# The-African-Research-Collective/karanta-ocr

Measured on AMD Instinct MI355X. Metric: pages_per_sec, higher is better.
Workload: dtype bf16; 1 GPU; Qwen2-VL-2B bf16 greedy, batch=8 synthetic 1024x1024 pages per GPU, max_pixels=1003520 (grid 70x70, 1225 image tokens), prompt P=1394 tokens, T_out=1024 (ignore_eos), random-init weights; global_batch=8, parallelism=dp1, decode=hipGraph replay

## Files before the change

include/karanta_hip.h:

```cpp
#ifndef KARANTA_HIP_H
#define KARANTA_HIP_H

#include <stddef.h>
#include <stdint.h>

#ifdef __cplusplus
extern "C" {
#endif

typedef void* kr_stream;
typedef uint16_t kr_bf16;

#define KR_ABI_VERSION 403

#define KR_OK 0
#define KR_ERR_ARG (-1)
#define KR_ERR_HIP (-2)
#define KR_ERR_RCCL (-3)
#define KR_ERR_STATE (-4)

#define KR_EPI_NONE 0
#define KR_EPI_QUICK_GELU 1
#define KR_EPI_GELU_ERF 2
#define KR_EPI_SILU_MUL 3
#define KR_EPI_SILU_MUL8 4

int kr_version(void);
const char* kr_last_error(void);
int kr_device_info(int device, char* name64, int* compute_units, size_t* total_mem);
int kr_set_device(int device);
int kr_stream_synchronize(kr_stream s);
int kr_stream_create_cu_mask(kr_stream* out, int cus_enabled);
int kr_stream_create_cu_range(kr_stream* out, int first_cu, int n_cus);
int kr_stream_destroy(kr_stream s);

int kr_event_create(void** ev);
int kr_event_destroy(void* ev);
int kr_event_record(void* ev, kr_stream s);
int kr_stream_wait_event(kr_stream s, void* ev);
int kr_event_synchronize(void* ev);
int kr_event_elapsed_ms(void* start, void* stop, float* ms);

int kr_graph_begin_capture(kr_stream s);
int kr_graph_end_capture(kr_stream s, void** graph_exec);
int kr_graph_launch(void* graph_exec, kr_stream s);
int kr_graph_destroy(void* graph_exec);


int kr_cast_pad_f32_bf16(const float* src, kr_bf16* dst, int64_t rows, int k, int k_pad, kr_stream s);

int kr_layernorm(const kr_bf16* x, const kr_bf16* w, const kr_bf16* b, kr_bf16* y,
                 int64_t rows, int d, float eps, kr_stream s);

int kr_rmsnorm(const kr_bf16* x, int64_t ldx, const kr_bf16* w, kr_bf16* y,
               int64_t rows, int d, float eps, kr_stream s);


int kr_gemm_bf16(const kr_bf16* A, int64_t lda, const kr_bf16* W, const kr_bf16* bias,
                 const kr_bf16* residual, int64_t ldr, kr_bf16* C, int64_t ldc,
                 int64_t M, int N, int K, int epilogue, int w_packed, kr_stream s);

#define KR_GEMM_SCRATCH_BYTES ((size_t)512 * 65536)
int kr_gemm_bf16_ws(const kr_bf16* A, int64_t lda, const kr_bf16* W, const kr_bf16* bias,
                    const kr_bf16* residual, int64_t ldr, kr_bf16* C, int64_t ldc,
                    int64_t M, int N, int K, int epilogue, int w_packed, float* scratch, size_t scratch_bytes, kr_stream s);

int kr_gemm_fp8(const kr_bf16* A, int64_t lda, const uint8_t* w_packed_fp8, const float* w_scale, const kr_bf16* bias,
                const kr_bf16* residual, int64_t ldr, kr_bf16* C, int64_t ldc, int64_t M, int N, int K, int epilogue,
                kr_stream s);

int kr_quantize_rows_fp8(const kr_bf16* x, int64_t ldx, uint8_t* q, int64_t ldq, float* scale, int64_t rows, int K, kr_stream s);
int kr_gemm_fp8a(const uint8_t* A8, int64_t lda, const float* a_scale, const uint8_t* w_packed_fp8, const float* w_scale,
                 const kr_bf16* bias, const kr_bf16* residual, int64_t ldr, kr_bf16* C, int64_t ldc, int64_t M, int N, int K,
                 int epilogue, kr_stream s);

int kr_gemv_bf16(const kr_bf16* x, int64_t ldx, const kr_bf16* W, const kr_bf16* bias,
                 const kr_bf16* residual, int64_t ldr, kr_bf16* out, float* out_f32, int64_t ldc,
                 int M, int N, int K, int epilogue,
                 const kr_bf16* norm_w, float norm_eps, kr_stream s);


int kr_qkv_prep(const kr_bf16* qkv, int64_t ld_qkv, int q_off, int k_off, int v_off,
                const float* cos, const float* sin,
                const int32_t* blk_tok0, const int32_t* blk_ntok,
                const int64_t* blk_k_row0, const int64_t* blk_vt_blk, int n_blk,
                kr_bf16* q_out, int64_t q_head_stride, kr_bf16* k_out, int64_t k_head_stride,
                kr_bf16* vt_out, int64_t vt_head_stride, int q_heads, int kv_heads, int hd,
                kr_stream s);

int kr_rope2d_vision(kr_bf16* x, const float* cos, const float* sin, int64_t n, int heads, int hd,
                     int64_t row_stride, kr_stream s);

int kr_attn_varlen(const kr_bf16* q, const kr_bf16* k, const kr_bf16* vt, kr_bf16* out,
                   const int32_t* qblk, const int32_t* qblk_len, int n_qblk,
                   int64_t nq_total, int q_heads, int kv_heads, int hd,
                   int64_t k_head_stride, int64_t vt_head_stride, float scale, int causal,
                   kr_stream s);
int kr_attn_varlen_q(const kr_bf16* q, const kr_bf16* k, const kr_bf16* vt, kr_bf16* out,
                     const int32_t* qblk, const int32_t* qblk_len, int n_qblk,
                     int64_t nq_total, int q_heads, int kv_heads, int hd,
                     int64_t k_head_stride, int64_t vt_head_stride, float scale, int causal,
                     int q_block, kr_stream s);


int kr_embed_scatter(const int32_t* src, const kr_bf16* table, const kr_bf16* image_embeds,
                     kr_bf16* out, int64_t rows, int d, kr_stream s);


int kr_mrope(kr_bf16* x, const float* cos, const float* sin, int64_t n, int heads, int hd,
             int64_t row_stride, kr_stream s);
int kr_kv_append(const kr_bf16* k, const kr_bf16* v, int64_t row_stride,
                 const int32_t* tok_seq, const int32_t* tok_pos,
                 kr_bf16* kcache, kr_bf16* vtcache,
                 int64_t n, int kv_heads, int hd, int layer, int batch, int s_max, kr_stream s);

int kr_decode_qkv_prep(const kr_bf16* qkv, const float* inv_freq, const int32_t* ctx_len,
                       const int32_t* rope_delta, kr_bf16* q_out, kr_bf16* kcache, kr_bf16* vtcache,
                       int batch, int heads, int kv_heads, int hd, int layer, int s_max, kr_stream s);

int kr_attn_decode_gqa(const kr_bf16* q, const kr_bf16* kcache, const kr_bf16* vtcache,
                       const int32_t* ctx_len, kr_bf16* out, float* workspace,
                       int batch, int heads, int kv_heads, int hd, int layer, int s_max,
                       int n_split, float scale, kr_stream s);

int kr_argmax_embed(const float* logits, int64_t ld_logits, int vocab,
                    const kr_bf16* embed_table, int d,
                    int32_t* tokens_out, int32_t* history, int32_t* step_ptr, int32_t* ctx_len,
                    int32_t* finished, const int32_t* eos, int n_eos, int pad_id, int ignore_eos,
                    kr_bf16* x_next, int batch, int hist_stride, kr_stream s);

int kr_argmax(const float* logits, int64_t ld_logits, int vocab, int32_t* out, int batch, kr_stream s);

#define KR_DEC_PLAIN 0
#define KR_DEC_SILU 1
#define KR_DEC_ROPE_KV 2
#define KR_DEC_ARGMAX 3
#define KR_DEC_SILU8 4
#define KR_DEC_OUT_XP 0x100
int kr_linear_decode(int mode, const kr_bf16* x, int64_t ldx, const kr_bf16* w_packed, const kr_bf16* bias,
                     const kr_bf16* norm_w, float norm_eps, const kr_bf16* residual, int64_t ldr,
                     kr_bf16* out, float* out_f32, int64_t ldc, int M, int N, int K, int waves, int max_blocks, int ksplit,
                     float* ws, int32_t* counters, const float* attn_partials, int attn_split,
                     const float* cs_table, int cs_stride, const int32_t* prompt_len, const int32_t* ctx_len,
                     kr_bf16* q_out, kr_bf16* kcache, kr_bf16* vtcache, int heads, int kv_heads, int s_max,
                     float* amax_val, int32_t* amax_idx, kr_stream s);

int kr_linear_decode_wide(int mode, const kr_bf16* x, int64_t ldx, const kr_bf16* w_packed, const kr_bf16* bias,
                          const kr_bf16* norm_w, float norm_eps, const kr_bf16* residual, int64_t ldr,
                          kr_bf16* out, float* out_f32, int64_t ldc, int M, int N, int K, int blocks, int waves,
                          float* amax_val, int32_t* amax_idx, kr_stream s);

typedef struct kr_narrow_opts {
    float* zero_ptr;
    uint64_t zero_bytes;
    int32_t atomic_out;
    int32_t part_rows;
} kr_narrow_opts;

int kr_linear_decode_narrow(int mode, const kr_bf16* x, int64_t ldx, const float* part_in, int n_part_in,
                            kr_bf16* x_out, int64_t ldxo, const kr_bf16* w_packed, const kr_bf16* bias,
                            const kr_bf16* norm_w, float norm_eps, const kr_bf16* residual, int64_t ldr,
                            kr_bf16* out, float* out_f32, int64_t ldc, int M, int N, int K, int waves, int ksplit,
                            const float* cs_table, int cs_stride, const int32_t* prompt_len, const int32_t* ctx_len,
                            kr_bf16* q_out, kr_bf16* kcache, kr_bf16* vtcache, int heads, int kv_heads, int s_max,
                            const kr_narrow_opts* opts, kr_stream s);

int kr_decode_resnorm(const kr_bf16* x, int64_t ldx, const float* part_in, int n_part_in, int part_rows, kr_bf16* x_out,
                      int64_t ldxo, const kr_bf16* norm_w, float norm_eps, kr_bf16* h, int64_t ldh, int M, int K, kr_stream s);

int kr_linear_decode_wide_fp8(int mode, const kr_bf16* x, int64_t ldx, const uint8_t* w_packed_fp8, const float* w_scale,
                              const kr_bf16* bias, const kr_bf16* norm_w, float norm_eps, const kr_bf16* residual,
                              int64_t ldr, kr_bf16* out, float* out_f32, int64_t ldc, int M, int N, int K, int blocks,
                              int waves, float* amax_val, int32_t* amax_idx, kr_stream s);
int kr_linear_decode_narrow_fp8(int mode, const kr_bf16* x, int64_t ldx, const float* part_in, int n_part_in,
                                kr_bf16* x_out, int64_t ldxo, const uint8_t* w_packed_fp8, const float* w_scale,
                                const kr_bf16* bias, const kr_bf16* norm_w, float norm_eps, const kr_bf16* residual,
                                int64_t ldr, kr_bf16* out, float* out_f32, int64_t ldc, int M, int N, int K, int waves,
                                int ksplit, const float* cs_table, int cs_stride, const int32_t* prompt_len,
                                const int32_t* ctx_len, kr_bf16* q_out, kr_bf16* kcache, kr_bf16* vtcache, int heads,
                                int kv_heads, int s_max, const kr_narrow_opts* opts, kr_stream s);
int kr_pack_rows32(const kr_bf16* x, int64_t ldx, int M, int K, kr_bf16* xp, kr_stream s);

typedef struct kr_dec32 {
    const kr_bf16* xp;
    const void* w_packed;
    const float* w_scale;
    const kr_bf16* bias;
    const kr_bf16* residual;
    int64_t ldr;
    kr_bf16* out;
    float* out_f32;
    int64_t ldc;
    int32_t M, N, K;
    int32_t waves_ref, ksplit;
    int32_t atomic_out;
    int32_t tiles_per_wg;
    int32_t group_split;
    int32_t reserved0;
    float* zero_ptr;
    uint64_t zero_bytes;
    const float* cs_table; int32_t cs_stride; const int32_t* prompt_len; const int32_t* ctx_len;
    kr_bf16* q_out; kr_bf16* kcache; kr_bf16* vtcache; int32_t heads, kv_heads, s_max;
} kr_dec32;
int kr_linear_decode32(int mode, const kr_dec32* args, kr_stream s);

int kr_decode_resnorm32(const kr_bf16* x, int64_t ldx, const float* part_in, int n_part_in, int part_rows, kr_bf16* x_out,
                        int64_t ldxo, const kr_bf16* norm_w, float norm_eps, kr_bf16* h_xp, int M, int K, int sum_slabs_first,
                        kr_stream s);

int kr_fp8_to_bf16(const uint8_t* src, kr_bf16* dst, int64_t n, kr_stream s);

int kr_attn_decode_fused(const kr_bf16* q, const kr_bf16* kcache, const kr_bf16* vtcache,
                         const int32_t* ctx_len, kr_bf16* out, float* workspace, int32_t* counters,
                         int batch, int heads, int kv_heads, int hd, int s_max, int n_split,
                         float scale, kr_stream s);
int kr_attn_decode_slots(const kr_bf16* q, const kr_bf16* kcache, const kr_bf16* vtcache, const int32_t* ctx_len,
                         const int32_t* finished, float* workspace, int batch, int heads, int kv_heads, int hd, int s_max,
                         int n_split, float scale, kr_stream s);
// ... 85 lines not shown
```

karanta_ocr_amd/_lib.py:

```python
from __future__ import annotations

import ctypes as C
import os
from typing import Optional

_HERE = os.path.dirname(os.path.abspath(__file__))
LIB_PATH = os.path.join(_HERE, "libkaranta_hip.so")

c_p = C.c_void_p
i32, i64, f32 = C.c_int, C.c_int64, C.c_float


class KarantaHipError(RuntimeError):
    pass


SIGNATURES = {
    "kr_version": [],
    "kr_last_error": [],
    "kr_device_info": [i32, C.c_char_p, C.POINTER(i32), C.POINTER(C.c_size_t)],
    "kr_set_device": [i32],
    "kr_stream_synchronize": [c_p],
    "kr_stream_create_cu_mask": [C.POINTER(c_p), i32],
    "kr_stream_create_cu_range": [C.POINTER(c_p), i32, i32],
    "kr_stream_destroy": [c_p],
    "kr_event_create": [C.POINTER(c_p)],
    "kr_event_destroy": [c_p],
    "kr_event_record": [c_p, c_p],
    "kr_event_synchronize": [c_p],
    "kr_stream_wait_event": [c_p, c_p],
    "kr_event_elapsed_ms": [c_p, c_p, C.POINTER(f32)],
    "kr_graph_begin_capture": [c_p],
    "kr_graph_end_capture": [c_p, C.POINTER(c_p)],
    "kr_graph_launch": [c_p, c_p],
    "kr_graph_destroy": [c_p],
    "kr_cast_pad_f32_bf16": [c_p, c_p, i64, i32, i32, c_p],
    "kr_layernorm": [c_p, c_p, c_p, c_p, i64, i32, f32, c_p],
    "kr_rmsnorm": [c_p, i64, c_p, c_p, i64, i32, f32, c_p],
    "kr_gemm_bf16": [c_p, i64, c_p, c_p, c_p, i64, c_p, i64, i64, i32, i32, i32, i32, c_p],
    "kr_decode_resnorm": [c_p, i64, c_p, i32, i32, c_p, i64, c_p, f32, c_p, i64, i32, i32, c_p],
    "kr_decode_resnorm32": [c_p, i64, c_p, i32, i32, c_p, i64, c_p, f32, c_p, i32, i32, i32, c_p],
    "kr_pack_rows32": [c_p, i64, i32, i32, c_p, c_p],
    "kr_linear_decode32": [i32, c_p, c_p],
    "kr_attn_decode_merge32": [c_p, c_p, i32, i32, i32, i32, c_p],
    "kr_quantize_rows_fp8": [c_p, i64, c_p, i64, c_p, i64, i32, c_p],
    "kr_gemm_fp8a": [c_p, i64, c_p, c_p, c_p, c_p, c_p, i64, c_p, i64, i64, i32, i32, i32, c_p],
    "kr_gemm_bf16_ws": [c_p, i64, c_p, c_p, c_p, i64, c_p, i64, i64, i32, i32, i32, i32, c_p, C.c_size_t, c_p],
    "kr_gemv_bf16": [c_p, i64, c_p, c_p, c_p, i64, c_p, c_p, i64, i32, i32, i32, i32, c_p, f32, c_p],
    "kr_qkv_prep": [c_p, i64, i32, i32, i32, c_p, c_p, c_p, c_p, c_p, c_p, i32, c_p, i64, c_p, i64, c_p, i64,
                    i32, i32, i32, c_p],
    "kr_rope2d_vision": [c_p, c_p, c_p, i64, i32, i32, i64, c_p],
    "kr_attn_varlen": [c_p, c_p, c_p, c_p, c_p, c_p, i32, i64, i32, i32, i32, i64, i64, f32, i32, c_p],
    "kr_attn_varlen_q": [c_p, c_p, c_p, c_p, c_p, c_p, i32, i64, i32, i32, i32, i64, i64, f32, i32, i32, c_p],
    "kr_embed_scatter": [c_p, c_p, c_p, c_p, i64, i32, c_p],
    "kr_mrope": [c_p, c_p, c_p, i64, i32, i32, i64, c_p],
    "kr_kv_append": [c_p, c_p, i64, c_p, c_p, c_p, c_p, i64, i32, i32, i32, i32, i32, c_p],
    "kr_decode_qkv_prep": [c_p, c_p, c_p, c_p, c_p, c_p, c_p, i32, i32, i32, i32, i32, i32, c_p],
    "kr_attn_decode_gqa": [c_p, c_p, c_p, c_p, c_p, c_p, i32, i32, i32, i32, i32, i32, i32, f32, c_p],
    "kr_argmax_embed": [c_p, i64, i32, c_p, i32, c_p, c_p, c_p, c_p, c_p, c_p, i32, i32, i32, c_p, i32, i32, c_p],
    "kr_argmax": [c_p, i64, i32, c_p, i32, c_p],
    "kr_linear_decode": [i32, c_p, i64, c_p, c_p, c_p, f32, c_p, i64, c_p, c_p, i64, i32, i32, i32, i32, i32, i32, c_p, c_p,
                         c_p, i32, c_p, i32, c_p, c_p, c_p, c_p, c_p, i32, i32, i32, c_p, c_p, c_p],
    "kr_linear_decode_wide": [i32, c_p, i64, c_p, c_p, c_p, f32, c_p, i64, c_p, c_p, i64, i32, i32, i32, i32, i32, c_p, c_p, c_p],
    "kr_image_resize_bicubic_u8": [c_p, i32, i32, c_p, i32, i32, c_p, c_p, c_p, i32, c_p, c_p, i32, c_p],
    "kr_image_normalize_patchify": [c_p, i32, i32, c_p, c_p, i32, i32, i32, c_p, c_p],
    "kr_linear_decode_wide_fp8": [i32, c_p, i64, c_p, c_p, c_p, c_p, f32, c_p, i64, c_p, c_p, i64, i32, i32, i32, i32, i32, c_p, c_p, c_p],
    "kr_linear_decode_narrow_fp8": [i32, c_p, i64, c_p, i32, c_p, i64, c_p, c_p, c_p, c_p, f32, c_p, i64, c_p, c_p, i64,
                                    i32, i32, i32, i32, i32, c_p, i32, c_p, c_p, c_p, c_p, c_p, i32, i32, i32, c_p, c_p],
    "kr_fp8_to_bf16": [c_p, c_p, i64, c_p],
    "kr_gemm_fp8": [c_p, i64, c_p, c_p, c_p, c_p, i64, c_p, i64, i64, i32, i32, i32, c_p],
    "kr_gumbel_argmax": [c_p, i64, i32, c_p, c_p, c_p, c_p, c_p, c_p, i32, i32, c_p],
    "kr_gumbel_argmax_guided": [c_p, i64, i32, c_p, c_p, c_p, c_p, c_p, c_p, i32, i32, c_p, c_p, i32, i32, c_p],
    "kr_guide_build_masks": [c_p, c_p, i32, c_p, c_p, i32, c_p, i32, c_p, i32, c_p],
    "kr_sample_threshold": [c_p, i64, i32, c_p, c_p, c_p, i64, c_p, i32, c_p, c_p, i32, c_p, i32, c_p, i64, c_p, c_p, i32, c_p],
    "kr_gumbel_argmax_processed": [c_p, i64, i32, c_p, c_p, c_p, c_p, c_p, c_p, i32, i32, c_p, c_p, i32, i32, c_p, c_p, i64, c_p,
                                   i32, c_p, c_p],
    "kr_sample_count": [c_p, c_p, c_p, i64, i32, i32, c_p],
    "kr_logits_adjust": [c_p, i64, i32, c_p, c_p, c_p, c_p, c_p, c_p, c_p, i32, c_p],
    "kr_logits_restore": [c_p, i64, i32, c_p, c_p, c_p, i32, c_p],
    "kr_stop_tokens": [c_p, c_p, c_p, c_p, c_p, i32, i32, c_p],
    "kr_guide_advance": [c_p, c_p, c_p, c_p, c_p, c_p, i32, i32, c_p],
    "kr_logprobs_topk": [c_p, i64, i32, i32, i32, c_p, c_p, c_p, c_p, c_p, c_p, c_p, c_p, c_p, i32, i32, i32, i32, c_p],
    "kr_linear_decode_narrow": [i32, c_p, i64, c_p, i32, c_p, i64, c_p, c_p, c_p, f32, c_p, i64, c_p, c_p, i64,
                                i32, i32, i32, i32, i32, c_p, i32, c_p, c_p, c_p, c_p, c_p, i32, i32, i32, c_p, c_p],
    "kr_attn_decode_fused": [c_p, c_p, c_p, c_p, c_p, c_p, c_p, i32, i32, i32, i32, i32, i32, f32, c_p],
    "kr_attn_decode_slots": [c_p, c_p, c_p, c_p, c_p, c_p, i32, i32, i32, i32, i32, i32, f32, c_p],
    "kr_attn_decode_merge": [c_p, c_p, i32, i32, i32, i32, c_p],
    "kr_sample_greedy": [c_p, c_p, i32, c_p, i32, c_p, c_p, i32, c_p, c_p, c_p, c_p, i32, i32, i32, c_p, i32, c_p],
    "kr_comm_unique_id": [c_p],
    "kr_comm_init": [C.POINTER(c_p), i32, i32, c_p],
    "kr_comm_count": [c_p, C.POINTER(i32)],
    "kr_comm_destroy": [c_p],
    "kr_rccl_version": [C.POINTER(i32)],
    "kr_bcast_weights": [c_p, c_p, C.c_size_t, i32, c_p],
    "kr_selftest_mfma": [c_p],
    "kr_probe_launch_floor": [c_p, i32, i32, i32, C.POINTER(f32)],
    "kr_probe_stream_read": [c_p, C.c_size_t, i32, i32, c_p, C.POINTER(f32)],
    "kr_launch_null": [c_p],
}
_RESTYPES = {"kr_last_error": C.c_char_p}

EXPERIMENT_SIGNATURES = {
    "kr_linear_decode_narrow_x32": [i32, c_p, i64, c_p, i32, c_p, i64, c_p, i64, c_p, c_p, c_p, c_p, f32, c_p, i64, c_p, c_p, i64,
                                    i32, i32, i32, i32, i32, c_p, i32, c_p, c_p, c_p, c_p, c_p, i32, i32, i32, c_p,
                                    c_p, C.c_size_t, i32, c_p],
    "kr_oproj_heads": [c_p, i32, c_p, c_p, c_p, i64, i32, i32, i32, c_p],
    "kr_linear_decode_wide_x32": [i32, c_p, i64, c_p, i64, c_p, c_p, c_p, f32, c_p, c_p, i64, i32, i32, i32, i32, i32, c_p, c_p, c_p],
    "kr_prefetch": [c_p, C.c_size_t, i32, c_p],
}


class NarrowOpts(C.Structure):
    _fields_ = [("zero_ptr", c_p), ("zero_bytes", C.c_uint64), ("atomic_out", C.c_int32), ("part_rows", C.c_int32)]


def narrow_opts(zero_ptr: int = 0, zero_bytes: int = 0, atomic_out: bool = False, part_rows: int = 0):
    if not (zero_bytes or atomic_out or part_rows):
        return None
    return C.byref(NarrowOpts(zero_ptr or None, int(zero_bytes), 1 if atomic_out else 0, int(part_rows)))

class Dec32(C.Structure):
    _fields_ = [("xp", c_p), ("w_packed", c_p), ("w_scale", c_p), ("bias", c_p), ("residual", c_p), ("ldr", C.c_int64),
                ("out", c_p), ("out_f32", c_p), ("ldc", C.c_int64), ("M", C.c_int32), ("N", C.c_int32), ("K", C.c_int32),
                ("waves_ref", C.c_int32), ("ksplit", C.c_int32), ("atomic_out", C.c_int32), ("tiles_per_wg", C.c_int32),
                ("group_split", C.c_int32), ("reserved0", C.c_int32), ("zero_ptr", c_p), ("zero_bytes", C.c_uint64),
                ("cs_table", c_p), ("cs_stride", C.c_int32), ("prompt_len", c_p), ("ctx_len", c_p),
                ("q_out", c_p), ("kcache", c_p), ("vtcache", c_p), ("heads", C.c_int32), ("kv_heads", C.c_int32), ("s_max", C.c_int32)]


ABI_MAJOR = 4
DEC_OUT_XP = 0x100
ADJ_CAP = 320
EPI_NONE, EPI_QUICK_GELU, EPI_GELU_ERF, EPI_SILU_MUL, EPI_SILU_MUL8 = 0, 1, 2, 3, 4
DEC_PLAIN, DEC_SILU, DEC_ROPE_KV, DEC_ARGMAX, DEC_SILU8 = 0, 1, 2, 3, 4


class _Lib:
    def __init__(self, path: str):
        if not os.path.exists(path):
            raise KarantaHipError(
                f"{path} not found: build it with `python -m karanta_ocr_amd.build` "
                "(the MI355X engine has no CPU fallback)")
        import torch

        try:
            self._dll = C.CDLL(path, mode=C.RTLD_GLOBAL)
        except OSError as e:
            raise KarantaHipError(f"cannot load {path}: {e}") from e
        self.path = path
        for name, argtypes in SIGNATURES.items():
            try:
                fn = getattr(self._dll, name)
            except AttributeError as e:
                raise KarantaHipError(f"{path} does not export {name}") from e
            fn.argtypes = argtypes
            fn.restype = _RESTYPES.get(name, C.c_int)
            if name in ("kr_version", "kr_last_error"):
                setattr(self, name, fn)
            else:
                setattr(self, name, self._checked(name, fn))
        if self.kr_version() // 100 != ABI_MAJOR:
            raise KarantaHipError(f"{path} reports kr_version() = {self.kr_version()}, this binding is written against ABI major "
                                  f"{ABI_MAJOR} (include/karanta_hip.h): rebuild with `python -m karanta_ocr_amd.build`")
        self.experiments = hasattr(self._dll, "kr_oproj_heads")
        for name, argtypes in EXPERIMENT_SIGNATURES.items():
            if self.experiments:
                fn = getattr(self._dll, name)
                fn.argtypes, fn.restype = argtypes, C.c_int
                setattr(self, name, self._checked(name, fn))
            else:
                setattr(self, name, self._absent(name))

    @staticmethod
    def _absent(name):
        def call(*_):
            raise KarantaHipError(f"{name} is an experiment entry point (include/karanta_hip_experiments.h): this library was built "
                                  "without -DKR_EXPERIMENTS (csrc/tools/build_variant.py; load it through KARANTA_HIP_LIB)")
        call.__name__ = name
        return call

    def _checked(self, name, fn):
        def call(*args):
            rc = fn(*args)
            if rc != 0:
                msg = self._dll.kr_last_error()
                raise KarantaHipError(f"{name} -> {rc}: {msg.decode() if msg else ''}")
            return rc

        call.__name__ = name
        call.raw = fn
        return call


_LIB: Optional[_Lib] = None


def lib() -> _Lib:
    global _LIB
    if _LIB is None:
        _LIB = _Lib(os.environ.get("KARANTA_HIP_LIB", LIB_PATH))
# ... 6 lines not shown
```

karanta_ocr_amd/csrc/kr_gemm.hip:

```cpp
#include <algorithm>
#include <cstdlib>
#include <mutex>
#include <optional>

#include "kr_common.h"

namespace {

constexpr int BK = 64;
struct G128 { static constexpr int BM = 128, BN = 128, WM = 2, WN = 2; };
struct G256 { static constexpr int BM = 256, BN = 256, WM = 2, WN = 4; };

__device__ __forceinline__ int lds_off(int r, int c) { return r * 128 + ((c ^ ((r >> 1) & 7)) << 4); }

template <bool PACKED, int ROWS, int NTHR>
__device__ __forceinline__ void stage_tile(const kr_bf16* __restrict__ g, int64_t ld, int64_t row0, int64_t rows_total,
                                           int k0, char* lds_tile, int tid, int wave) {
#pragma unroll
    for (int p = 0; p < ROWS * 8 / NTHR; ++p) {
        const int idx = p * NTHR + tid;
        const int r = idx >> 3, cp = idx & 7;
        const int c = cp ^ ((r >> 1) & 7);
        int64_t gr = row0 + r;
        gr = gr < rows_total ? gr : rows_total - 1;
// ... 5 lines not shown
    }
}

template <int EPI, int NT, int MT, bool LDSEPI, bool HAS_R, int CH = 0>
__device__ __forceinline__ void gemm_epilogue_impl(f32x4 (&acc)[NT][MT], const kr_bf16* __restrict__ bias,
                                                   const kr_bf16* __restrict__ R, int64_t ldr, kr_bf16* __restrict__ C, int64_t ldc,
                                                   int64_t M, int N, int64_t m_base, int n_base, int fr, int fg, char* wlds_) {
    constexpr bool HALF = EPI == KR_EPI_SILU_MUL8;
    constexpr int ROWB = HALF ? 64 : 128;
    char* const wlds = wlds_;
    auto swz = [](int r) { return HALF ? ((r >> 1) & 3) : (r & 7); };
    auto flush = [&](int mt0, int nmt) {
        constexpr int LPR = ROWB / 16, RPI = 64 / LPR;
        const int lane = fg * 16 + fr;
        const int n_out = HALF ? (n_base >> 1) : n_base, n_lim = HALF ? (N >> 1) : N;
#pragma unroll
        for (int it = 0; it < MT * 16 / RPI; ++it) {
            if (it < nmt * 16 / RPI) {
                const int r = it * RPI + lane / LPR, c = lane % LPR;
                const u32x4 v = *reinterpret_cast<const u32x4*>(wlds + r * ROWB + ((c ^ swz(r)) << 4));
                const int64_t m = m_base + mt0 * 16 + r;
                const int n = n_out + c * 8;
                if (m < M && n < n_lim) *reinterpret_cast<u32x4*>(C + m * ldc + n) = v;
            }
        }
    };
    constexpr int RM = CH > 0 ? CH : MT;
    if (EPI == KR_EPI_SILU_MUL8) {
        bf16x4 bv[NT];
#pragma unroll
        for (int nt = 0; nt < NT; ++nt) {
            const int n = min(n_base + nt * 16, N - 16);
            bv[nt] = bias ? *reinterpret_cast<const bf16x4*>(bias + n + fg * 4) : bf16x4{};
        }
#pragma unroll
        for (int mt = 0; mt < MT; ++mt) {
            const int64_t m = m_base + mt * 16 + fr;
#pragma unroll
            for (int nt = 0; nt < NT; ++nt) {
                const int n = n_base + nt * 16;
                float g[4], u[4];
#pragma unroll
                for (int j = 0; j < 4; ++j) g[j] = acc[nt][mt][j] + bf2f(bv[nt][j]);
#pragma unroll
                for (int j = 0; j < 4; ++j) u[j] = __shfl_xor(g[j], 32, 64);
                bf16x4 o;
#pragma unroll
                for (int j = 0; j < 4; ++j) o[j] = f2bf(act_silu(g[j]) * u[j]);
                if (LDSEPI) {
                    const int r = (mt % RM) * 16 + fr;
                    if (fg < 2) *reinterpret_cast<bf16x4*>(wlds + r * ROWB + ((nt ^ swz(r)) << 4) + (fg & 1) * 8) = o;
                } else if (fg < 2 && n < N && m < M) {
                    *reinterpret_cast<bf16x4*>(C + m * ldc + (n >> 1) + fg * 4) = o;
                }
            }
            if (LDSEPI && CH > 0 && (mt % RM) == RM - 1) flush(mt - (RM - 1), RM);
        }
    } else if (EPI == KR_EPI_SILU_MUL) {
#pragma unroll
        for (int mt = 0; mt < MT; ++mt) {
            const int64_t m = m_base + mt * 16 + fr;
            if (m >= M) continue;
#pragma unroll
            for (int pr = 0; pr < NT / 2; ++pr) {
                const int n = n_base + pr * 32 + fg * 4;
                if (n >= N) continue;
                const int oc = ((n_base) >> 1) + pr * 16 + fg * 4;
                bf16x4 o;
#pragma unroll
                for (int j = 0; j < 4; ++j) o[j] = f2bf(act_silu(acc[2 * pr][mt][j]) * acc[2 * pr + 1][mt][j]);
                *reinterpret_cast<bf16x4*>(C + m * ldc + oc) = o;
            }
        }
    } else {
        bf16x4 bv[NT];
        int ncl[NT];
#pragma unroll
        for (int nt = 0; nt < NT; ++nt) {
            ncl[nt] = min(n_base + nt * 16 + fg * 4, N - 4);
            bv[nt] = bias ? *reinterpret_cast<const bf16x4*>(bias + ncl[nt]) : bf16x4{};
        }
#pragma unroll
        for (int mt = 0; mt < MT; ++mt) {
            const int64_t m = m_base + mt * 16 + fr;
            const int64_t mc = m < M ? m : M - 1;
            bf16x4 rv[NT];
#pragma unroll
            for (int nt = 0; nt < NT; ++nt) rv[nt] = HAS_R ? *reinterpret_cast<const bf16x4*>(R + mc * ldr + ncl[nt]) : bf16x4{};
#pragma unroll
            for (int nt = 0; nt < NT; ++nt) {
                const int n = n_base + nt * 16 + fg * 4;
                float v[4];
#pragma unroll
                for (int j = 0; j < 4; ++j) v[j] = acc[nt][mt][j];
                if (bias) {
#pragma unroll
                    for (int j = 0; j < 4; ++j) v[j] += bf2f(bv[nt][j]);
                }
                if (EPI == KR_EPI_QUICK_GELU) {
#pragma unroll
                    for (int j = 0; j < 4; ++j) v[j] = act_quick_gelu(v[j]);
                } else if (EPI == KR_EPI_GELU_ERF) {
#pragma unroll
                    for (int j = 0; j < 4; ++j) v[j] = act_gelu_erf(v[j]);
                }
                if (HAS_R) {
#pragma unroll
                    for (int j = 0; j < 4; ++j) v[j] += bf2f(rv[nt][j]);
                }
                bf16x4 o;
#pragma unroll
                for (int j = 0; j < 4; ++j) o[j] = f2bf(v[j]);
                if (LDSEPI) {
                    const int r = (mt % RM) * 16 + fr;
                    *reinterpret_cast<bf16x4*>(wlds + r * ROWB + (((nt * 2 + (fg >> 1)) ^ swz(r)) << 4) + (fg & 1) * 8) = o;
                } else if (m < M && n < N) {
                    *reinterpret_cast<bf16x4*>(C + m * ldc + n) = o;
                }
            }
            if (LDSEPI && CH > 0 && (mt % RM) == RM - 1) flush(mt - (RM - 1), RM);
        }
    }
    if (LDSEPI && CH == 0) flush(0, MT);
}

template <int EPI, int NT, int MT, bool LDSEPI, int CH = 0>
__device__ __forceinline__ void gemm_epilogue(f32x4 (&acc)[NT][MT], const kr_bf16* __restrict__ bias,
                                              const kr_bf16* __restrict__ R, int64_t ldr, kr_bf16* __restrict__ C, int64_t ldc,
                                              int64_t M, int N, int64_t m_base, int n_base, int fr, int fg, char* wlds) {
    constexpr bool L = LDSEPI && EPI != KR_EPI_SILU_MUL;
    if constexpr (EPI == KR_EPI_SILU_MUL || EPI == KR_EPI_SILU_MUL8) {
        gemm_epilogue_impl<EPI, NT, MT, L, false, CH>(acc, bias, R, ldr, C, ldc, M, N, m_base, n_base, fr, fg, wlds);
    } else {
        if (R) gemm_epilogue_impl<EPI, NT, MT, L, true, CH>(acc, bias, R, ldr, C, ldc, M, N, m_base, n_base, fr, fg, wlds);
        else gemm_epilogue_impl<EPI, NT, MT, L, false, CH>(acc, bias, R, ldr, C, ldc, M, N, m_base, n_base, fr, fg, wlds);
    }
}

__device__ __forceinline__ void tile_coords(unsigned id, unsigned tiles_m, unsigned tiles_n, unsigned group_m, unsigned& tm,
                                            unsigned& tn) {
    if (group_m <= 1) {
        tm = id / tiles_n;
        tn = id - tm * tiles_n;
        return;
    }
    const unsigned per_group = group_m * tiles_n;
    const unsigned g = id / per_group, first = g * group_m;
    const unsigned gsz = min(tiles_m - first, group_m);
    const unsigned r = id - g * per_group;
    tn = r / gsz;
    tm = first + (r - tn * gsz);
}

template <int EPI, bool WPACK, typename G, int STAGES = 2>
__global__ void __launch_bounds__(G::WM * G::WN * 64) gemm_kernel(const kr_bf16* __restrict__ A, int64_t lda,
                                                   const kr_bf16* __restrict__ W, const kr_bf16* __restrict__ bias,
                                                   const kr_bf16* __restrict__ R, int64_t ldr, kr_bf16* __restrict__ C,
                                                   int64_t ldc, int64_t M, int N, int K, int tiles_n, unsigned nwg,
                                                   int ptiles_n, unsigned qbase, int group_m, int ksplit, int ks_mode,
                                                   float* __restrict__ ws) {
    constexpr int BM = G::BM, BN = G::BN, NTHR = G::WM * G::WN * 64;
    constexpr int WTM = BM / G::WM, WTN = BN / G::WN;
    constexpr int MT = WTM / 16, NT = WTN / 16;
    constexpr int A_BYTES = BM * BK * 2, W_BYTES = BN * BK * 2, STAGE = A_BYTES + W_BYTES;
    extern __shared__ __attribute__((aligned(16))) char smem[];
    const int tid = threadIdx.x;
    const int lane = tid & 63;
    const int wave = __builtin_amdgcn_readfirstlane(tid >> 6);
    const int wr = wave / G::WN, wc = wave % G::WN;

    unsigned wg = xcd_remap(blockIdx.x, nwg);
    int64_t m0 = (int64_t)(wg / tiles_n) * BM;
    int n0 = (int)(wg % tiles_n) * BN;
    unsigned qid = 0, sidx = 0;
    if (ptiles_n > 0) {
        if (ks_mode == 1) {
            wg = blockIdx.x;
            qid = wg / (unsigned)ksplit;
            sidx = wg - qid * (unsigned)ksplit;
            wg = qid;
        } else {
            qid = wg;
        }
        const unsigned parent = qbase + (wg >> 2), sub = wg & 3u;
        unsigned tm, tn;
        tile_coords(parent, (unsigned)((M + 255) >> 8), (unsigned)ptiles_n, (unsigned)group_m, tm, tn);
        m0 = (int64_t)tm * 256 + (sub >> 1) * 128;
        n0 = (int)tn * 256 + (int)(sub & 1u) * 128;
        if (m0 >= M) return;
    }

    f32x4 acc[NT][MT];
#pragma unroll
    for (int i = 0; i < NT; ++i)
#pragma unroll
        for (int j = 0; j < MT; ++j) acc[i][j] = (f32x4){0.f, 0.f, 0.f, 0.f};

    int kt0 = 0, nk = K / BK;
    if (ks_mode == 1) {
        const int q = nk / ksplit, r = nk - q * ksplit;
        kt0 = (int)sidx * q + min((int)sidx, r);
        nk = kt0 + q + ((int)sidx < r ? 1 : 0);
    }
    const int fr = lane & 15, fg = lane >> 4;
    constexpr int FRAGS = NT * MT;
    if (ks_mode == 2) {
        for (int sp = 0; sp < ksplit; ++sp) {
            const f32x4* part = reinterpret_cast<const f32x4*>(ws) + (((size_t)qid * ksplit + sp) * NTHR + tid) * FRAGS;
#pragma unroll
            for (int i = 0; i < NT; ++i)
#pragma unroll
                for (int j = 0; j < MT; ++j) {
                    const f32x4 pv = part[i * MT + j];
#pragma unroll
                    for (int c = 0; c < 4; ++c) acc[i][j][c] += pv[c];
                }
        }
        nk = 0;
    }
    constexpr int LPT = (BM + BN) * 8 / NTHR;
    auto stage = [&](int kt, int buf) {
        stage_tile<false, BM, NTHR>(A, lda, m0, M, kt * BK, smem + buf * STAGE, tid, wave);
        stage_tile<WPACK, BN, NTHR>(W, K, n0, N, kt * BK, smem + buf * STAGE + A_BYTES, tid, wave);
    };
    if constexpr (STAGES == 2) {
        if (kt0 < nk) {
            stage(kt0, 0);
            asm volatile("s_waitcnt vmcnt(0)" ::: "memory");
        }
        __syncthreads();
    } else {
        static_assert(STAGES == 4, "ring depth");
#pragma unroll
        for (int p = 0; p < STAGES - 1; ++p)
            if (kt0 + p < nk) stage(kt0 + p, p);
    }

    for (int kt = kt0; kt < nk; ++kt) {
        const int ki = kt - kt0;
        char* cur = smem + (ki % STAGES) * STAGE;
        if constexpr (STAGES == 2) {
            if (kt + 1 < nk) stage(kt + 1, (ki + 1) & 1);
        } else {
            if (kt + STAGES - 1 < nk) stage(kt + STAGES - 1, (ki + STAGES - 1) % STAGES);
            const int later = min(STAGES - 1, nk - 1 - kt);
            if (later == 3) asm volatile("s_waitcnt vmcnt(%0)" ::"n"(3 * LPT) : "memory");
            else if (later == 2) asm volatile("s_waitcnt vmcnt(%0)" ::"n"(2 * LPT) : "memory");
            else if (later == 1) asm volatile("s_waitcnt vmcnt(%0)" ::"n"(1 * LPT) : "memory");
            else asm volatile("s_waitcnt vmcnt(0)" ::: "memory");
            asm volatile("" ::: "memory");
            __builtin_amdgcn_s_barrier();
            asm volatile("" ::: "memory");
        }
        const char* At = cur;
        const char* Wt = cur + A_BYTES;
#pragma unroll
        for (int ks = 0; ks < 2; ++ks) {
            bf16x8 xa[MT], wb[NT];
#pragma unroll
            for (int t = 0; t < NT; ++t)
                wb[t] = *reinterpret_cast<const bf16x8*>(Wt + lds_off(wc * WTN + t * 16 + fr, ks * 4 + fg));
#pragma unroll
            for (int t = 0; t < MT; ++t)
                xa[t] = *reinterpret_cast<const bf16x8*>(At + lds_off(wr * WTM + t * 16 + fr, ks * 4 + fg));
#pragma unroll
            for (int nt = 0; nt < NT; ++nt)
#pragma unroll
                for (int mt = 0; mt < MT; ++mt)
                    acc[nt][mt] = __builtin_amdgcn_mfma_f32_16x16x32_bf16(wb[nt], xa[mt], acc[nt][mt], 0, 0, 0);
        }
        if constexpr (STAGES == 2) {
            asm volatile("s_waitcnt vmcnt(0)" ::: "memory");
            __syncthreads();
        } else {
            asm volatile("" ::: "memory");
            __builtin_amdgcn_s_barrier();
            asm volatile("" ::: "memory");
        }
    }

    if (ks_mode == 1) {
        f32x4* part = reinterpret_cast<f32x4*>(ws) + (((size_t)qid * ksplit + sidx) * NTHR + tid) * FRAGS;
#pragma unroll
        for (int i = 0; i < NT; ++i)
#pragma unroll
            for (int j = 0; j < MT; ++j) part[i * MT + j] = acc[i][j];
        return;
    }
    gemm_epilogue<EPI, NT, MT, G::BM == 256>(acc, bias, R, ldr, C, ldc, M, N, m0 + wr * WTM, n0 + wc * WTN, fr, fg,
                                             smem + wave * (WTM * 128));
}

constexpr int PK = 32, PBUF = 2 * 256 * PK * 2, PSTAGES = 4;

template <bool PACKED>
__device__ __forceinline__ void stage_rows32(const kr_bf16* __restrict__ g, int64_t ld, int64_t row0, int64_t rows_total, int k0,
                                             char* lds_op, int lane, int wave) {
#pragma unroll
    for (int h = 0; h < 2; ++h) {
        const int r = h * 128 + wave * 16 + (lane >> 2);
        const int c = (lane & 3) ^ (((lane >> 5) & 1) << 1);
        int64_t gr = row0 + r;
        gr = gr < rows_total ? gr : rows_total - 1;
        const kr_bf16* src = PACKED ? g + ((((gr >> 4) * (ld >> 5) + (k0 >> 5)) * 4 + c) * 16 + (gr & 15)) * 8
                                    : g + gr * ld + k0 + c * 8;
        char* dst = lds_op + (h * 128 + wave * 16) * 64;
        __builtin_amdgcn_global_load_lds((const __attribute__((address_space(1))) void*)src,
                                         (__attribute__((address_space(3))) void*)dst, 16, 0, 0);
    }
}

__device__ __forceinline__ void stage_w8_rows32(const uint8_t* __restrict__ g, int K, int n0, int N, int k0, char* lds_op, int lane,
                                                int wave) {
    int rb = (n0 >> 4) + 2 * wave + (lane >> 5);
    rb = min(rb, (N >> 4) - 1);
    const uint8_t* src = g + ((int64_t)rb * (K >> 6) + (k0 >> 6)) * 1024 + ((k0 & 32) ? 512 : 0) + (lane & 31) * 16;
    char* dst = lds_op + wave * 1024;
    __builtin_amdgcn_global_load_lds((const __attribute__((address_space(1))) void*)src,
                                     (__attribute__((address_space(3))) void*)dst, 16, 0, 0);
}

__device__ __forceinline__ void stage_a8_rows32(const uint8_t* __restrict__ g, int64_t ld, int64_t row0, int64_t rows_total, int k0,
                                                char* lds_op, int lane, int wave) {
    const int r = wave * 32 + (lane >> 1);
    const int p = (lane & 1) ^ ((r >> 3) & 1);
    int64_t gr = row0 + r;
    gr = gr < rows_total ? gr : rows_total - 1;
    const uint8_t* src = g + gr * ld + k0 + p * 16;
    char* dst = lds_op + wave * 1024;
    __builtin_amdgcn_global_load_lds((const __attribute__((address_space(1))) void*)src,
                                     (__attribute__((address_space(3))) void*)dst, 16, 0, 0);
}

__device__ __forceinline__ bf16x8 fp8x8_to_bf16(u32x2 q) {
    u32x4 o;
#pragma unroll
    for (int i = 0; i < 2; ++i) {
        o[2 * i + 0] = __builtin_bit_cast(unsigned, __builtin_amdgcn_cvt_scalef32_pk_bf16_fp8((int)q[i], 1.0f, false));
        o[2 * i + 1] = __builtin_bit_cast(unsigned, __builtin_amdgcn_cvt_scalef32_pk_bf16_fp8((int)q[i], 1.0f, true));
    }
    return __builtin_bit_cast(bf16x8, o);
}

template <int EPI, bool WPACK, bool W8, bool A8 = false, bool PERSIST = false>
__global__ void __launch_bounds__(512) gemm_pipe_kernel(const kr_bf16* __restrict__ A, int64_t lda, const kr_bf16* __restrict__ W,
                                                        const kr_bf16* __restrict__ bias, const kr_bf16* __restrict__ R,
                                                        int64_t ldr, kr_bf16* __restrict__ C, int64_t ldc, int64_t M, int N, int K,
                                                        int tiles_n, unsigned nwg, const float* __restrict__ w_scale, int group_m,
                                                        const float* __restrict__ a_scale = nullptr, int stagger = 0) {
    static_assert(!A8 || W8, "fp8 activations go with fp8 weights");
    if (stagger > 0 && blockIdx.x < 256u && ((blockIdx.x >> 3) & 1u)) {
        for (int i = 0; i < stagger; ++i) __builtin_amdgcn_s_sleep(127);
    }
    constexpr int NT = 4, MT = 8, A_BYTES = 256 * PK * 2;
    const uint8_t* W8p = reinterpret_cast<const uint8_t*>(W);
    const uint8_t* A8p = reinterpret_cast<const uint8_t*>(A);
    extern __shared__ __attribute__((aligned(16))) char smem[];
    const int tid = threadIdx.x, lane = tid & 63;
    const int wave = __builtin_amdgcn_readfirstlane(tid >> 6);
    const int wr = wave >> 2, wc = wave & 3;
    const int fr = lane & 15, fg = lane >> 4;
    int64_t m0;
    int n0;
    auto set_tile = [&](unsigned t) {
        unsigned id;
        if constexpr (PERSIST) {
            const unsigned r0 = (t / gridDim.x) * gridDim.x;
            id = r0 + xcd_remap(t - r0, min(gridDim.x, nwg - r0));
        } else {
            id = xcd_remap(t, nwg);
        }
        unsigned tm, tn;
        tile_coords(id, (unsigned)((M + 255) >> 8), (unsigned)tiles_n, (unsigned)group_m, tm, tn);
        m0 = (int64_t)tm * 256;
        n0 = (int)tn * 256;
    };
    unsigned tile = blockIdx.x;
    set_tile(tile);

    f32x4 acc[NT][MT];

    const int nk = K / PK;
    const int sw = ((fg ^ (((fr >> 3) & 1) << 1)) << 4);
    const int a_off = A8 ? (wr * 128 + fr) * 32 + ((((fg >> 1) ^ ((fr >> 3) & 1))) << 4) + ((fg & 1) << 3)
                         : (wr * 128 + fr) * 64 + sw;
    const int w_off = W8 ? A_BYTES + wc * 4 * 512 + (fg >> 1) * 256 + fr * 16 + (fg & 1) * 8
                         : A_BYTES + (wc * 64 + fr) * 64 + sw;
    auto stage_w = [&](int k0, char* buf) {
        if constexpr (W8) stage_w8_rows32(W8p, K, n0, N, k0, buf + A_BYTES, lane, wave);
        else stage_rows32<WPACK>(W, K, n0, N, k0, buf + A_BYTES, lane, wave);
    };
    auto stage_a = [&](int k0, char* buf) {
        if constexpr (A8) stage_a8_rows32(A8p, lda, m0, M, k0, buf, lane, wave);
        else stage_rows32<false>(A, lda, m0, M, k0, buf, lane, wave);
    };

#pragma unroll
    for (int t = 0; t < 3; ++t) {
        if (t < nk) {
            char* buf = smem + t * PBUF;
            stage_w(t * PK, buf);
            stage_a(t * PK, buf);
        }
    }
    auto wait_two = [] {
        if constexpr (A8) asm volatile("s_waitcnt vmcnt(4)" ::: "memory");
        else if constexpr (W8) asm volatile("s_waitcnt vmcnt(6)" ::: "memory");
        else asm volatile("s_waitcnt vmcnt(8)" ::: "memory");
    };
    auto wait_one = [] {
        if constexpr (A8) asm volatile("s_waitcnt vmcnt(2)" ::: "memory");
        else if constexpr (W8) asm volatile("s_waitcnt vmcnt(3)" ::: "memory");
        else asm volatile("s_waitcnt vmcnt(4)" ::: "memory");
    };
    if (nk >= 3) wait_two();
    else if (nk == 2) wait_one();
    else asm volatile("s_waitcnt vmcnt(0)" ::: "memory");
    __builtin_amdgcn_s_barrier();

    bf16x8 wb[NT], xa[4];
    u32x2 xq[4];
    for (;;) {
#pragma unroll
    for (int i = 0; i < NT; ++i)
#pragma unroll
        for (int j = 0; j < MT; ++j) acc[i][j] = (f32x4){0.f, 0.f, 0.f, 0.f};
    if (wr == 1) __builtin_amdgcn_s_barrier();
    for (int k = 0; k < nk; ++k) {
        const char* cur = smem + (k & 3) * PBUF;
        char* nxt = smem + ((k + 3) & 3) * PBUF;
        const bool more = k + 3 < nk;
        u32x2 wq[NT];
        if constexpr (W8) {
#pragma unroll
            for (int t = 0; t < NT; ++t) wq[t] = *reinterpret_cast<const u32x2*>(cur + w_off + t * 512);
        } else {
#pragma unroll
            for (int t = 0; t < NT; ++t) wb[t] = *reinterpret_cast<const bf16x8*>(cur + w_off + t * 16 * 64);
        }
        __builtin_amdgcn_sched_barrier(0);
        if constexpr (A8) {
#pragma unroll
            for (int t = 0; t < 4; ++t) xq[t] = *reinterpret_cast<const u32x2*>(cur + a_off + t * 16 * 32);
        } else {
#pragma unroll
            for (int t = 0; t < 4; ++t) xa[t] = *reinterpret_cast<const bf16x8*>(cur + a_off + t * 16 * 64);
        }
        if (more) stage_w((k + 3) * PK, nxt);
        __builtin_amdgcn_s_barrier();
        asm volatile("s_waitcnt lgkmcnt(0)" ::: "memory");
        if constexpr (W8 && !A8) {
#pragma unroll
            for (int t = 0; t < NT; ++t) wb[t] = fp8x8_to_bf16(wq[t]);
        }
        __builtin_amdgcn_s_setprio(1);
#pragma unroll
        for (int mt = 0; mt < 4; ++mt)
#pragma unroll
            for (int nt = 0; nt < NT; ++nt) {
                if constexpr (A8)
                    acc[nt][mt] = __builtin_amdgcn_mfma_f32_16x16x32_fp8_fp8(__builtin_bit_cast(long, wq[nt]), __builtin_bit_cast(long, xq[mt]),
                                                                             acc[nt][mt], 0, 0, 0);
                else
                    acc[nt][mt] = __builtin_amdgcn_mfma_f32_16x16x32_bf16(wb[nt], xa[mt], acc[nt][mt], 0, 0, 0);
            }
        __builtin_amdgcn_s_setprio(0);
        __builtin_amdgcn_s_barrier();
        if constexpr (A8) {
#pragma unroll
            for (int t = 0; t < 4; ++t) xq[t] = *reinterpret_cast<const u32x2*>(cur + a_off + (4 + t) * 16 * 32);
        } else {
#pragma unroll
            for (int t = 0; t < 4; ++t) xa[t] = *reinterpret_cast<const bf16x8*>(cur + a_off + (4 + t) * 16 * 64);
        }
        if (more) stage_a((k + 3) * PK, nxt);
        if (more) wait_two();
        else if (k + 3 == nk) wait_one();
        else asm volatile("s_waitcnt vmcnt(0)" ::: "memory");
        __builtin_amdgcn_s_barrier();
        asm volatile("s_waitcnt lgkmcnt(0)" ::: "memory");
        __builtin_amdgcn_s_setprio(1);
#pragma unroll
        for (int mt = 0; mt < 4; ++mt)
#pragma unroll
            for (int nt = 0; nt < NT; ++nt) {
                if constexpr (A8)
                    acc[nt][4 + mt] = __builtin_amdgcn_mfma_f32_16x16x32_fp8_fp8(__builtin_bit_cast(long, wq[nt]), __builtin_bit_cast(long, xq[mt]),
                                                                                 acc[nt][4 + mt], 0, 0, 0);
                else
                    acc[nt][4 + mt] = __builtin_amdgcn_mfma_f32_16x16x32_bf16(wb[nt], xa[mt], acc[nt][4 + mt], 0, 0, 0);
            }
        __builtin_amdgcn_s_setprio(0);
        __builtin_amdgcn_s_barrier();
    }
    if (wr == 0) __builtin_amdgcn_s_barrier();
    const int64_t m0_cur = m0;
    const int n0_cur = n0;
    bool more_tiles = false;
    if constexpr (PERSIST) {
        tile += gridDim.x;
        more_tiles = tile < nwg;
        if (more_tiles) {
            set_tile(tile);
#pragma unroll
            for (int t = 0; t < 3; ++t) {
                if (t < nk) {
                    char* buf = smem + t * PBUF;
                    stage_w(t * PK, buf);
                    stage_a(t * PK, buf);
                }
            }
        }
    }
    if constexpr (W8) {
#pragma unroll
        for (int nt = 0; nt < NT; ++nt) {
            const f32x4 sc = *reinterpret_cast<const f32x4*>(w_scale + min(n0_cur + wc * 64 + nt * 16 + fg * 4, N - 4));
#pragma unroll
            for (int mt = 0; mt < MT; ++mt)
#pragma unroll
                for (int j = 0; j < 4; ++j) acc[nt][mt][j] *= sc[j];
        }
    }
    if constexpr (A8) {
#pragma unroll
        for (int mt = 0; mt < MT; ++mt) {
            const int64_t m = m0_cur + wr * 128 + mt * 16 + fr;
            const float as = a_scale[m < M ? m : M - 1];
#pragma unroll
            for (int nt = 0; nt < NT; ++nt)
#pragma unroll
                for (int j = 0; j < 4; ++j) acc[nt][mt][j] *= as;
        }
    }
    if constexpr (PERSIST) {
        gemm_epilogue<EPI, NT, MT, true, 2>(acc, bias, R, ldr, C, ldc, M, N, m0_cur + wr * 128, n0_cur + wc * 64, fr, fg,
                                            smem + PSTAGES * PBUF + wave * 4096);
        if (!more_tiles) break;
        asm volatile("s_waitcnt vmcnt(0)" ::: "memory");
        __builtin_amdgcn_s_barrier();
    } else {
        gemm_epilogue<EPI, NT, MT, true>(acc, bias, R, ldr, C, ldc, M, N, m0_cur + wr * 128, n0_cur + wc * 64, fr, fg,
                                         smem + wave * (128 * 128));
        break;
    }
    }
}

typedef __attribute__((ext_vector_type(8))) int i32x8;
typedef __attribute__((ext_vector_type(16))) float f32x16;

__device__ __forceinline__ void stage_a8_rows64(const uint8_t* __restrict__ g, int64_t ld, int64_t row0, int64_t rows_total, int k0,
                                                char* lds_op, int lane, int wave) {
#pragma unroll
    for (int h = 0; h < 2; ++h) {
        const int r = h * 128 + wave * 16 + (lane >> 2);
        const int c = (lane & 3) ^ ((lane >> 4) & 3);
        int64_t gr = row0 + r;
        gr = gr < rows_total ? gr : rows_total - 1;
        const uint8_t* src = g + gr * ld + k0 + c * 16;
        char* dst = lds_op + (h * 128 + wave * 16) * 64;
        __builtin_amdgcn_global_load_lds((const __attribute__((address_space(1))) void*)src,
                                         (__attribute__((address_space(3))) void*)dst, 16, 0, 0);
    }
}

__device__ __forceinline__ void stage_w8_rows64(const uint8_t* __restrict__ g, int K, int n0, int N, int k0, char* lds_op, int lane,
                                                int wave) {
#pragma unroll
    for (int h = 0; h < 2; ++h) {
        int rb = (n0 >> 4) + 2 * wave + h;
        rb = min(rb, (N >> 4) - 1);
        const uint8_t* src = g + ((int64_t)rb * (K >> 6) + (k0 >> 6)) * 1024 + lane * 16;
        char* dst = lds_op + (2 * wave + h) * 1024;
        __builtin_amdgcn_global_load_lds((const __attribute__((address_space(1))) void*)src,
                                         (__attribute__((address_space(3))) void*)dst, 16, 0, 0);
    }
}

template <int EPI, bool TWO>
__global__ void __launch_bounds__(512) gemm_pipe_mx_kernel(const uint8_t* __restrict__ A8p, int64_t lda, const uint8_t* __restrict__ W8p,
                                                           const kr_bf16* __restrict__ bias, const kr_bf16* __restrict__ R, int64_t ldr,
                                                           kr_bf16* __restrict__ C, int64_t ldc, int64_t M, int N, int K, int tiles_n,
                                                           unsigned nwg, const float* __restrict__ w_scale, int group_m,
                                                           const float* __restrict__ a_scale) {
    constexpr int NT = 2, MT = 4, XK = 64, A_BYTES = 256 * XK, XBUF = 2 * A_BYTES;
    constexpr int ONE = 0x7f7f7f7f;
    extern __shared__ __attribute__((aligned(16))) char smem[];
    const int tid = threadIdx.x, lane = tid & 63;
    const int wave = __builtin_amdgcn_readfirstlane(tid >> 6);
    const int wr = wave >> 2, wc = wave & 3;
    const int cl = lane & 31, h = lane >> 5;
    const unsigned wg = xcd_remap(blockIdx.x, nwg);
    unsigned tm, tn;
    tile_coords(wg, (unsigned)((M + 255) >> 8), (unsigned)tiles_n, (unsigned)group_m, tm, tn);
    const int64_t m0 = (int64_t)tm * 256;
    const int n0 = (int)tn * 256;

    f32x16 acc[NT][MT];
#pragma unroll
    for (int i = 0; i < NT; ++i)
#pragma unroll
        for (int j = 0; j < MT; ++j)
#pragma unroll
            for (int e = 0; e < 16; ++e) acc[i][j][e] = 0.f;

    const int nk = K / XK;
    const int a_off = (wr * 128 + cl) * 64 + ((((2 * h) ^ ((cl >> 2) & 3))) << 4);
    const int a_off2 = (wr * 128 + cl) * 64 + ((((2 * h + 1) ^ ((cl >> 2) & 3))) << 4);
    const int w_off = A_BYTES + (wc * 4 + (cl >> 4)) * 1024 + (2 * h) * 256 + (cl & 15) * 16;

    if constexpr (TWO) {
        const int ni = nk >> 1;
        {
            stage_w8_rows64(W8p, K, n0, N, 0, smem + A_BYTES, lane, wave);
            stage_a8_rows64(A8p, lda, m0, M, 0, smem, lane, wave);
            stage_w8_rows64(W8p, K, n0, N, XK, smem + XBUF + A_BYTES, lane, wave);
            stage_a8_rows64(A8p, lda, m0, M, XK, smem + XBUF, lane, wave);
        }
        asm volatile("s_waitcnt vmcnt(0)" ::: "memory");
        __builtin_amdgcn_s_barrier();
        if (wr == 1) __builtin_amdgcn_s_barrier();
        for (int i = 0; i < ni; ++i) {
            const char* cur = smem + (i & 1) * 2 * XBUF;
            char* oth = smem + ((i + 1) & 1) * 2 * XBUF;
            const bool more = i + 1 < ni;
            u32x4 wq[2][NT][2], xq[2][2][2];
#pragma unroll
            for (int kt = 0; kt < 2; ++kt)
#pragma unroll
                for (int t = 0; t < NT; ++t) {
                    wq[kt][t][0] = *reinterpret_cast<const u32x4*>(cur + kt * XBUF + w_off + t * 2048);
                    wq[kt][t][1] = *reinterpret_cast<const u32x4*>(cur + kt * XBUF + w_off + t * 2048 + 256);
                }
            __builtin_amdgcn_sched_barrier(0);
#pragma unroll
            for (int kt = 0; kt < 2; ++kt)
#pragma unroll
                for (int t = 0; t < 2; ++t) {
                    xq[kt][t][0] = *reinterpret_cast<const u32x4*>(cur + kt * XBUF + a_off + t * 32 * 64);
                    xq[kt][t][1] = *reinterpret_cast<const u32x4*>(cur + kt * XBUF + a_off2 + t * 32 * 64);
                }
            if (more) {
#pragma unroll
                for (int kt = 0; kt < 2; ++kt) {
                    stage_w8_rows64(W8p, K, n0, N, (2 * i + 2 + kt) * XK, oth + kt * XBUF + A_BYTES, lane, wave);
                    stage_a8_rows64(A8p, lda, m0, M, (2 * i + 2 + kt) * XK, oth + kt * XBUF, lane, wave);
                }
            }
            __builtin_amdgcn_s_barrier();
            asm volatile("s_waitcnt lgkmcnt(0)" ::: "memory");
            i32x8 wf[2][NT];
#pragma unroll
            for (int kt = 0; kt < 2; ++kt)
#pragma unroll
                for (int t = 0; t < NT; ++t)
#pragma unroll
                    for (int e = 0; e < 4; ++e) {
                        wf[kt][t][e] = (int)wq[kt][t][0][e];
                        wf[kt][t][4 + e] = (int)wq[kt][t][1][e];
                    }
            __builtin_amdgcn_s_setprio(1);
#pragma unroll
            for (int kt = 0; kt < 2; ++kt)
#pragma unroll
                for (int mt = 0; mt < 2; ++mt) {
                    i32x8 xf;
#pragma unroll
                    for (int e = 0; e < 4; ++e) {
                        xf[e] = (int)xq[kt][mt][0][e];
                        xf[4 + e] = (int)xq[kt][mt][1][e];
                    }
#pragma unroll
                    for (int nt = 0; nt < NT; ++nt)
                        acc[nt][mt] = __builtin_amdgcn_mfma_scale_f32_32x32x64_f8f6f4(wf[kt][nt], xf, acc[nt][mt], 0, 0, 0, ONE, 0, ONE);
                }
            __builtin_amdgcn_s_setprio(0);
            __builtin_amdgcn_s_barrier();
#pragma unroll
            for (int kt = 0; kt < 2; ++kt)
#pragma unroll
                for (int t = 0; t < 2; ++t) {
                    xq[kt][t][0] = *reinterpret_cast<const u32x4*>(cur + kt * XBUF + a_off + (2 + t) * 32 * 64);
                    xq[kt][t][1] = *reinterpret_cast<const u32x4*>(cur + kt * XBUF + a_off2 + (2 + t) * 32 * 64);
                }
            asm volatile("s_waitcnt vmcnt(0) lgkmcnt(0)" ::: "memory");
            __builtin_amdgcn_s_barrier();
            __builtin_amdgcn_s_setprio(1);
#pragma unroll
            for (int kt = 0; kt < 2; ++kt)
#pragma unroll
                for (int mt = 0; mt < 2; ++mt) {
                    i32x8 xf;
// ... 70 lines not shown
        for (int t = 0; t < 2; ++t) {
            xq[t][0] = *reinterpret_cast<const u32x4*>(cur + a_off + (2 + t) * 32 * 64);
            xq[t][1] = *reinterpret_cast<const u32x4*>(cur + a_off2 + (2 + t) * 32 * 64);
        }
        if (more) stage_a8_rows64(A8p, lda, m0, M, (k + 3) * XK, nxt, lane, wave);
        if (more) asm volatile("s_waitcnt vmcnt(8)" ::: "memory");
        else if (k + 3 == nk) asm volatile("s_waitcnt vmcnt(4)" ::: "memory");
        else asm volatile("s_waitcnt vmcnt(0)" ::: "memory");
        __builtin_amdgcn_s_barrier();
        asm volatile("s_waitcnt lgkmcnt(0)" ::: "memory");
        __builtin_amdgcn_s_setprio(1);
#pragma unroll
        for (int mt = 0; mt < 2; ++mt) {
            i32x8 xf;
#pragma unroll
            for (int e = 0; e < 4; ++e) {
                xf[e] = (int)xq[mt][0][e];
                xf[4 + e] = (int)xq[mt][1][e];
            }
#pragma unroll
            for (int nt = 0; nt < NT; ++nt)
                acc[nt][2 + mt] = __builtin_amdgcn_mfma_scale_f32_32x32x64_f8f6f4(wf[nt], xf, acc[nt][2 + mt], 0, 0, 0, ONE, 0, ONE);
        }
        __builtin_amdgcn_s_setprio(0);
        __builtin_amdgcn_s_barrier();
    }
    }
    if (wr == 0) __builtin_amdgcn_s_barrier();

    constexpr bool HALF = EPI == KR_EPI_SILU_MUL8;
    constexpr int ROWB = HALF ? 64 : 128;
    char* const wlds = smem + wave * (128 * 128);
    const int64_t m_base = m0 + wr * 128;
    const int n_base = n0 + wc * 64;
    auto swz = [](int r) { return HALF ? ((r >> 1) & 3) : (r & 7); };
    float as[MT];
#pragma unroll
    for (int mt = 0; mt < MT; ++mt) {
        const int64_t m = m_base + mt * 32 + cl;
        as[mt] = a_scale[m < M ? m : M - 1];
    }
#pragma unroll
    for (int nt = 0; nt < NT; ++nt) {
#pragma unroll
        for (int q = 0; q < 4; ++q) {
            const int nq = n_base + nt * 32 + 8 * q + 4 * h;
            const int ncl = min(nq, N - 4);
            const f32x4 ws4 = *reinterpret_cast<const f32x4*>(w_scale + ncl);
            const bf16x4 bv = bias ? *reinterpret_cast<const bf16x4*>(bias + ncl) : bf16x4{};
#pragma unroll
            for (int mt = 0; mt < MT; ++mt)
#pragma unroll
                for (int j = 0; j < 4; ++j) acc[nt][mt][4 * q + j] = acc[nt][mt][4 * q + j] * ws4[j] * as[mt] + bf2f(bv[j]);
        }
    }
#pragma unroll
    for (int mt = 0; mt < MT; ++mt) {
        const int r = mt * 32 + cl;
        const int64_t m = m_base + r;
        const int64_t mc = m < M ? m : M - 1;
#pragma unroll
        for (int nt = 0; nt < NT; ++nt) {
            if constexpr (HALF) {
#pragma unroll
                for (int k16 = 0; k16 < 2; ++k16) {
                    bf16x4 o;
#pragma unroll
                    for (int j = 0; j < 4; ++j) o[j] = f2bf(act_silu(acc[nt][mt][8 * k16 + j]) * acc[nt][mt][8 * k16 + 4 + j]);
                    const int cc = nt * 2 + k16;
                    *reinterpret_cast<bf16x4*>(wlds + r * ROWB + ((cc ^ swz(r)) << 4) + h * 8) = o;
                }
            } else {
#pragma unroll
                for (int q = 0; q < 4; ++q) {
                    const int nq = n_base + nt * 32 + 8 * q + 4 * h;
                    float v[4];
#pragma unroll
                    for (int j = 0; j < 4; ++j) v[j] = acc[nt][mt][4 * q + j];
                    if (R) {
                        const bf16x4 rv = *reinterpret_cast<const bf16x4*>(R + mc * ldr + min(nq, N - 4));
#pragma unroll
                        for (int j = 0; j < 4; ++j) v[j] += bf2f(rv[j]);
                    }
                    bf16x4 o;
#pragma unroll
                    for (int j = 0; j < 4; ++j) o[j] = f2bf(v[j]);
                    const int cc = nt * 4 + q;
                    *reinterpret_cast<bf16x4*>(wlds + r * ROWB + ((cc ^ swz(r)) << 4) + h * 8) = o;
                }
            }
        }
    }
    {
        constexpr int LPR = ROWB / 16, RPI = 64 / LPR;
        const int n_out = HALF ? (n_base >> 1) : n_base, n_lim = HALF ? (N >> 1) : N;
#pragma unroll
        for (int it = 0; it < 128 / RPI; ++it) {
            const int r = it * RPI + lane / LPR, c = lane % LPR;
            const u32x4 v = *reinterpret_cast<const u32x4*>(wlds + r * ROWB + ((c ^ swz(r)) << 4));
            const int64_t m = m_base + r;
            const int n = n_out + c * 8;
            if (m < M && n < n_lim) *reinterpret_cast<u32x4*>(C + m * ldc + n) = v;
        }
    }
}

inline int kr_cu_count() {
    static int cus[64] = {0};
    int dev = 0;
    if (hipGetDevice(&dev) != hipSuccess || dev < 0 || dev >= 64) return 256;
    if (cus[dev] == 0) {
        int n = 0;
        cus[dev] = (hipDeviceGetAttribute(&n, hipDeviceAttributeMultiprocessorCount, dev) == hipSuccess && n > 0) ? n : 256;
    }
    return cus[dev];
}

inline std::optional<int> env_int(const char* name) {
    const char* v = getenv(name);
    return v ? std::optional<int>(atoi(v)) : std::nullopt;
}
constexpr bool MX_TWO_DEFAULT = false;

struct GemmTuning {
    int tile = env_int("KARANTA_GEMM_TILE").value_or(0);
    bool tail = env_int("KARANTA_GEMM_TAIL").value_or(1) != 0;
    int tail_min_k = env_int("KARANTA_GEMM_TAIL_MINK").value_or(0);
    int tail_ksplit = env_int("KARANTA_GEMM_TAIL_KSPLIT").value_or(16);
    std::optional<int> group_m = env_int("KARANTA_GEMM_GROUP_M");
    int stagger = env_int("KARANTA_GEMM_STAGGER").value_or(0);
    std::optional<int> stages = env_int("KARANTA_GEMM_STAGES");
    bool mx = env_int("KARANTA_FP8_MX").value_or(1) != 0;
    bool mx2 = env_int("KARANTA_FP8_MX2").value_or(MX_TWO_DEFAULT) != 0;
#ifdef KR_GEMM_PERSIST_EXPERIMENT
    bool persist = env_int("KARANTA_GEMM_PERSIST").value_or(1) != 0;
#endif

    int group_m_for(int tiles_n) const { return group_m.value_or(tiles_n >= 8 ? 8 : 1); }
    bool deep_ring(int64_t nwg) const { return stages ? *stages == 4 : nwg <= kr_cu_count(); }
};

struct GemmCall {
    const kr_bf16* A;
    int64_t lda;
    const kr_bf16 *W, *bias, *R;
    int64_t ldr;
    kr_bf16* C;
    int64_t ldc, M;
    int N, K;
    const float *w_scale, *a_scale;
    float* scratch;
    kr_stream s;
    GemmTuning tune;
};
constexpr int TAIL_MAX_WGS = 512, TAIL_WG_BYTES = 256 * 16 * 16;
static_assert((size_t)TAIL_MAX_WGS * TAIL_WG_BYTES == KR_GEMM_SCRATCH_BYTES, "karanta_hip.h: KR_GEMM_SCRATCH_BYTES");

template <int EPI, bool WPACK, typename G, int STAGES>
int launch_gemm_kernel(const GemmCall& c, unsigned nwg, int tiles_n, int ptiles_n, unsigned qbase, int group_m, int ksplit = 1,
                       int ks_mode = 0, float* ws = nullptr) {
    constexpr int LDS = STAGES * (G::BM + G::BN) * BK * 2;
    static KrPerDeviceOnce attr_set;
    if (attr_set.need()) {
        KR_CHECK_HIP(hipFuncSetAttribute(reinterpret_cast<const void*>(&gemm_kernel<EPI, WPACK, G, STAGES>),
                                         hipFuncAttributeMaxDynamicSharedMemorySize, LDS));
    }
    gemm_kernel<EPI, WPACK, G, STAGES><<<nwg, G::WM * G::WN * 64, LDS, kr_hs(c.s)>>>(
        c.A, c.lda, c.W, c.bias, c.R, c.ldr, c.C, c.ldc, c.M, c.N, c.K, tiles_n, nwg, ptiles_n, qbase, group_m, ksplit, ks_mode, ws);
    KR_CHECK_LAUNCH();
    return KR_OK;
}

template <int EPI, bool WPACK, typename G>
int launch_gemm3(const GemmCall& c) {
    const int64_t tiles_m = (c.M + G::BM - 1) / G::BM;
    const int tiles_n = (c.N + G::BN - 1) / G::BN;
    const int64_t nwg = tiles_m * tiles_n;
    KR_CHECK_ARG(nwg < (1ll << 31), "kr_gemm_bf16: grid too large");
    if constexpr (G::BM == 128) {
        if (c.tune.deep_ring(nwg)) return launch_gemm_kernel<EPI, WPACK, G, 4>(c, (unsigned)nwg, tiles_n, 0, 0u, 0);
    }
    return launch_gemm_kernel<EPI, WPACK, G, 2>(c, (unsigned)nwg, tiles_n, 0, 0u, 0);
}

template <int EPI, bool WPACK>
int launch_gemm_tail(const GemmCall& c, int ptiles_n, unsigned tile0, unsigned n_tiles, int group_m) {
    const unsigned nq = 4 * n_tiles;
    const int cap = c.tune.tail_ksplit;
    int ksplit = 1;
    if (cap > 1 && c.K >= 4096) ksplit = std::max(1, std::min(std::min(cap, (c.K / BK) / 8), (int)(kr_cu_count() / nq)));
    float* ws = (ksplit > 1 && nq * (unsigned)ksplit <= (unsigned)TAIL_MAX_WGS) ? c.scratch : nullptr;
    if (ws) {
        int rc = launch_gemm_kernel<EPI, WPACK, G128, 4>(c, nq * ksplit, 1, ptiles_n, tile0, group_m, ksplit, 1, ws);
        if (rc != KR_OK) return rc;
        return launch_gemm_kernel<EPI, WPACK, G128, 2>(c, nq, 1, ptiles_n, tile0, group_m, ksplit, 2, ws);
    }
    if (c.tune.deep_ring(nq)) return launch_gemm_kernel<EPI, WPACK, G128, 4>(c, nq, 1, ptiles_n, tile0, group_m);
    return launch_gemm_kernel<EPI, WPACK, G128, 2>(c, nq, 1, ptiles_n, tile0, group_m);
}

template <int EPI, bool WPACK, bool W8 = false, bool A8 = false>
int launch_gemm_pipe(const GemmCall& c) {
    constexpr int LDS = PSTAGES * PBUF;
    const int64_t tiles_m = (c.M + 255) / 256;
    const int tiles_n = (c.N + 255) / 256;
    int64_t nwg = tiles_m * tiles_n;
    KR_CHECK_ARG(nwg < (1ll << 31), "kr_gemm_bf16: grid too large");
    unsigned tail = 0;
    if constexpr (!W8) {
        const int cus = kr_cu_count();
        const int64_t t = nwg % cus;
        if (nwg > cus && t > 0 && 2 * t <= cus && (c.K >= c.tune.tail_min_k || t <= 4) && c.tune.tail) {
            tail = (unsigned)t;
            nwg -= t;
        }
    }
    static KrPerDeviceOnce attr_set;
    if (attr_set.need()) {
        KR_CHECK_HIP(hipFuncSetAttribute(reinterpret_cast<const void*>(&gemm_pipe_kernel<EPI, WPACK, W8, A8>),
                                         hipFuncAttributeMaxDynamicSharedMemorySize, LDS));
#ifdef KR_GEMM_PERSIST_EXPERIMENT
        KR_CHECK_HIP(hipFuncSetAttribute(reinterpret_cast<const void*>(&gemm_pipe_kernel<EPI, WPACK, W8, A8, true>),
                                         hipFuncAttributeMaxDynamicSharedMemorySize, LDS + 8 * 4096));
#endif
    }
    const int group_m = c.tune.group_m_for(tiles_n);
#ifdef KR_GEMM_PERSIST_EXPERIMENT
    if (c.tune.persist && nwg > kr_cu_count())
        gemm_pipe_kernel<EPI, WPACK, W8, A8, true><<<(unsigned)kr_cu_count(), 512, LDS + 8 * 4096, kr_hs(c.s)>>>(
            c.A, c.lda, c.W, c.bias, c.R, c.ldr, c.C, c.ldc, c.M, c.N, c.K, tiles_n, (unsigned)nwg, c.w_scale, group_m, c.a_scale, 0);
    else
#endif
        gemm_pipe_kernel<EPI, WPACK, W8, A8><<<(unsigned)nwg, 512, LDS, kr_hs(c.s)>>>(
            c.A, c.lda, c.W, c.bias, c.R, c.ldr, c.C, c.ldc, c.M, c.N, c.K, tiles_n, (unsigned)nwg, c.w_scale, group_m, c.a_scale,
            c.tune.stagger);
    KR_CHECK_LAUNCH();
    if constexpr (!W8) {
        if (tail) return launch_gemm_tail<EPI, WPACK>(c, tiles_n, (unsigned)nwg, tail, group_m);
    }
    return KR_OK;
}

template <int EPI>
int launch_gemm_pipe_mx(const GemmCall& c) {
    constexpr int LDS = 4 * 32768;
    const int64_t tiles_m = (c.M + 255) / 256;
    const int tiles_n = (c.N + 255) / 256;
    const int64_t nwg = tiles_m * tiles_n;
    KR_CHECK_ARG(nwg < (1ll << 31), "kr_gemm_fp8a: grid too large");
    static KrPerDeviceOnce attr_set;
    if (attr_set.need()) {
        KR_CHECK_HIP(hipFuncSetAttribute(reinterpret_cast<const void*>(&gemm_pipe_mx_kernel<EPI, false>), hipFuncAttributeMaxDynamicSharedMemorySize, LDS));
        KR_CHECK_HIP(hipFuncSetAttribute(reinterpret_cast<const void*>(&gemm_pipe_mx_kernel<EPI, true>), hipFuncAttributeMaxDynamicSharedMemorySize, LDS));
    }
    const auto fn = (c.tune.mx2 && (c.K % 128) == 0) ? &gemm_pipe_mx_kernel<EPI, true> : &gemm_pipe_mx_kernel<EPI, false>;
    fn<<<(unsigned)nwg, 512, LDS, kr_hs(c.s)>>>(reinterpret_cast<const uint8_t*>(c.A), c.lda, reinterpret_cast<const uint8_t*>(c.W), c.bias,
                                                c.R, c.ldr, c.C, c.ldc, c.M, c.N, c.K, tiles_n, (unsigned)nwg, c.w_scale,
                                                c.tune.group_m_for(tiles_n), c.a_scale);
    KR_CHECK_LAUNCH();
    return KR_OK;
}

template <int EPI, bool WPACK>
int launch_gemm2(const GemmCall& c) {
    int tile = c.tune.tile;
    if (tile != 128 && tile != 256 && tile != 512) {
        const int64_t wgs = ((c.M + 255) / 256) * ((c.N + 255) / 256);
        tile = (wgs >= 192 && c.N % 256 == 0) ? 512 : 128;
    }
    if ((c.ldc & 7) != 0 || (reinterpret_cast<uintptr_t>(c.C) & 15) != 0) tile = 128;
    if (tile == 512) return launch_gemm_pipe<EPI, WPACK>(c);
    if (tile == 256) return launch_gemm3<EPI, WPACK, G256>(c);
    return launch_gemm3<EPI, WPACK, G128>(c);
}

template <int EPI>
int launch_gemm(const GemmCall& c, int w_packed) {
    return w_packed ? launch_gemm2<EPI, true>(c) : launch_gemm2<EPI, false>(c);
}

}

extern "C" int kr_gemm_bf16(const kr_bf16* A, int64_t lda, const kr_bf16* W, const kr_bf16* bias,
                            const kr_bf16* residual, int64_t ldr, kr_bf16* C, int64_t ldc, int64_t M, int N, int K,
                            int epilogue, int w_packed, kr_stream s) {
    return kr_gemm_bf16_ws(A, lda, W, bias, residual, ldr, C, ldc, M, N, K, epilogue, w_packed, nullptr, 0, s);
}

extern "C" int kr_gemm_bf16_ws(const kr_bf16* A, int64_t lda, const kr_bf16* W, const kr_bf16* bias,
                               const kr_bf16* residual, int64_t ldr, kr_bf16* C, int64_t ldc, int64_t M, int N, int K,
                               int epilogue, int w_packed, float* scratch, size_t scratch_bytes, kr_stream s) {
    KR_CHECK_ARG(scratch == nullptr || (scratch_bytes >= KR_GEMM_SCRATCH_BYTES && ((uintptr_t)scratch & 15) == 0),
                 "kr_gemm_bf16_ws: scratch of %zu bytes (KR_GEMM_SCRATCH_BYTES = %zu, 16-byte aligned)", scratch_bytes,
                 (size_t)KR_GEMM_SCRATCH_BYTES);
    KR_CHECK_ARG(A && W && C, "kr_gemm_bf16: null pointer");
    KR_CHECK_ARG(M >= 0 && N > 0 && K > 0, "kr_gemm_bf16: bad sizes M=%lld N=%d K=%d", (long long)M, N, K);
    KR_CHECK_ARG(K % BK == 0, "kr_gemm_bf16: K=%d must be a multiple of %d", K, BK);
    KR_CHECK_ARG(N % 16 == 0, "kr_gemm_bf16: N=%d must be a multiple of 16", N);
    KR_CHECK_ARG(lda >= K && (lda & 7) == 0, "kr_gemm_bf16: lda=%lld", (long long)lda);
    KR_CHECK_ARG((ldc & 3) == 0 && (residual == nullptr || (ldr & 3) == 0), "kr_gemm_bf16: ldc/ldr alignment");
    KR_CHECK_ARG(((uintptr_t)A & 15) == 0 && ((uintptr_t)W & 15) == 0 && ((uintptr_t)C & 7) == 0,
                 "kr_gemm_bf16: pointer alignment");
    if (M == 0) return KR_OK;
    const GemmCall c{A, lda, W, bias, residual, ldr, C, ldc, M, N, K, nullptr, nullptr, scratch, s, GemmTuning()};
    switch (epilogue) {
        case KR_EPI_NONE:
            KR_CHECK_ARG(ldc >= N, "kr_gemm_bf16: ldc < N");
            return launch_gemm<KR_EPI_NONE>(c, w_packed);
        case KR_EPI_QUICK_GELU:
            KR_CHECK_ARG(ldc >= N, "kr_gemm_bf16: ldc < N");
            return launch_gemm<KR_EPI_QUICK_GELU>(c, w_packed);
        case KR_EPI_GELU_ERF:
            KR_CHECK_ARG(ldc >= N, "kr_gemm_bf16: ldc < N");
            return launch_gemm<KR_EPI_GELU_ERF>(c, w_packed);
        case KR_EPI_SILU_MUL:
            KR_CHECK_ARG(N % 32 == 0 && ldc >= N / 2 && !bias && !residual,
                         "kr_gemm_bf16: SILU_MUL needs N%%32==0, no bias/residual");
            return launch_gemm<KR_EPI_SILU_MUL>(c, w_packed);
        case KR_EPI_SILU_MUL8:
            KR_CHECK_ARG(ldc >= N / 2 && !residual, "kr_gemm_bf16: SILU_MUL8 takes no residual");
            return launch_gemm<KR_EPI_SILU_MUL8>(c, w_packed);
        default:
            kr_set_error("kr_gemm_bf16: unknown epilogue %d", epilogue);
            return KR_ERR_ARG;
    }
}

namespace {
template <int QMAX>
__global__ void __launch_bounds__(256) quantize_rows_fp8_kernel(const kr_bf16* __restrict__ x, int64_t ldx, uint8_t* __restrict__ q,
                                                                int64_t ldq, float* __restrict__ scale, int K) {
    __shared__ float red[4];
    const int tid = threadIdx.x, lane = tid & 63, wave = tid >> 6, kc = K >> 3;
    const kr_bf16* xr = x + (int64_t)blockIdx.x * ldx;
    bf16x8 v[QMAX];
    float amax = 0.f;
#pragma unroll
    for (int i = 0; i < QMAX; ++i) {
        const int c = tid + i * 256;
        if (c < kc) {
            v[i] = ld8(xr + c * 8);
#pragma unroll
            for (int j = 0; j < 8; ++j) amax = fmaxf(amax, fabsf(bf2f(v[i][j])));
        }
    }
#pragma unroll
    for (int o = 32; o >= 1; o >>= 1) amax = fmaxf(amax, __shfl_xor(amax, o, 64));
    if (lane == 0) red[wave] = amax;
    __syncthreads();
    amax = fmaxf(fmaxf(red[0], red[1]), fmaxf(red[2], red[3]));
    const float sc = amax > 0.f ? amax / 448.0f : 1.0f;
    if (tid == 0) scale[blockIdx.x] = sc;
    uint8_t* qr = q + (int64_t)blockIdx.x * ldq;
#pragma unroll
    for (int i = 0; i < QMAX; ++i) {
        const int c = tid + i * 256;
        if (c < kc) {
            u32x2 o;
#pragma unroll
            for (int h = 0; h < 2; ++h) {
                int w = 0;
                w = __builtin_amdgcn_cvt_pk_fp8_f32(bf2f(v[i][4 * h + 0]) / sc, bf2f(v[i][4 * h + 1]) / sc, w, false);
                w = __builtin_amdgcn_cvt_pk_fp8_f32(bf2f(v[i][4 * h + 2]) / sc, bf2f(v[i][4 * h + 3]) / sc, w, true);
                o[h] = (unsigned)w;
            }
            *reinterpret_cast<u32x2*>(qr + c * 8) = o;
        }
    }
}
}

extern "C" int kr_quantize_rows_fp8(const kr_bf16* x, int64_t ldx, uint8_t* q, int64_t ldq, float* scale, int64_t rows, int K,
                                    kr_stream s) {
    KR_CHECK_ARG(x && q && scale, "kr_quantize_rows_fp8: null pointer");
    KR_CHECK_ARG(rows >= 0 && rows < (1ll << 31) && K > 0 && K % 8 == 0 && K <= 8 * 256 * 12, "kr_quantize_rows_fp8: rows=%lld K=%d (K %% 8, K <= 24576)",
                 (long long)rows, K);
    KR_CHECK_ARG(ldx >= K && (ldx & 7) == 0 && ldq >= K && (ldq & 15) == 0 && ((uintptr_t)x & 15) == 0 && ((uintptr_t)q & 15) == 0,
                 "kr_quantize_rows_fp8: strides / alignment");
    if (rows == 0) return KR_OK;
    const int per = ((K >> 3) + 255) / 256;
    if (per <= 2) quantize_rows_fp8_kernel<2><<<(unsigned)rows, 256, 0, kr_hs(s)>>>(x, ldx, q, ldq, scale, K);
    else if (per <= 4) quantize_rows_fp8_kernel<4><<<(unsigned)rows, 256, 0, kr_hs(s)>>>(x, ldx, q, ldq, scale, K);
    else if (per <= 8) quantize_rows_fp8_kernel<8><<<(unsigned)rows, 256, 0, kr_hs(s)>>>(x, ldx, q, ldq, scale, K);
    else quantize_rows_fp8_kernel<12><<<(unsigned)rows, 256, 0, kr_hs(s)>>>(x, ldx, q, ldq, scale, K);
    KR_CHECK_LAUNCH();
    return KR_OK;
}

extern "C" int kr_gemm_fp8a(const uint8_t* A8, int64_t lda, const float* a_scale, const uint8_t* w_packed_fp8, const float* w_scale,
                            const kr_bf16* bias, const kr_bf16* residual, int64_t ldr, kr_bf16* C, int64_t ldc, int64_t M, int N, int K,
                            int epilogue, kr_stream s) {
    KR_CHECK_ARG(A8 && a_scale && w_packed_fp8 && w_scale && C, "kr_gemm_fp8a: null pointer");
    KR_CHECK_ARG(M >= 0 && N > 0 && K > 0, "kr_gemm_fp8a: bad sizes M=%lld N=%d K=%d", (long long)M, N, K);
    KR_CHECK_ARG(K % 64 == 0 && N % 16 == 0, "kr_gemm_fp8a: K=%d must be a multiple of 64, N=%d of 16", K, N);
    KR_CHECK_ARG(lda >= K && (lda & 15) == 0, "kr_gemm_fp8a: lda=%lld (bytes, a multiple of 16)", (long long)lda);
    KR_CHECK_ARG((ldc & 7) == 0 && ((uintptr_t)C & 15) == 0 && (residual == nullptr || (ldr & 3) == 0),
                 "kr_gemm_fp8a: C must be 16-byte aligned with ldc %% 8 == 0 (ldr %% 4 == 0)");
    KR_CHECK_ARG(((uintptr_t)A8 & 15) == 0 && ((uintptr_t)w_packed_fp8 & 15) == 0 && ((uintptr_t)w_scale & 15) == 0,
                 "kr_gemm_fp8a: pointer alignment");
    if (M == 0) return KR_OK;
    const GemmCall c{reinterpret_cast<const kr_bf16*>(A8), lda, reinterpret_cast<const kr_bf16*>(w_packed_fp8), bias, residual, ldr, C, ldc,
                     M, N, K, w_scale, a_scale, nullptr, s, GemmTuning()};
    const bool mx = c.tune.mx && N % 32 == 0;
    switch (epilogue) {
        case KR_EPI_NONE:
            KR_CHECK_ARG(ldc >= N, "kr_gemm_fp8a: ldc < N");
            return mx ? launch_gemm_pipe_mx<KR_EPI_NONE>(c) : launch_gemm_pipe<KR_EPI_NONE, true, true, true>(c);
        case KR_EPI_SILU_MUL8:
            KR_CHECK_ARG(ldc >= N / 2 && !residual, "kr_gemm_fp8a: SILU_MUL8 takes no residual");
            return mx ? launch_gemm_pipe_mx<KR_EPI_SILU_MUL8>(c) : launch_gemm_pipe<KR_EPI_SILU_MUL8, true, true, true>(c);
        default:
            kr_set_error("kr_gemm_fp8a: epilogue %d (NONE and SILU_MUL8 only: the decoder's prefill linears)", epilogue);
            return KR_ERR_ARG;
    }
}

extern "C" int kr_gemm_fp8(const kr_bf16* A, int64_t lda, const uint8_t* w_packed_fp8, const float* w_scale, const kr_bf16* bias,
                           const kr_bf16* residual, int64_t ldr, kr_bf16* C, int64_t ldc, int64_t M, int N, int K, int epilogue,
                           kr_stream s) {
    KR_CHECK_ARG(A && w_packed_fp8 && w_scale && C, "kr_gemm_fp8: null pointer");
    KR_CHECK_ARG(M >= 0 && N > 0 && K > 0, "kr_gemm_fp8: bad sizes M=%lld N=%d K=%d", (long long)M, N, K);
    KR_CHECK_ARG(K % 64 == 0 && N % 16 == 0, "kr_gemm_fp8: K=%d must be a multiple of 64, N=%d of 16", K, N);
    KR_CHECK_ARG(lda >= K && (lda & 7) == 0, "kr_gemm_fp8: lda=%lld", (long long)lda);
    KR_CHECK_ARG((ldc & 7) == 0 && ((uintptr_t)C & 15) == 0 && (residual == nullptr || (ldr & 3) == 0),
                 "kr_gemm_fp8: C must be 16-byte aligned with ldc %% 8 == 0 (ldr %% 4 == 0)");
    KR_CHECK_ARG(((uintptr_t)A & 15) == 0 && ((uintptr_t)w_packed_fp8 & 15) == 0 && ((uintptr_t)w_scale & 15) == 0,
                 "kr_gemm_fp8: pointer alignment");
    if (M == 0) return KR_OK;
    const GemmCall c{A, lda, reinterpret_cast<const kr_bf16*>(w_packed_fp8), bias, residual, ldr, C, ldc, M, N, K, w_scale, nullptr, nullptr,
                     s, GemmTuning()};
    switch (epilogue) {
        case KR_EPI_NONE:
            KR_CHECK_ARG(ldc >= N, "kr_gemm_fp8: ldc < N");
            return launch_gemm_pipe<KR_EPI_NONE, true, true>(c);
        case KR_EPI_SILU_MUL8:
            KR_CHECK_ARG(ldc >= N / 2 && !residual, "kr_gemm_fp8: SILU_MUL8 takes no residual");
            return launch_gemm_pipe<KR_EPI_SILU_MUL8, true, true>(c);
        default:
            kr_set_error("kr_gemm_fp8: epilogue %d (NONE and SILU_MUL8 only: the decoder's prefill linears)", epilogue);
            return KR_ERR_ARG;
    }
}

namespace {

constexpr int GV_U = 4;

template <int NT, int EPI, bool XLDS, bool OUTF32>
__global__ void __launch_bounds__(256) gemv_kernel(const kr_bf16* __restrict__ x, int64_t ldx,
                                                   const kr_bf16* __restrict__ W, const kr_bf16* __restrict__ bias,
                                                   const kr_bf16* __restrict__ R, int64_t ldr, kr_bf16* __restrict__ out,
                                                   float* __restrict__ outf, int64_t ldc, int M, int N, int K,
                                                   const kr_bf16* __restrict__ norm_w, float norm_eps) {
    extern __shared__ __attribute__((aligned(16))) char smem[];
    const int tid = threadIdx.x;
    const int lane = tid & 63;
    const int wave = __builtin_amdgcn_readfirstlane(tid >> 6);
    const int fr = lane & 15, fg = lane >> 4;
    const int n_base = blockIdx.x * (NT * 16);
    const int nchunks = K >> 6;
    const int xrow_bytes = K * 2 + 16;
    float* red = reinterpret_cast<float*>(smem + (XLDS ? ((M * xrow_bytes + 127) & ~127) : 0));
    float* rstd_s = red + 4 * NT * 256;

    const kr_bf16* wp[NT];
#pragma unroll
    for (int t = 0; t < NT; ++t) {
        int n = n_base + t * 16 + fr;
        n = n < N ? n : N - 1;
        wp[t] = W + (int64_t)n * K + fg * 16;
    }
    bf16x8 wbuf[GV_U][NT][2];
#pragma unroll
    for (int u = 0; u < GV_U; ++u) {
        const int c = wave + 4 * u;
        if (c < nchunks) {
#pragma unroll
            for (int t = 0; t < NT; ++t) {
                wbuf[u][t][0] = ld8_nt(wp[t] + c * 64);
                wbuf[u][t][1] = ld8_nt(wp[t] + c * 64 + 8);
// ... 192 lines not shown
```

karanta_ocr_amd/engine.py:

```python
from __future__ import annotations

import ctypes as C
import math
import os
import time
from dataclasses import dataclass, field
from typing import Any, Dict, List, Optional, Sequence, Tuple

import numpy as np
import torch

from . import image_processing as IP
from . import positions as POS
from ._lib import (ADJ_CAP, DEC_ARGMAX, DEC_OUT_XP, DEC_PLAIN, DEC_ROPE_KV, DEC_SILU8, Dec32, EPI_GELU_ERF, EPI_NONE, EPI_QUICK_GELU, EPI_SILU_MUL8,
                   KarantaHipError, lib, narrow_opts, ptr)
from .config import ModelConfig
from .sampling import StepFeatures, adjust_table, has_penalties, needs_processing, sampling_params, temperature
from .weights import pack_w16x64, to_bf16_bits

BF16 = torch.bfloat16
GEMM_SCRATCH_BYTES = 512 * 65536
FP8_ACT_DEFAULT = False
SEQUENCE_SWITCHES = ("KARANTA_NARROW", "KARANTA_NARROW_O", "KARANTA_DEFER_DOWN", "KARANTA_WIDE", "KARANTA_ATOMIC_SLAB", "KARANTA_DEC32")


def _bits(w: np.ndarray) -> np.ndarray:
    return w if w.dtype == np.uint16 else to_bf16_bits(np.asarray(w, dtype=np.float32))


def _align(n: int, a: int = 256) -> int:
    return (n + a - 1) // a * a


class DeviceWeights:

    def __init__(self, cfg: ModelConfig, device: torch.device, weight_dtype: str = "bf16"):
        if weight_dtype not in ("bf16", "fp8"):
            raise ValueError(f"weight_dtype {weight_dtype!r} (bf16 or fp8)")
        self.cfg = cfg
        self.device = device
        self.weight_dtype = weight_dtype
        self.layout: Dict[str, Tuple[int, Tuple[int, ...]]] = {}
        self.nbytes = 0
        self.arena: Optional[torch.Tensor] = None
        self._plan()

    def _add(self, name: str, shape: Tuple[int, ...], itemsize: int = 2):
        self.layout[name] = (self.nbytes, tuple(shape))
        self.nbytes = _align(self.nbytes + itemsize * int(np.prod(shape)))

    def _plan(self):
        v, t = self.cfg.vision, self.cfg.text
        self._add("vit.patch", (v.embed_dim, v.patch_dim_padded))
        v25 = v.variant == "qwen2_5"
        for i in range(v.depth):
            p = f"vit.{i}."
            self._add(p + "ln1.w", (v.embed_dim,))
            self._add(p + "qkv.w", (3 * v.embed_dim, v.embed_dim)); self._add(p + "qkv.b", (3 * v.embed_dim,))
            self._add(p + "proj.w", (v.embed_dim, v.embed_dim)); self._add(p + "proj.b", (v.embed_dim,))
            self._add(p + "ln2.w", (v.embed_dim,))
            if v25:
                fp = v.mlp_dim_padded
                self._add(p + "gate_up.w", (2 * fp, v.embed_dim)); self._add(p + "gate_up.b", (2 * fp,))
                self._add(p + "down.w", (v.embed_dim, fp)); self._add(p + "down.b", (v.embed_dim,))
            else:
                self._add(p + "ln1.b", (v.embed_dim,)); self._add(p + "ln2.b", (v.embed_dim,))
                self._add(p + "fc1.w", (v.mlp_dim, v.embed_dim)); self._add(p + "fc1.b", (v.mlp_dim,))
                self._add(p + "fc2.w", (v.embed_dim, v.mlp_dim)); self._add(p + "fc2.b", (v.embed_dim,))
        self._add("vit.merger.ln.w", (v.embed_dim,))
        if not v25:
            self._add("vit.merger.ln.b", (v.embed_dim,))
        self._add("vit.merger.fc1.w", (v.merge_dim, v.merge_dim)); self._add("vit.merger.fc1.b", (v.merge_dim,))
        self._add("vit.merger.fc2.w", (v.hidden_size, v.merge_dim)); self._add("vit.merger.fc2.b", (v.hidden_size,))
        self._add("llm.embed", (t.vocab_size, t.hidden_size))
        for i in range(t.num_layers):
            p = f"llm.{i}."
            self._add(p + "ln1.w", (t.hidden_size,))
            self._add(p + "qkv.w", (t.qkv_dim, t.hidden_size)); self._add(p + "qkv.b", (t.qkv_dim,))
            self._add(p + "o.w", (t.hidden_size, t.q_dim))
            self._add(p + "ln2.w", (t.hidden_size,))
            self._add(p + "gate_up.w", (2 * t.intermediate_size, t.hidden_size))
            self._add(p + "down.w", (t.hidden_size, t.intermediate_size))
            if self.weight_dtype == "fp8":
                for n, shape in (("qkv", (t.qkv_dim, t.hidden_size)), ("o", (t.hidden_size, t.q_dim)),
                                 ("gate_up", (2 * t.intermediate_size, t.hidden_size)), ("down", (t.hidden_size, t.intermediate_size))):
                    self._add(p + n + ".w8", shape, itemsize=1)
                    self._add(p + n + ".s", (shape[0],), itemsize=4)
        self._add("llm.norm.w", (t.hidden_size,))
        self._add("llm.lm_head", (t.vocab_size, t.hidden_size))

    def allocate(self):
        self.arena = torch.zeros(self.nbytes, dtype=torch.uint8, device=self.device)

    def view(self, name: str) -> torch.Tensor:
        off, shape = self.layout[name]
        n = int(np.prod(shape))
        return self.arena[off:off + 2 * n].view(BF16).view(*shape)

    def view_u8(self, name: str) -> torch.Tensor:
        off, shape = self.layout[name]
        return self.arena[off:off + int(np.prod(shape))].view(*shape)

    def view_f32(self, name: str) -> torch.Tensor:
        off, shape = self.layout[name]
        return self.arena[off:off + 4 * int(np.prod(shape))].view(torch.float32).view(*shape)

    def has(self, name: str) -> bool:
        return name in self.layout

    def _put(self, name: str, bits: np.ndarray):
        off, shape = self.layout[name]
        assert tuple(bits.shape) == shape, (name, bits.shape, shape)
        src = torch.from_numpy(np.ascontiguousarray(bits).view(np.uint8).reshape(-1))
        self.arena[off:off + src.numel()].copy_(src, non_blocking=False)

    def load(self, w: Dict[str, np.ndarray]):
        if self.arena is None:
            self.allocate()
        v, t = self.cfg.vision, self.cfg.text
        V, Lm = "model.visual.", "model.language_model."
        pe = _bits(w[V + "patch_embed.proj.weight"]).reshape(v.embed_dim, -1)
        pad = np.zeros((v.embed_dim, v.patch_dim_padded), np.uint16)
        pad[:, :pe.shape[1]] = pe
        self._put("vit.patch", pad)
        v25 = v.variant == "qwen2_5"
        for i in range(v.depth):
            s, d = f"{V}blocks.{i}.", f"vit.{i}."
            names = [("norm1.weight", "ln1.w"), ("attn.qkv.weight", "qkv.w"), ("attn.qkv.bias", "qkv.b"),
                     ("attn.proj.weight", "proj.w"), ("attn.proj.bias", "proj.b"), ("norm2.weight", "ln2.w")]
            if not v25:
                names += [("norm1.bias", "ln1.b"), ("norm2.bias", "ln2.b"), ("mlp.fc1.weight", "fc1.w"),
                          ("mlp.fc1.bias", "fc1.b"), ("mlp.fc2.weight", "fc2.w"), ("mlp.fc2.bias", "fc2.b")]
            for a, b in names:
                self._put(d + b, _bits(w[s + a]))
            if v25:
                ffv, fp, D = v.mlp_dim, v.mlp_dim_padded, v.embed_dim
                def padded(a, rows):
                    out = np.zeros((rows,) + a.shape[1:], np.uint16)
                    out[:a.shape[0]] = a
                    return out
                g = padded(_bits(w[s + "mlp.gate_proj.weight"]), fp).reshape(fp // 8, 8, D)
                u = padded(_bits(w[s + "mlp.up_proj.weight"]), fp).reshape(fp // 8, 8, D)
                self._put(d + "gate_up.w", np.stack([g, u], 1).reshape(2 * fp, D))
                gb = padded(_bits(w[s + "mlp.gate_proj.bias"]), fp).reshape(fp // 8, 8)
                ub = padded(_bits(w[s + "mlp.up_proj.bias"]), fp).reshape(fp // 8, 8)
                self._put(d + "gate_up.b", np.stack([gb, ub], 1).reshape(2 * fp))
                dw = np.zeros((D, fp), np.uint16)
                dw[:, :ffv] = _bits(w[s + "mlp.down_proj.weight"])
                self._put(d + "down.w", dw)
                self._put(d + "down.b", _bits(w[s + "mlp.down_proj.bias"]))
        merger = [("merger.ln_q.weight", "ln.w"), ("merger.mlp.0.weight", "fc1.w"), ("merger.mlp.0.bias", "fc1.b"),
                  ("merger.mlp.2.weight", "fc2.w"), ("merger.mlp.2.bias", "fc2.b")]
        if not v25:
            merger.append(("merger.ln_q.bias", "ln.b"))
        for a, b in merger:
            self._put("vit.merger." + b, _bits(w[V + a]))
        self._put("llm.embed", _bits(w[Lm + "embed_tokens.weight"]))
        ff = t.intermediate_size
        if ff % 8:
            raise KarantaHipError(f"intermediate_size {ff} must be a multiple of 8")
        fp8 = self.weight_dtype == "fp8"
        for i in range(t.num_layers):
            s, d = f"{Lm}layers.{i}.", f"llm.{i}."
            self._put(d + "ln1.w", _bits(w[s + "input_layernorm.weight"]))
            self._put(d + "ln2.w", _bits(w[s + "post_attention_layernorm.weight"]))
            self._put(d + "qkv.b", np.concatenate([_bits(w[s + f"self_attn.{n}_proj.bias"]) for n in "qkv"], 0))
            if fp8:
                from .weights import as_f32, fp8_e4m3_to_f32, pack_w16x64_fp8, quantize_fp8_rows
                qs = {n: quantize_fp8_rows(as_f32(w[s + n + ".weight"])) for n in
                      ("self_attn.q_proj", "self_attn.k_proj", "self_attn.v_proj", "self_attn.o_proj", "mlp.gate_proj",
                       "mlp.up_proj", "mlp.down_proj")}
                il = lambda a, b: np.stack([a.reshape((ff // 8, 8) + a.shape[1:]), b.reshape((ff // 8, 8) + b.shape[1:])], 1) \
                    .reshape((2 * ff,) + a.shape[1:])
                fused = {"qkv": tuple(np.concatenate([qs[f"self_attn.{n}_proj"][k] for n in "qkv"], 0) for k in (0, 1)),
                         "o": qs["self_attn.o_proj"],
                         "gate_up": (il(qs["mlp.gate_proj"][0], qs["mlp.up_proj"][0]), il(qs["mlp.gate_proj"][1], qs["mlp.up_proj"][1])),
                         "down": qs["mlp.down_proj"]}
                for n, (q, sc) in fused.items():
                    off8, _ = self.layout[d + n + ".w8"]
                    src = torch.from_numpy(np.ascontiguousarray(pack_w16x64_fp8(q)).reshape(-1))
                    self.arena[off8:off8 + src.numel()].copy_(src, non_blocking=False)
                    offs, _ = self.layout[d + n + ".s"]
                    srcs = torch.from_numpy(np.ascontiguousarray(sc, np.float32).view(np.uint8).reshape(-1))
                    self.arena[offs:offs + srcs.numel()].copy_(srcs, non_blocking=False)
                    self._put(d + n + ".w", pack_w16x64(to_bf16_bits(fp8_e4m3_to_f32(q) * sc[:, None])))
                continue
            self._put(d + "qkv.w", pack_w16x64(np.concatenate([_bits(w[s + f"self_attn.{n}_proj.weight"]) for n in "qkv"], 0)))
            self._put(d + "o.w", pack_w16x64(_bits(w[s + "self_attn.o_proj.weight"])))
            g = _bits(w[s + "mlp.gate_proj.weight"]).reshape(ff // 8, 8, -1)
            u = _bits(w[s + "mlp.up_proj.weight"]).reshape(ff // 8, 8, -1)
            self._put(d + "gate_up.w", pack_w16x64(np.stack([g, u], 1).reshape(2 * ff, -1)))
            self._put(d + "down.w", pack_w16x64(_bits(w[s + "mlp.down_proj.weight"])))
        self._put("llm.norm.w", _bits(w[Lm + "norm.weight"]))
        head = w[Lm + "embed_tokens.weight"] if (t.tie_word_embeddings or "lm_head.weight" not in w) else w["lm_head.weight"]
        self._put("llm.lm_head", pack_w16x64(_bits(head)))
        torch.cuda.synchronize(self.device)


@dataclass
class PageRequest:
    input_ids: np.ndarray
    pixel_values: Optional[np.ndarray] = None
    grids: List[Tuple[int, int, int]] = field(default_factory=list)
    temperature: float = 0.0
    seed: int = 0
    images: Optional[List[Any]] = None
    guide: Any = None
    logprobs: Optional[int] = None
    top_k: int = 0
    top_p: float = 1.0
    min_p: float = 0.0
    repetition_penalty: float = 1.0
    frequency_penalty: float = 0.0
    presence_penalty: float = 0.0
    logit_bias: Optional[Dict[int, float]] = None
    min_tokens: int = 0
    stop_token_ids: Tuple[int, ...] = ()


@dataclass
class GenerateResult:
    tokens: List[np.ndarray]
    finish_reasons: List[str]
    prompt_tokens: List[int]
    timings: Dict[str, float]
    logits: Optional[np.ndarray] = None
    logprobs: Optional[List[Optional[Dict[str, np.ndarray]]]] = None


class DeviceGuide:

    def __init__(self, guide, trans: torch.Tensor, masks: torch.Tensor):
        self.guide, self.trans, self.masks = guide, trans, masks
        self.start = int(guide.start)


@dataclass
class DevicePlan:
    host: POS.AttnPlan
    blk_tok0: torch.Tensor
    blk_ntok: torch.Tensor
    blk_kr: torch.Tensor
    blk_vb: torch.Tensor
    qblk: torch.Tensor
    qlen: torch.Tensor
    n_blk: int


def device_plan(plan: POS.AttnPlan, dev: torch.device) -> DevicePlan:
    t_ = lambda a: torch.from_numpy(np.ascontiguousarray(a)).to(dev)
    return DevicePlan(plan, t_(plan.blk_tok0), t_(plan.blk_ntok), t_(plan.blk_k_row0), t_(plan.blk_vt_blk), t_(plan.qblk),
                      t_(plan.qblk_len), len(plan.blk_tok0))


@dataclass
class VitTables:
    cos: torch.Tensor
    sin: torch.Tensor
    full: DevicePlan
    perm: Optional[torch.Tensor] = None
    inv: Optional[torch.Tensor] = None
    win: Optional[DevicePlan] = None


@dataclass
class Admission:
    B: int
    slots: List[int]
    whole_batch: bool
    lens: List[int]
    M: int
    src: np.ndarray
    cos: np.ndarray
    sin: np.ndarray
    deltas: np.ndarray
    plan: POS.AttnPlan
    last_rows: np.ndarray
    cs: np.ndarray
    n_img: int
    temps: Optional[np.ndarray] = None
    seeds: Optional[np.ndarray] = None
    guides: Optional[list] = None
    procs: Optional[list] = None
    adjs: Optional[list] = None
    need: StepFeatures = StepFeatures()


class Engine:
    def __init__(self, cfg: ModelConfig, device: str = "cuda:0", max_batch: int = 8, s_max: int = 4096,
                 max_patches: int = 8 * 5476, max_prompt_tokens: int = 8 * 2048, decode_splits: int = 16,
                 weight_dtype: str = "bf16", fp8_activations: Optional[bool] = None, admission_cus: Optional[int] = None):
        if not torch.cuda.is_available():
            raise KarantaHipError("no HIP device: the karanta MI355X engine has no CPU fallback")
        self.L = lib()
        self.cfg = cfg
        self.device = torch.device(device)
        torch.cuda.set_device(self.device)
        self.stream = torch.cuda.Stream(device=self.device)
        self.s = self.stream.cuda_stream
        self.B = max_batch
        if max_batch > 32:
            raise KarantaHipError("max_batch > 32: the decode kernels take at most two 16-row column tiles")
        self.s_max = _align(s_max, 64)
        self.max_patches = max_patches
        self.max_tokens = max_prompt_tokens
        self.n_split = decode_splits
        self._ignore_eos = self._freeze_finished = self._want_logits = False
        self._caps = self._step = StepFeatures()
        self._logprobs = None
        self._adm_stream = None
        env_cus = os.environ.get("KARANTA_ADMIT_CUS")
        self.admission_cus = int(env_cus) if env_cus is not None else (int(admission_cus) if admission_cus else 0)
        self._adm_stream_handle = None
        self.disjoint_decode = os.environ.get("KARANTA_DISJOINT_DECODE", "1") != "0"
        self._dec_stream, self._dec_stream_handle, self._adm_inflight = None, None, 0
        self.n_cus = int(torch.cuda.get_device_properties(self.device).multi_processor_count)
        self._resample_cache: Dict[tuple, tuple] = {}
        self.persist_blocks = int(os.environ.get("KARANTA_PERSIST_BLOCKS", "512"))
        if type(self) is Engine and any(os.environ.get(k, "0") not in ("", "0") for k in
                                        ("KARANTA_PREFETCH", "KARANTA_FAST_RESIDUAL", "KARANTA_ATTN_FUSED", "KARANTA_MERGE_IN_OPROJ")):
            raise KarantaHipError("KARANTA_PREFETCH / KARANTA_FAST_RESIDUAL / KARANTA_ATTN_FUSED / KARANTA_MERGE_IN_OPROJ are decode "
                                  "experiments: they run on csrc/tools/experiment_engine.ExperimentEngine with a -DKR_EXPERIMENTS "
                                  "library (csrc/tools/build_variant.py, KARANTA_HIP_LIB), not on the product engine")
        if os.environ.get("KARANTA_RESNORM32_QKV", "1") != "1":
            raise KarantaHipError("KARANTA_RESNORM32_QKV is retired: the packed family with the fused row-major qkv launch was "
                                  "measured and dropped (profiles/r04_decode32_chains.txt)")
        moved = [k for k in SEQUENCE_SWITCHES if os.environ.get(k, "1") != "1"] + [k for k in ("KARANTA_RESNORM_QKV",) if k in os.environ]
        if type(self) is Engine and moved:
            raise KarantaHipError(" / ".join(moved) + ": superseded decode launch sequences run on csrc/tools/experiment_engine."
                                  "ExperimentEngine (csrc/tools/decode_ab.py builds it for such a variant), not on the product engine")
        v, t = cfg.vision, cfg.text
        if v.head_dim not in (80, 128) or t.head_dim != 128:
            raise KarantaHipError(f"unsupported head dims vit={v.head_dim} llm={t.head_dim}")
        self.w = DeviceWeights(cfg, self.device, weight_dtype)
        self.fp8 = weight_dtype == "fp8"
        self.fp8_prefill_gemm = os.environ.get("KARANTA_FP8_PREFILL", "1") == "1"
        env = os.environ.get("KARANTA_FP8_ACT")
        self.fp8_act = self.fp8 and self.fp8_prefill_gemm and (bool(fp8_activations) if fp8_activations is not None
                                                              else (env == "1" if env is not None else FP8_ACT_DEFAULT))
        self._graphs: Dict[Tuple[int, bool], int] = {}
        self._prof_on = False
        self._prof_events: List[Tuple[C.c_void_p, C.c_void_p]] = []
        self._prof_next = 0
        self._last_batch = max_batch
        self._alloc()

    def _alloc(self):
        v, t, dev = self.cfg.vision, self.cfg.text, self.device
        N, M, B = self.max_patches, self.max_tokens, self.B
        z = lambda *shape, dtype=BF16: torch.zeros(*shape, dtype=dtype, device=dev)
        nvb = N // 64 + 64
        if v.variant == "qwen2_5":
            per_win = (v.window_merge_units * v.spatial_merge_size) ** 2
            nvb = max(nvb, 2 * (N // max(1, min(64, per_win))) + 64)
        self.v_pix = z(N, v.patch_dim, dtype=torch.float32)
        self.v_in = z(N, v.patch_dim_padded)
        self.v_x = z(N, v.embed_dim)
        self.v_h = z(N, v.embed_dim)
        self.v_qkv = z(N, 3 * v.embed_dim)
        self.v_q = z(v.num_heads, N, v.head_dim)
        self.v_k = z(v.num_heads, N, v.head_dim)
        self.v_vt = z(v.num_heads, nvb, v.head_dim, 64)
        self.v_o = z(N, v.embed_dim)
        self.v_f = z(N, v.mlp_dim_padded)
        self.v_perm = None
        self.v_m1 = z(N // 4 + 1, v.merge_dim)
        self._vit_cache = {}
        self._vit_rot_cache = {}
        self.img_embeds = z(N // 4 + 1, t.hidden_size)
        self.p_x = z(M, t.hidden_size)
        self.p_h = z(M, t.hidden_size)
        self.p_qkv = z(M, t.qkv_dim)
        self.p_q = z(t.num_heads, M, t.head_dim)
        self.p_o = z(M, t.q_dim)
        self.p_act = z(M, t.intermediate_size)
        self.p_cos = z(M, t.head_dim, dtype=torch.float32)
        self.p_sin = z(M, t.head_dim, dtype=torch.float32)
        self.p_src = z(M, dtype=torch.int32)
        if self.fp8_act:
            self.p_a8 = z(M, (max(t.intermediate_size, t.hidden_size, t.q_dim) + 15) // 16 * 16, dtype=torch.uint8)
            self.p_as = z(M, dtype=torch.float32)
        self.gemm_scratch = z(GEMM_SCRATCH_BYTES // 4, dtype=torch.float32)
        self.kcache = z(t.num_layers, B, t.num_kv_heads, self.s_max, t.head_dim)
        self.vtcache = z(t.num_layers, B, t.num_kv_heads, self.s_max // 64, t.head_dim, 64)
        self.d_x = z(B, t.hidden_size)
        self.d_x2 = z(B, t.hidden_size)
        self.d_part = z(4 if B > 16 else 2, B, t.hidden_size, dtype=torch.float32)
        if t.hidden_size // 16 >= 192:
            self.down_waves_small = 8
        self.d_qkv = z(B, t.qkv_dim)
        Bp = 32 if B > 16 else B
        self.d_h = z(Bp, t.hidden_size)
        self.d_q = z(B, t.num_heads, t.head_dim)
        self.d_o = z(Bp, t.q_dim)
        self.d_act = z(Bp, t.intermediate_size)
        self.d_logits = z(B, t.vocab_size, dtype=torch.float32)
        self.d_ws = z(B * t.num_heads * self.n_split * (t.head_dim + 4), dtype=torch.float32)
        self.wv_qkv = self._waves(t.hidden_size // 64)
        self.wv_o = self._waves(t.q_dim // 64)
        self.wv_down = self._waves(t.intermediate_size // 64)
        self.wv_wide = 4
        for name in ("qkv", "o", "down", "wide"):
            v_ = os.environ.get("KARANTA_WV_" + name.upper())
            if v_:
                setattr(self, "wv_" + name, int(v_))
        self.defer_down = t.hidden_size in (1536, 2048, 3584)
        self.wide_mode = t.hidden_size % 512 == 0 and t.hidden_size <= 4096
        self.wide_blocks = int(os.environ.get("KARANTA_WIDE_BLOCKS", "256"))
        self.wide_waves = int(os.environ.get("KARANTA_WIDE_WAVES", "0"))
        self.wide_spread32 = os.environ.get("KARANTA_WIDE_SPREAD32", "1") == "1"
        if self.B > 16 and not (self.wide_mode and t.intermediate_size % 64 == 0):
            raise KarantaHipError("max_batch > 16 needs the wide / narrow decode kernels (hidden_size % 512 == 0) and hidden_size <= 2048 or == 3584")
        self.row_split = self.B > 16 and t.hidden_size > 2048
        self.family32, self.resnorm_qkv = self.B > 16, self.row_split
        self.group_split_down = int(os.environ.get("KARANTA_DOWN_GS", "1"))
        if self.row_split and t.hidden_size != 3584:
            raise KarantaHipError("max_batch > 16: hidden_size <= 2048 or == 3584 (the 7B width) only")
        if self.fp8 and not self.wide_mode:
            raise KarantaHipError("fp8 weights need the wide / narrow decode kernels: hidden_size % 512 == 0 and <= 4096")
        self.n_amax = (max(self._amax_parts(0), self._amax_parts(32)) if self.wide_mode
                       else (t.vocab_size // 16 + 1) // 2)
        self.d_amax_v = z(B, self.n_amax, dtype=torch.float32)
        self.d_amax_i = z(B, self.n_amax, dtype=torch.int32)
        self.d_plen = z(B, dtype=torch.int32)
        self.d_cs = None
        self.d_ctx = z(B, dtype=torch.int32)
        self.d_delta = z(B, dtype=torch.int32)
        self.d_tok = z(B, dtype=torch.int32)
        self.d_fin = z(B, dtype=torch.int32)
        self._snap_ring, self._snap_next, self._snap_event, self._copy_stream = None, 0, None, None
        self.d_temp = z(B, dtype=torch.float32)
        self.d_seed = z(B, dtype=torch.int32)
        self.d_gtrans = z(B, dtype=torch.int64)
        self.d_gmasks = z(B, dtype=torch.int64)
        self.d_gstate = z(B, dtype=torch.int32)
        self.mask_words = 2 * ((t.vocab_size + 63) // 64)
        self.d_sp = torch.tensor(np.tile(sampling_params(PageRequest(np.zeros(0, np.int64))), (B, 1)), device=dev)
        self.d_counts = z(B, t.vocab_size, dtype=torch.int32)
        self.bits_words = (t.vocab_size + 31) // 32
        self.d_pbits = z(B, self.bits_words, dtype=torch.int32)
        self.d_work = z(B, t.vocab_size, dtype=torch.float32)
        self.d_thr = z(B, dtype=torch.int32)
        self.d_live = z(B, dtype=torch.int32)
        self.d_adj_ids = z(B, ADJ_CAP, dtype=torch.int32)
        self.d_adj_val = z(B, ADJ_CAP, dtype=torch.float32)
        self.d_adj_flag = z(B, ADJ_CAP, dtype=torch.int32)
        self.d_adj_meta = z(B, 4, dtype=torch.int32)
        self.d_adj_saved = z(B, ADJ_CAP, dtype=torch.float32)
        self.d_voc_off = self.d_voc_bytes = None
        self._guides: Dict[str, DeviceGuide] = {}
        self._slot_guides: Dict[int, DeviceGuide] = {}
        self.lp_part = max(64 if t.vocab_size > 4096 else 1, -(-t.vocab_size // 4096))
        self.d_lp = self.d_lpi = None
        self.d_lp_pv = z(B, self.lp_part, 20, dtype=torch.float32)
        self.d_lp_pi = z(B, self.lp_part, 20, dtype=torch.int32)
        self.d_lp_ms = z(B, self.lp_part, 2, dtype=torch.float32)
        self.max_new = 0
        self._req_max_new = 0
        self.d_hist = None
        self.d_eos = torch.tensor(list(self.cfg.eos_token_ids), dtype=torch.int32, device=dev)
        self.d_invfreq = torch.from_numpy(POS.rope_inv_freq(t.head_dim, t.rope_theta)).to(dev)
        self.d_last = z(B, dtype=torch.int32)
        torch.cuda.synchronize(dev)

    @staticmethod
    def _waves(nchunks: int) -> int:
        return 16 if nchunks >= 64 else 8 if nchunks >= 16 else 4

    def load_weights(self, weights: Dict[str, np.ndarray]):
        self.w.load(weights)

    def _gemm(self, A, W, C_, M, bias=None, res=None, epi=EPI_NONE, packed=False, w8=None, w_scale=None):
        N, K = W.shape
        if w8 is not None and self.fp8_act:
            ldq = self.p_a8.stride(0)
            self.L.kr_quantize_rows_fp8(ptr(A), A.stride(0), ptr(self.p_a8), ldq, ptr(self.p_as), M, K, self.s)
            self.L.kr_gemm_fp8a(ptr(self.p_a8), ldq, ptr(self.p_as), ptr(w8), ptr(w_scale), ptr(bias), ptr(res),
                                res.stride(0) if res is not None else 0, ptr(C_), C_.stride(0), M, N, K, epi, self.s)
            return
        if w8 is not None and self.fp8_prefill_gemm:
            self.L.kr_gemm_fp8(ptr(A), A.stride(0), ptr(w8), ptr(w_scale), ptr(bias), ptr(res),
                               res.stride(0) if res is not None else 0, ptr(C_), C_.stride(0), M, N, K, epi, self.s)
            return
        self.L.kr_gemm_bf16_ws(ptr(A), A.stride(0), ptr(W), ptr(bias), ptr(res), res.stride(0) if res is not None else 0,
                               ptr(C_), C_.stride(0), M, N, K, epi, 1 if packed else 0, ptr(self.gemm_scratch),
                               self.gemm_scratch.numel() * 4, self.s)

    def _dec(self, mode, x, W, M, out=None, out_f32=None, norm_w=None, waves=4):
        t = self.cfg.text
        N, K = W.shape
        o = out if out is not None else out_f32
        self.L.kr_linear_decode(mode, ptr(x), x.stride(0), ptr(W), 0, ptr(norm_w), t.rms_norm_eps, 0, 0, ptr(out), ptr(out_f32),
                                o.stride(0) if o is not None else 0, M, N, K, waves, self.persist_blocks, 1, 0, 0,
                                0, self.n_split, ptr(self.d_cs), self.max_new, ptr(self.d_plen),
                                ptr(self.d_ctx), ptr(self.d_q), 0, 0, t.num_heads, t.num_kv_heads, self.s_max,
                                ptr(self.d_amax_v), ptr(self.d_amax_i), self.s)

    def _dec_narrow(self, mode, x, W, M, out=None, out_f32=None, bias=None, norm_w=None, res=None, waves=8, ksplit=1,
                    part_in=None, x_out=None, kc=0, vc=0, w8=None, w_scale=None, zero=None, atomic_out=False):
        t = self.cfg.text
        N, K = W.shape
        o = out if out is not None else out_f32
        head = (mode, ptr(x), x.stride(0), ptr(part_in), int(part_in.shape[0]) if part_in is not None else 0, ptr(x_out),
                x_out.stride(0) if x_out is not None else 0)
        args = (ptr(bias), ptr(norm_w), t.rms_norm_eps, ptr(res), res.stride(0) if res is not None else 0, ptr(out),
                ptr(out_f32), o.stride(-2) if o is not None else 0, M, N, K, waves, ksplit, ptr(self.d_cs), self.max_new,
                ptr(self.d_plen), ptr(self.d_ctx), ptr(self.d_q), kc, vc, t.num_heads, t.num_kv_heads, self.s_max,
                narrow_opts(ptr(zero), zero.numel() * 4 if zero is not None else 0, atomic_out), self.s)
        if w8 is not None:
            self.L.kr_linear_decode_narrow_fp8(*head, ptr(w8), ptr(w_scale), *args)
        else:
            self.L.kr_linear_decode_narrow(*head, ptr(W), *args)

    def _dec32(self, mode, xp, W, M, waves_ref, out=None, out_f32=None, bias=None, res=None, ksplit=1, atomic_out=False, zero=None,
               kc=0, vc=0, w8=None, w_scale=None, tiles_per_wg=0, group_split=False):
        t = self.cfg.text
        N, K = W.shape
        o = out if out is not None else out_f32
        a = Dec32(ptr(xp), ptr(w8 if w8 is not None else W), ptr(w_scale), ptr(bias), ptr(res), res.stride(0) if res is not None else 0,
                  ptr(out), ptr(out_f32), o.stride(-2) if o is not None else 0, M, N, K, waves_ref, ksplit, 1 if atomic_out else 0,
                  tiles_per_wg, 1 if group_split else 0, 0, ptr(zero) if zero is not None else None,
                  zero.numel() * 4 if zero is not None else 0,
                  ptr(self.d_cs), self.max_new, ptr(self.d_plen), ptr(self.d_ctx), ptr(self.d_q), kc or None, vc or None,
                  t.num_heads, t.num_kv_heads, self.s_max)
        self.L.kr_linear_decode32(mode, C.byref(a), self.s)
# ... 37 lines not shown
            self.L.kr_linear_decode_wide(mode, ptr(x), x.stride(0), ptr(W), *tail)

    def _h2d(self, dst: torch.Tensor, arr: np.ndarray):
        src = torch.from_numpy(np.ascontiguousarray(arr))
        dst.view(-1)[:src.numel()].copy_(src.view(-1), non_blocking=False)

    def _vit_tables(self, grids) -> VitTables:
        key = tuple(tuple(int(x) for x in g) for g in grids)
        hit = self._vit_cache.get(key)
        if hit is None:
            v, dev = self.cfg.vision, self.device
            t_ = lambda a: torch.from_numpy(np.ascontiguousarray(a)).to(dev)
            per_img = []
            for g in key:
                hit_i = self._vit_rot_cache.get(g)
                if hit_i is None:
                    c_i, s_i = POS.vision_rotary_tables((g,), v.head_dim, v.spatial_merge_size)
                    hit_i = (t_(c_i), t_(s_i))
                    if len(self._vit_rot_cache) > 64:
                        self._vit_rot_cache.clear()
                    self._vit_rot_cache[g] = hit_i
                per_img.append(hit_i)
            cos = per_img[0][0] if len(per_img) == 1 else torch.cat([c for c, _ in per_img])
            sin = per_img[0][1] if len(per_img) == 1 else torch.cat([s_ for _, s_ in per_img])
            hit = VitTables(cos, sin, device_plan(POS.vit_attn_plan(key), dev))
            if v.variant == "qwen2_5":
                unit = v.spatial_merge_size ** 2
                order, win_lens = POS.vision_window_order(key, v.spatial_merge_size, v.window_size, v.patch_size)
                perm = (order[:, None] * unit + np.arange(unit)[None, :]).reshape(-1)
                perm_long = t_(perm.astype(np.int64))
                hit.cos, hit.sin = cos.index_select(0, perm_long), sin.index_select(0, perm_long)
                hit.perm, hit.inv = t_(perm.astype(np.int32)), t_(np.argsort(order).astype(np.int32))
                hit.win = device_plan(POS.segments_attn_plan(win_lens), dev)
            if len(self._vit_cache) > 16:
                self._vit_cache.clear()
            self._vit_cache[key] = hit
        return hit

    def patches_from_images(self, images: Sequence[np.ndarray], min_pixels: int = IP.MIN_PIXELS,
                            max_pixels: int = IP.MAX_PIXELS_CLASS_DEFAULT,
                            grids: Optional[Sequence[Sequence[int]]] = None):
        v, L, s, dev = self.cfg.vision, self.L, self.s, self.device
        unit = v.patch_size * v.spatial_merge_size
        metas, total = [], 0
        if grids is not None and len(grids) != len(images):
            raise KarantaHipError(f"{len(images)} images but {len(grids)} grids")
        for k, im in enumerate(images):
            if isinstance(im, torch.Tensor):
                if im.dtype != torch.uint8 or im.dim() != 3 or im.shape[2] != 3 or not im.is_contiguous():
                    raise KarantaHipError("device images must be contiguous HWC uint8 RGB tensors")
            else:
                im = np.asarray(im)
                if im.ndim == 2:
                    im = np.stack([im] * 3, axis=-1)
                if im.dtype != np.uint8 or im.ndim != 3 or im.shape[2] != 3:
                    raise KarantaHipError("images must be HWC uint8 RGB arrays")
                im = np.ascontiguousarray(im)
            h, w = int(im.shape[0]), int(im.shape[1])
            if grids is not None:
                g = [int(x) for x in grids[k]]
                if g[0] != 1 or g[1] % v.spatial_merge_size or g[2] % v.spatial_merge_size or min(g[1:]) < 1:
                    raise KarantaHipError(f"image grid {tuple(g)} is not (1, even, even)")
                rh, rw = g[1] * v.patch_size, g[2] * v.patch_size
            else:
                rh, rw = IP.smart_resize(h, w, unit, min_pixels, max_pixels)
            metas.append((im, h, w, rh, rw))
            total += (rh // v.patch_size) * (rw // v.patch_size)
        out = torch.empty(total, v.patch_dim, dtype=torch.float32, device=dev)
        mean = (C.c_float * 3)(*[float(x) for x in IP.CLIP_MEAN])
        std = (C.c_float * 3)(*[float(x) for x in IP.CLIP_STD])
        grids, off = [], 0
        with torch.cuda.stream(self.stream):
            for im, h, w, rh, rw in metas:
                if isinstance(im, torch.Tensor):
                    src = im if im.device == dev else im.to(dev)
                else:
                    src = torch.from_numpy(im if im.flags.writeable else im.copy()).to(dev)
                key = (h, w, rh, rw)
                tabs = self._resample_cache.get(key)
                if tabs is None:
                    t_ = lambda a: torch.from_numpy(np.ascontiguousarray(a)).to(dev)
                    hb, hk = IP.resample_tables(w, rw) if rw != w else (None, None)
                    vb, vk = IP.resample_tables(h, rh) if rh != h else (None, None)
                    tabs = tuple(None if a is None else t_(a) for a in (hb, hk, vb, vk))
                    if len(self._resample_cache) > 64:
                        self._resample_cache.clear()
                    self._resample_cache[key] = tabs
                hb, hk, vb, vk = tabs
                dst = torch.empty(rh, rw, 3, dtype=torch.uint8, device=dev)
                tmp = torch.empty(h, rw, 3, dtype=torch.uint8, device=dev) if (rw != w and rh != h) else None
                L.kr_image_resize_bicubic_u8(ptr(src), h, w, ptr(dst), rh, rw, ptr(tmp), ptr(hb), ptr(hk),
                                             hk.shape[1] if hk is not None else 0, ptr(vb), ptr(vk),
                                             vk.shape[1] if vk is not None else 0, s)
                n = (rh // v.patch_size) * (rw // v.patch_size)
                L.kr_image_normalize_patchify(ptr(dst), rh, rw, mean, std, v.patch_size, v.spatial_merge_size,
                                              v.temporal_patch_size, ptr(out[off:]), s)
                grids.append((1, rh // v.patch_size, rw // v.patch_size))
                off += n
        return out, grids

    def _pixels_for(self, pages: Sequence[PageRequest], pixel_values_device):
        if pixel_values_device is not None:
            return pixel_values_device
        with_images = [p for p in pages if p.images]
        if with_images:
            if any(p.pixel_values is not None and len(p.pixel_values) for p in pages):
                raise KarantaHipError("a batch mixes pages with `images` and pages with `pixel_values`")
            for p in pages:
                if len(p.images or []) != len(p.grids):
                    raise KarantaHipError(f"a page has {len(p.images or [])} images but {len(p.grids)} grids")
            pix, _ = self.patches_from_images([im for p in pages for im in (p.images or [])],
                                              grids=[g for p in pages for g in p.grids])
            return pix
        pvs = [p.pixel_values for p in pages if p.pixel_values is not None and len(p.pixel_values)]
        if not pvs:
            return None
        return np.concatenate(pvs, 0) if len(pvs) > 1 else pvs[0]

    def vit_forward(self, pixel_values, grids: Sequence[Sequence[int]]) -> torch.Tensor:
        v, L, s, w = self.cfg.vision, self.L, self.s, self.w
        n = int(pixel_values.shape[0])
        if n == 0:
            return self.img_embeds[:0]
        if n > self.max_patches:
            raise KarantaHipError(f"{n} patches > max_patches {self.max_patches}")
        with torch.cuda.stream(self.stream):
            tab = self._vit_tables(grids)
            assert tab.full.host.n_tokens == n, (tab.full.host.n_tokens, n)
            if isinstance(pixel_values, torch.Tensor):
                pix = pixel_values
                if pix.dtype != torch.float32 or not pix.is_cuda or not pix.is_contiguous():
                    raise KarantaHipError("device pixel_values must be a contiguous fp32 CUDA tensor")
            else:
                self._h2d(self.v_pix, np.asarray(pixel_values, dtype=np.float32))
                pix = self.v_pix
            D, H, hd, d_out = v.embed_dim, v.num_heads, v.head_dim, self.cfg.text.hidden_size
            x, h = self.v_x, self.v_h
            L.kr_cast_pad_f32_bf16(ptr(pix), ptr(self.v_in), n, v.patch_dim, v.patch_dim_padded, s)
            self._gemm(self.v_in, w.view("vit.patch"), x, n)
            if max(pl.host.n_vt_blocks for pl in (tab.full, tab.win) if pl is not None) > self.v_vt.shape[1]:
                raise KarantaHipError("too many image segments for the V^T buffer")
            v25 = v.variant == "qwen2_5"
            if v25:
                L.kr_embed_scatter(ptr(tab.perm), ptr(x), 0, ptr(h), n, D, s)
                x, h = h, x
                norm = lambda name: L.kr_rmsnorm(ptr(x), D, ptr(w.view(name + ".w")), ptr(h), n, D, 1e-6, s)
                up, down, epi = "gate_up", "down", EPI_SILU_MUL8
            else:
                norm = lambda name: L.kr_layernorm(ptr(x), ptr(w.view(name + ".w")), ptr(w.view(name + ".b")), ptr(h), n, D, 1e-6, s)
                up, down, epi = "fc1", "fc2", EPI_QUICK_GELU
            for i in range(v.depth):
                p = f"vit.{i}."
                norm(p + "ln1")
                self._gemm(h, w.view(p + "qkv.w"), self.v_qkv, n, bias=w.view(p + "qkv.b"))
                self._attention(self.v_qkv, D, 2 * D, tab.cos, tab.sin, tab.win if v25 and i not in v.fullatt_block_indexes else tab.full,
                                self.v_q, self.v_k, self.v_k.stride(0), self.v_vt, self.v_vt.stride(0), self.v_o, H, H, hd, causal=False)
                self._gemm(self.v_o, w.view(p + "proj.w"), x, n, bias=w.view(p + "proj.b"), res=x)
                norm(p + "ln2")
                self._gemm(h, w.view(p + up + ".w"), self.v_f, n, bias=w.view(p + up + ".b"), epi=epi)
                self._gemm(self.v_f, w.view(p + down + ".w"), x, n, bias=w.view(p + down + ".b"), res=x)
            norm("vit.merger.ln")
            T = n // (v.spatial_merge_size ** 2)
            merged_in = h.view(-1)[: T * v.merge_dim].view(T, v.merge_dim)
            self._gemm(merged_in, w.view("vit.merger.fc1.w"), self.v_m1, T, bias=w.view("vit.merger.fc1.b"), epi=EPI_GELU_ERF)
            out = self.v_o.view(-1)[: T * d_out].view(T, d_out) if v25 else self.img_embeds
            self._gemm(self.v_m1, w.view("vit.merger.fc2.w"), out, T, bias=w.view("vit.merger.fc2.b"))
            if v25:
                L.kr_embed_scatter(ptr(tab.inv), ptr(out), 0, ptr(self.img_embeds), T, d_out, s)
        return self.img_embeds[:T]

    def _attention(self, qkv, k_off, v_off, cos, sin, dp: DevicePlan, q, k, k_stride, vt, vt_stride, out, H, KVH, hd, causal):
        L, s = self.L, self.s
        L.kr_qkv_prep(ptr(qkv), qkv.shape[1], 0, k_off, v_off, ptr(cos), ptr(sin),
                      ptr(dp.blk_tok0), ptr(dp.blk_ntok), ptr(dp.blk_kr), ptr(dp.blk_vb), dp.n_blk,
                      ptr(q), q.stride(0), ptr(k), k_stride, ptr(vt), vt_stride, H, KVH, hd, s)
        L.kr_attn_varlen_q(ptr(q), ptr(k), ptr(vt), ptr(out), ptr(dp.qblk), ptr(dp.qlen), dp.host.qblk.shape[0], q.shape[1],
                           H, KVH, hd, k_stride, vt_stride, hd ** -0.5, 1 if causal else 0, dp.host.q_block, s)

    def set_vocab(self, token_bytes: Sequence[bytes]):
        from .guided import pack_vocab
        V = self.cfg.text.vocab_size
        tb = list(token_bytes)[:V] + [b""] * max(0, V - len(token_bytes))
        off, flat = pack_vocab(tb)
        self.d_voc_off = torch.from_numpy(off).to(self.device)
        self.d_voc_bytes = torch.from_numpy(flat).to(self.device)
        self._guides.clear()

    def compile_guide(self, guide) -> DeviceGuide:
        from .guided import Guide, compile_regex
        if isinstance(guide, DeviceGuide):
            return guide
        if isinstance(guide, str):
            hit = self._guides.get(guide)
            if hit is not None:
                return hit
            guide = compile_regex(guide)
        if not isinstance(guide, Guide):
            raise KarantaHipError(f"not a guide: {type(guide).__name__}")
        if guide.pattern and guide.pattern in self._guides:
            return self._guides[guide.pattern]
        if self.d_voc_off is None:
            raise KarantaHipError("guided decoding needs the vocabulary's byte strings: call Engine.set_vocab() first")
        S = guide.n_states
        trans = torch.from_numpy(np.ascontiguousarray(guide.trans).view(np.int16)).to(self.device)
        accept = torch.from_numpy(np.ascontiguousarray(guide.accept).astype(np.uint8)).to(self.device)
        masks = torch.empty(S, self.mask_words, dtype=torch.int32, device=self.device)
        torch.cuda.current_stream(self.device).synchronize()
        with torch.cuda.stream(self.stream):
            self.L.kr_guide_build_masks(ptr(trans), ptr(accept), S, ptr(self.d_voc_off), ptr(self.d_voc_bytes),
                                        self.cfg.text.vocab_size, ptr(self.d_eos), self.d_eos.numel(), ptr(masks),
                                        self.mask_words, self.s)
        self.stream.synchronize()
        dg = DeviceGuide(guide, trans, masks)
        if guide.pattern:
            if len(self._guides) >= 64:
                self._guides.pop(next(iter(self._guides)))
            self._guides[guide.pattern] = dg
        return dg

    def _guide_rows(self, pages):
        rows = []
        for p in pages:
            g = getattr(p, "guide", None)
            if g is None:
                rows.append((0, 0, 0, None))
                continue
            dg = self.compile_guide(g)
            rows.append((dg.trans.data_ptr(), dg.masks.data_ptr(), dg.start, dg))
        return rows

    def _ensure_history(self, max_new_tokens: int):
        grow = self.d_hist is None or self.max_new < max_new_tokens
        if grow:
            self.max_new = max_new_tokens
            self.d_hist = torch.zeros(max_new_tokens + 1, self.B, dtype=torch.int32, device=self.device)
            self.d_cs = torch.zeros(self.B, max_new_tokens, self.cfg.text.head_dim, dtype=torch.float32, device=self.device)
        if self._logprobs is not None and (self.d_lp is None or self.d_lp.shape[0] < self.max_new + 1):
            self.d_lp = torch.zeros(self.max_new + 1, self.B, 21, dtype=torch.float32, device=self.device)
            self.d_lpi = torch.zeros(self.max_new + 1, self.B, 20, dtype=torch.int32, device=self.device)
            grow = True
        if grow:
            for g in self._graphs.values():
                self.L.kr_graph_destroy(g)
            self._graphs.clear()

    def seq_room(self) -> int:
        return self.s_max - (1 if self._freeze_finished else 0)

    def _prefill_prepare(self, pages: Sequence[PageRequest], n_image_tokens_total: int, slots: Optional[Sequence[int]] = None,
                         budgets: Optional[Sequence[int]] = None) -> Admission:
        cfg, t = self.cfg, self.cfg.text
        B = len(pages)
        whole_batch = slots is None
        slots = list(range(B)) if whole_batch else [int(j) for j in slots]
        if len(slots) != B or len(set(slots)) != B or min(slots) < 0 or max(slots) >= self.B:
            raise KarantaHipError(f"slots {slots} do not name {B} distinct slots below {self.B}")
        lens = [int(len(p.input_ids)) for p in pages]
        M = sum(lens)
        if M > self.max_tokens:
            raise KarantaHipError(f"{M} prompt tokens > max_prompt_tokens {self.max_tokens}")
        if budgets is None:
            budgets = [self._req_max_new] * B
        if len(budgets) != B or max(budgets) > self.max_new:
            raise KarantaHipError(f"budgets {list(budgets)} do not fit {B} pages / the history of {self.max_new} tokens")
        self._check_budgets(pages, budgets)
        src = np.empty(M, np.int32)
        cos = np.empty((M, t.head_dim), np.float32)
        sin = np.empty((M, t.head_dim), np.float32)
        deltas = np.zeros(self.B, np.int32)
        off, img_off = 0, 0
        for b, pg in enumerate(pages):
            ids = np.asarray(pg.input_ids).reshape(-1)
            is_img = ids == cfg.image_token_id
            k = int(is_img.sum())
            row = ids.astype(np.int64).copy()
            row[is_img] = -(np.arange(img_off, img_off + k) + 1)
            if row.max(initial=0) >= t.vocab_size:
                raise KarantaHipError("token id out of vocabulary")
            src[off:off + len(ids)] = row
            pos3, delta = POS.rope_index_one(ids, pg.grids, cfg.image_token_id, cfg.vision.spatial_merge_size)
            c, sn = POS.mrope_tables(pos3, t.head_dim, t.rope_theta, t.mrope_section)
            cos[off:off + len(ids)], sin[off:off + len(ids)] = c, sn
            deltas[b] = delta
            off += len(ids)
            img_off += k
        if img_off != n_image_tokens_total:
            raise KarantaHipError(f"Image features and image tokens do not match, tokens: {img_off}, "
                                  f"features: {n_image_tokens_total}")
        plan = POS.prefill_attn_plan(lens, slots, t.num_kv_heads, self.s_max)
        last_rows = (np.cumsum(lens) - 1).astype(np.int32)
        kk = np.arange(self.max_new, dtype=np.int64)
        cs = np.zeros((B, self.max_new, t.head_dim), np.float32)
        for b in range(B):
            p1 = lens[b] + kk + int(deltas[b])
            c_, s_ = POS.mrope_tables(np.stack([p1, p1, p1]), t.head_dim, t.rope_theta, t.mrope_section)
            cs[b, :, : t.head_dim // 2], cs[b, :, t.head_dim // 2:] = c_[:, : t.head_dim // 2], s_[:, : t.head_dim // 2]
        return Admission(B, slots, whole_batch, lens, M, src, cos, sin, deltas, plan, last_rows, cs, n_image_tokens_total)

    def _vit_and_prepare(self, pages: Sequence[PageRequest], pixel_values_device=None, slots: Optional[Sequence[int]] = None,
                         budgets: Optional[Sequence[int]] = None) -> Admission:
        pix = self._pixels_for(pages, pixel_values_device)
        n_img_tok = self.vit_forward(pix, [g for p in pages for g in p.grids]).shape[0] if pix is not None else 0
        return self._prefill_prepare(pages, n_img_tok, slots, budgets)

    def prefill(self, pages: Sequence[PageRequest], n_image_tokens_total: int, slots: Optional[Sequence[int]] = None,
                defer_activation: bool = False, adm: Optional[Admission] = None) -> Admission:
        t, L, s, w = self.cfg.text, self.L, self.s, self.w
        if adm is None or adm.n_img != n_image_tokens_total:
            adm = self._prefill_prepare(pages, n_image_tokens_total, slots)
        adm.need = self._admit_features(pages)
        M, d = adm.M, t.hidden_size
        with torch.cuda.stream(self.stream):
            self._h2d(self.p_src, adm.src)
            self._h2d(self.p_cos, adm.cos)
            self._h2d(self.p_sin, adm.sin)
            adm.temps = np.asarray([temperature(p) for p in pages], np.float32)
            adm.seeds = np.asarray([int(getattr(p, "seed", 0) or 0) & 0xFFFFFFFF for p in pages], np.uint32).view(np.int32)
            adm.guides = self._guide_rows(pages)
            adm.procs = self._control_rows(pages)
            adm.adjs = self._adjust_rows(pages)
            if not defer_activation:
                self._write_state(adm)
            self._h2d(self.d_last, adm.last_rows)
            dp = device_plan(adm.plan, self.device)
            L.kr_embed_scatter(ptr(self.p_src), ptr(w.view("llm.embed")), ptr(self.img_embeds), ptr(self.p_x), M, d, s)
            for i in range(t.num_layers):
                p = f"llm.{i}."
                L.kr_rmsnorm(ptr(self.p_x), d, ptr(w.view(p + "ln1.w")), ptr(self.p_h), M, d, t.rms_norm_eps, s)
                self._gemm(self.p_h, w.view(p + "qkv.w"), self.p_qkv, M, bias=w.view(p + "qkv.b"), packed=True, **self._w8kw(p + "qkv.w"))
                kc, vc = self.kcache[i], self.vtcache[i]
                self._attention(self.p_qkv, t.q_dim, t.q_dim + t.kv_dim, self.p_cos, self.p_sin, dp, self.p_q, kc, kc.stride(1),
                                vc, vc.stride(1), self.p_o, t.num_heads, t.num_kv_heads, t.head_dim, causal=True)
                self._gemm(self.p_o, w.view(p + "o.w"), self.p_x, M, res=self.p_x, packed=True, **self._w8kw(p + "o.w"))
                L.kr_rmsnorm(ptr(self.p_x), d, ptr(w.view(p + "ln2.w")), ptr(self.p_h), M, d, t.rms_norm_eps, s)
                self._gemm(self.p_h, w.view(p + "gate_up.w"), self.p_act, M, epi=EPI_SILU_MUL8, packed=True, **self._w8kw(p + "gate_up.w"))
                self._gemm(self.p_act, w.view(p + "down.w"), self.p_x, M, res=self.p_x, packed=True, **self._w8kw(p + "down.w"))
            if not defer_activation:
                self._first_tokens(adm)
        return adm

    def _admit_features(self, pages) -> StepFeatures:
        need, caps = StepFeatures.of(pages), self._caps
        if need.guided and not caps.guided:
            raise KarantaHipError("a page carries a guide but the engine is not in its guided configuration "
                                  "(generate() decides from its pages; begin_slots(guided=True) for slot mode)")
        if need.adjust and not caps.adjust:
            raise KarantaHipError("a page asks for logit_bias / min_tokens / stop_token_ids but the engine is in its greedy "
                                  "configuration (generate() decides from its pages; begin_slots(sampling=True) for slot mode)")
        if need.sampling and not caps.sampling:
            raise KarantaHipError("a page asks for temperature > 0 but the engine is in its greedy configuration "
                                  "(generate() decides from its pages; begin_slots(sampling=True) for slot mode)")
        if need.processing and not caps.processing:
            raise KarantaHipError("a page asks for top_k / top_p / min_p / penalties but the engine is in its greedy "
                                  "configuration (generate() decides from its pages; begin_slots(sampling=True) for slot mode)")
        self._step |= need
        return need

    def _control_rows(self, pages):
        if not self._caps.processing:
            return None
        V, rows = self.cfg.text.vocab_size, []
        for p in pages:
            sp, nd = sampling_params(p), needs_processing(p)
            bits = None
            if nd and sp[3] != 1.0:
                ids = np.asarray(p.input_ids, np.int64).reshape(-1)
                ids = ids[(ids >= 0) & (ids < V)]
                bits = np.zeros(self.bits_words, np.uint32)
                np.bitwise_or.at(bits, ids >> 5, (np.uint32(1) << (ids & 31).astype(np.uint32)))
            rows.append((sp, bits, nd))
        return rows

    def _adjust_rows(self, pages):
        if not self._caps.adjust:
            return None
        try:
            return [adjust_table(p, self.cfg.eos_token_ids, self.cfg.text.vocab_size) for p in pages]
        except ValueError as e:
            raise KarantaHipError(str(e)) from e

    def _write_state(self, a: Admission):
        gt, gm, gs, dgs = zip(*a.guides)
        lens = np.asarray(a.lens, np.int32)
        sampler = ((self.d_temp, a.temps), (self.d_seed, a.seeds))
        fields = ((self.d_gtrans, np.asarray(gt, np.int64)), (self.d_gmasks, np.asarray(gm, np.int64)),
                  (self.d_gstate, np.asarray(gs, np.int32)), (self.d_delta, a.deltas),
                  (self.d_ctx, lens - 1), (self.d_plen, lens))
        if a.whole_batch:
            for dst, rows in sampler + fields:
                padded = np.zeros(self.B, rows.dtype)
                padded[:a.B] = rows[:a.B]
                self._h2d(dst, padded)
            self._h2d(self.d_cs, a.cs)
            self.d_fin.zero_()
            self._slot_guides = {b: dg for b, dg in enumerate(dgs) if dg is not None}
        else:
            for b, j in enumerate(a.slots):
                for dst, rows in fields:
                    self._h2d(dst[j:j + 1], rows[b:b + 1])
                self._h2d(self.d_cs[j], a.cs[b])
                for dst, rows in sampler:
                    self._h2d(dst[j:j + 1], rows[b:b + 1])
                self.d_fin[j:j + 1].zero_()
                self._slot_guides.pop(j, None)
                if dgs[b] is not None:
                    self._slot_guides[j] = dgs[b]
        for (sp, bits, nd), j in zip(a.procs or (), a.slots):
            self._h2d(self.d_sp[j], sp)
            if bits is not None:
                self._h2d(self.d_pbits[j], bits.view(np.int32))
            if nd:
                self.d_counts[j].zero_()
        if a.adjs is not None and a.whole_batch:
            self.d_adj_meta.zero_()
        for tab, j in zip(a.adjs or (), a.slots):
            if tab is None:
                if not a.whole_batch:
                    self.d_adj_meta[j].zero_()
                continue
            for dst, rows in zip((self.d_adj_ids, self.d_adj_val, self.d_adj_flag, self.d_adj_meta), tab):
                self._h2d(dst[j], rows)

    def _first_tokens(self, a: Admission):
        d = self.cfg.text.hidden_size
        for b, j, n in ((0, 0, a.B),) if a.whole_batch else ((b, j, 1) for b, j in enumerate(a.slots)):
            self.L.kr_embed_scatter(ptr(self.d_last[b:]), ptr(self.p_x), 0, ptr(self.d_x[j:]), n, d, self.s)
            self._lm_head_and_sample(n, slot0=j)

    def _lm_head_and_sample(self, B: int, x=None, slot0: int = 0):
        t, L, w, s = self.cfg.text, self.L, self.w, self.s
        x = self.d_x if x is None else x
        j = slot0
        step = self._step
        logits = self.d_logits[j:] if (self._want_logits or step.sampling or step.processing or self._logprobs is not None) else None
        if self.wide_mode:
            self._dec_wide(DEC_ARGMAX, x[j:], w.view("llm.lm_head"), B, norm_w=w.view("llm.norm.w"), out_f32=logits)
        else:
            self._dec(DEC_ARGMAX, x[j:], w.view("llm.lm_head"), B, norm_w=w.view("llm.norm.w"), out_f32=logits,
                      waves=self.wv_wide)
        n_part = self._amax_parts(B) if self.wide_mode else self.n_amax
        flags = (1 if self._ignore_eos else 0) | (2 if self._freeze_finished else 0)
        gm, gs = (ptr(self.d_gmasks[j:]), ptr(self.d_gstate[j:])) if step.guided else (None, None)
        if step.adjust:
            adj = (ptr(self.d_adj_ids[j:]), ptr(self.d_adj_val[j:]), ptr(self.d_adj_flag[j:]), ptr(self.d_adj_meta[j:]))
            L.kr_logits_adjust(ptr(logits), self.d_logits.stride(0), t.vocab_size, *adj, ptr(self.d_ctx[j:]), ptr(self.d_plen[j:]),
                               ptr(self.d_adj_saved[j:]), B, s)
        if step.processing:
            n_part = min(64, n_part)
            V, ld = t.vocab_size, self.d_logits.stride(0)
            L.kr_sample_threshold(ptr(logits), ld, V, ptr(self.d_temp[j:]), ptr(self.d_sp[j:]), ptr(self.d_counts[j:]), V,
                                  ptr(self.d_pbits[j:]), self.bits_words, gm, gs, self.mask_words, ptr(self.d_fin[j:]), flags,
                                  ptr(self.d_work[j:]), V, ptr(self.d_thr[j:]), ptr(self.d_live[j:]), B, s)
            L.kr_gumbel_argmax_processed(ptr(logits), ld, V, ptr(self.d_temp[j:]), ptr(self.d_seed[j:]), ptr(self.d_ctx[j:]),
                                         ptr(self.d_plen[j:]), ptr(self.d_amax_v), ptr(self.d_amax_i), n_part, B, gm, gs,
                                         self.mask_words, int(self.cfg.eos_token_ids[0]), ptr(self.d_sp[j:]),
                                         ptr(self.d_counts[j:]), V, ptr(self.d_pbits[j:]), self.bits_words, ptr(self.d_thr[j:]), s)
        elif step.sampling:
            n_part = min(64, n_part)
            mw, fb = (self.mask_words, int(self.cfg.eos_token_ids[0])) if step.guided else (0, 0)
            L.kr_gumbel_argmax_guided(ptr(logits), self.d_logits.stride(0), t.vocab_size, ptr(self.d_temp[j:]), ptr(self.d_seed[j:]),
                                      ptr(self.d_ctx[j:]), ptr(self.d_plen[j:]), ptr(self.d_amax_v), ptr(self.d_amax_i), n_part, B,
                                      gm, gs, mw, fb, s)
        L.kr_sample_greedy(ptr(self.d_amax_v), ptr(self.d_amax_i), n_part, ptr(w.view("llm.embed")), t.hidden_size,
                           ptr(self.d_tok[j:]), ptr(self.d_hist[:, j:]), self.d_hist.stride(0), ptr(self.d_plen[j:]),
                           ptr(self.d_ctx[j:]), ptr(self.d_fin[j:]), ptr(self.d_eos), self.d_eos.numel(),
                           self.cfg.pad_token_id, flags, ptr(self.d_x[j:]), B, s)
        if step.adjust:
            L.kr_stop_tokens(ptr(self.d_tok[j:]), adj[0], adj[2], adj[3], ptr(self.d_fin[j:]), flags, B, s)
        if step.processing:
            L.kr_sample_count(ptr(self.d_tok[j:]), ptr(self.d_live[j:]), ptr(self.d_counts[j:]), t.vocab_size, t.vocab_size, B, s)
        if step.guided:
            L.kr_guide_advance(ptr(self.d_tok[j:]), ptr(self.d_fin[j:]), ptr(self.d_gtrans[j:]), ptr(self.d_gstate[j:]),
                               ptr(self.d_voc_off), ptr(self.d_voc_bytes), t.vocab_size, B, s)
        if step.adjust:
            L.kr_logits_restore(ptr(logits), self.d_logits.stride(0), t.vocab_size, adj[0], adj[3], ptr(self.d_adj_saved[j:]), B, s)
        if self._logprobs is not None:
            L.kr_logprobs_topk(ptr(logits), self.d_logits.stride(0), t.vocab_size, int(self._logprobs), self.lp_part,
                               ptr(self.d_lp_pv), ptr(self.d_lp_pi), ptr(self.d_lp_ms), ptr(self.d_tok[j:]), ptr(self.d_ctx[j:]),
                               ptr(self.d_plen[j:]), ptr(self.d_fin[j:]), ptr(self.d_lp[:, j:]), ptr(self.d_lpi[:, j:]),
                               self.d_lp.shape[0], self.B, 20, B, s)

    def _decode_step_launches(self, B: int):
        t, L, w, s = self.cfg.text, self.L, self.w, self.s
        H, KVH, hd = t.num_heads, t.num_kv_heads, t.head_dim
        nl = t.num_layers
# ... 433 lines not shown
```

karanta_ocr_amd/positions.py:

```python
from __future__ import annotations

from dataclasses import dataclass
from typing import Optional, List, Sequence, Tuple

import numpy as np

from .weights import bf16_round

F32 = np.float32


def vision_position_ids(grid_thw: Sequence[Sequence[int]], merge: int = 2) -> np.ndarray:
    out = []
    for t, h, w in grid_thw:
        hh = np.arange(h)[:, None].repeat(w, 1)
        ww = np.arange(w)[None, :].repeat(h, 0)
        shp = (h // merge, merge, w // merge, merge)
        hh = hh.reshape(shp).transpose(0, 2, 1, 3).reshape(-1)
        ww = ww.reshape(shp).transpose(0, 2, 1, 3).reshape(-1)
        out.append(np.tile(np.stack([hh, ww], -1), (t, 1)))
    return np.concatenate(out, 0).astype(np.int64) if out else np.zeros((0, 2), np.int64)


def vision_rotary_tables(grid_thw: Sequence[Sequence[int]], head_dim: int, merge: int = 2,
                         theta: float = 10000.0) -> Tuple[np.ndarray, np.ndarray]:
    pos = vision_position_ids(grid_thw, merge)
    dim = head_dim // 2
    inv = (1.0 / (float(theta) ** (np.arange(0, dim, 2, dtype=np.float64) / dim))).astype(F32)
    fr = (pos[:, :, None].astype(F32) * inv[None, None, :]).reshape(pos.shape[0], -1)
    emb = np.concatenate([fr, fr], -1)
    return np.cos(emb).astype(F32), np.sin(emb).astype(F32)


def rope_index_one(input_ids: np.ndarray, grids: Sequence[Sequence[int]], image_token_id: int,
                   merge: int = 2) -> Tuple[np.ndarray, int]:
    ids = np.asarray(input_ids).reshape(-1)
    p = ids.shape[0]
    is_img = ids == image_token_id
    change = np.flatnonzero(np.diff(is_img.astype(np.int8))) + 1
    starts = np.concatenate([[0], change])
    ends = np.concatenate([change, [p]])
    cols: List[np.ndarray] = []
    cur = 0
    gi = 0
    for a, b in zip(starts, ends):
        n = int(b - a)
        if not is_img[a]:
            cols.append(np.tile(np.arange(n, dtype=np.int64)[None, :] + cur, (3, 1)))
            cur += n
        else:
            if gi >= len(grids):
                raise ValueError("more image-token runs than image grids")
            t, gh, gw = (int(v) for v in grids[gi])
            gi += 1
            lh, lw = gh // merge, gw // merge
            if t * lh * lw != n:
                raise ValueError(f"Image features and image tokens do not match, tokens: {n}, features: {t * lh * lw}")
            tt = np.repeat(np.arange(t, dtype=np.int64), lh * lw) + cur
            hh = np.tile(np.repeat(np.arange(lh, dtype=np.int64), lw), t) + cur
            ww = np.tile(np.arange(lw, dtype=np.int64), t * lh) + cur
            cols.append(np.stack([tt, hh, ww], 0))
            cur += max(gh, gw) // merge
    if gi != len(grids):
        raise ValueError("fewer image-token runs than image grids")
    pos = np.concatenate(cols, 1) if cols else np.zeros((3, 0), np.int64)
    delta = int(pos.max()) + 1 - p if p else 0
    return pos, delta


def mrope_tables(pos3: np.ndarray, head_dim: int, theta: float, mrope_section: Sequence[int],
                 round_bf16: bool = True) -> Tuple[np.ndarray, np.ndarray]:
    inv = (1.0 / (float(theta) ** (np.arange(0, head_dim, 2, dtype=np.float64) / head_dim))).astype(F32)
    fr = pos3[..., None].astype(F32) * inv
    sel = np.concatenate([np.full(s, i % 3) for i, s in enumerate(mrope_section)])
    ang = np.take_along_axis(fr, sel[None, None, :].repeat(fr.shape[1], 1), axis=0)[0]
    emb = np.concatenate([ang, ang], -1)
    cos, sin = np.cos(emb).astype(F32), np.sin(emb).astype(F32)
    if round_bf16:
        cos, sin = bf16_round(cos), bf16_round(sin)
    return cos, sin


def rope_inv_freq(head_dim: int, theta: float) -> np.ndarray:
    return (1.0 / (float(theta) ** (np.arange(0, head_dim, 2, dtype=np.float64) / head_dim))).astype(F32)


@dataclass
class AttnPlan:
    blk_tok0: np.ndarray
    blk_ntok: np.ndarray
    blk_k_row0: np.ndarray
    blk_vt_blk: np.ndarray
    qblk: np.ndarray
    qblk_len: np.ndarray
    n_tokens: int
    n_vt_blocks: int
    q_block: int = 128


def pick_q_block(lens: Sequence[int], causal: bool = False) -> int:
    lens = [int(n) for n in lens if int(n) > 0]
    return 256 if (not causal) and lens and sum(lens) / len(lens) >= 2048 else 128


def make_attn_plan(lens: Sequence[int], k_row0: Sequence[int], vt_blk0: Sequence[int], causal: bool,
                   q_block: Optional[int] = None) -> AttnPlan:
    if q_block is None:
        q_block = pick_q_block(lens, causal)
    if q_block not in (128, 256):
        raise ValueError(f"q_block {q_block} (128 or 256)")
    blk_tok0, blk_ntok, blk_kr, blk_vb, qblk, qlen = [], [], [], [], [], []
    tok = 0
    nvb = 0
    for s, n in enumerate(lens):
        n = int(n)
        for j in range(0, n, 64):
            blk_tok0.append(tok + j)
            blk_ntok.append(min(64, n - j))
            blk_kr.append(int(k_row0[s]) + j)
            blk_vb.append(int(vt_blk0[s]) + j // 64)
        for j in range(0, n, q_block):
            nq = min(q_block, n - j)
            qblk.append((tok + j, nq, int(k_row0[s]), int(vt_blk0[s])))
            qlen.append((n, j))
        tok += n
        nvb += (n + 63) // 64
    work = [min(n, j + nq) if causal else n for (_, nq, _, _), (n, j) in zip(qblk, qlen)]
    order = sorted(range(len(qblk)), key=lambda i: -((work[i] + 63) // 64))
    qblk = [qblk[i] for i in order]
    qlen = [qlen[i] for i in order]
    return AttnPlan(
        np.asarray(blk_tok0, np.int32), np.asarray(blk_ntok, np.int32), np.asarray(blk_kr, np.int64),
        np.asarray(blk_vb, np.int64), np.asarray(qblk, np.int32).reshape(-1, 4),
        np.asarray(qlen, np.int32).reshape(-1, 2), tok, nvb, q_block)


def vit_attn_plan(grid_thw: Sequence[Sequence[int]]) -> AttnPlan:
    lens = [int(t * h * w) for t, h, w in grid_thw]
    k_row0 = np.concatenate([[0], np.cumsum(lens)[:-1]]) if lens else []
    nb = [(n + 63) // 64 for n in lens]
    vt0 = np.concatenate([[0], np.cumsum(nb)[:-1]]) if lens else []
    return make_attn_plan(lens, k_row0, vt0, causal=False)


def vision_window_order(grid_thw: Sequence[Sequence[int]], merge: int, window_size: int, patch_size: int):
    ws = window_size // merge // patch_size
    if ws < 1:
        raise ValueError(f"window_size {window_size} is smaller than one merged unit")
    order: List[np.ndarray] = []
    win_lens: List[int] = []
    base = 0
    for t, h, w in grid_thw:
        lh, lw = int(h) // merge, int(w) // merge
        ids = np.arange(int(t) * lh * lw, dtype=np.int64).reshape(int(t), lh, lw)
        for ti in range(int(t)):
            for y0 in range(0, lh, ws):
                for x0 in range(0, lw, ws):
                    blk = ids[ti, y0:y0 + ws, x0:x0 + ws].reshape(-1)
                    order.append(blk + base)
                    win_lens.append(int(blk.size) * merge * merge)
        base += int(t) * lh * lw
    return (np.concatenate(order) if order else np.zeros(0, np.int64)), win_lens


def segments_attn_plan(lens: Sequence[int]) -> AttnPlan:
    lens = [int(n) for n in lens]
    k_row0 = np.concatenate([[0], np.cumsum(lens)[:-1]]) if lens else []
    nb = [(n + 63) // 64 for n in lens]
    vt0 = np.concatenate([[0], np.cumsum(nb)[:-1]]) if lens else []
    return make_attn_plan(lens, k_row0, vt0, causal=False)


def prefill_attn_plan(prompt_lens: Sequence[int], slots: Sequence[int], kv_heads: int, s_max: int) -> AttnPlan:
    k_row0 = [int(sl) * kv_heads * s_max for sl in slots]
    vt0 = [int(sl) * kv_heads * (s_max // 64) for sl in slots]
    return make_attn_plan(prompt_lens, k_row0, vt0, causal=True)


def vt_blocks(v_rows: np.ndarray) -> np.ndarray:
    v_rows = np.asarray(v_rows)
    *lead, S, hd = v_rows.shape
    a = np.swapaxes(v_rows.reshape(*lead, S // 64, 2, 32, hd), -1, -2)
    return np.ascontiguousarray(a).reshape(*lead, S // 64, hd, 64)


def vt_rows(vt: np.ndarray) -> np.ndarray:
    vt = np.asarray(vt)
    *lead, nb, hd, _ = vt.shape
    a = np.swapaxes(vt.reshape(*lead, nb, 2, hd, 32), -1, -2)
    return np.ascontiguousarray(a).reshape(*lead, nb * 64, hd)
```

karanta_ocr_amd/weights.py:

```python
from __future__ import annotations

import json
import os
from typing import Dict, Iterable, Optional

import numpy as np

from .config import ModelConfig, from_hf_config_dict



def bf16_round(x: np.ndarray) -> np.ndarray:
    x = np.ascontiguousarray(x, dtype=np.float32)
    u = x.view(np.uint32)
    r = ((u >> 16) & 1) + np.uint32(0x7FFF)
    out = ((u + r) & np.uint32(0xFFFF0000)).view(np.float32)
    return np.where(np.isnan(x), x, out)


def to_bf16_bits(x: np.ndarray) -> np.ndarray:
    x = np.ascontiguousarray(x, dtype=np.float32)
    u = x.view(np.uint32)
    r = ((u >> 16) & 1) + np.uint32(0x7FFF)
    return ((u + r) >> 16).astype(np.uint16)
# ... 21 lines not shown
            s[p + "norm2.bias"] = (v.embed_dim,)
        s[p + "attn.qkv.weight"] = (3 * v.embed_dim, v.embed_dim)
        s[p + "attn.qkv.bias"] = (3 * v.embed_dim,)
        s[p + "attn.proj.weight"] = (v.embed_dim, v.embed_dim)
        s[p + "attn.proj.bias"] = (v.embed_dim,)
        if v25:
            for n in ("gate_proj", "up_proj"):
                s[p + f"mlp.{n}.weight"] = (v.mlp_dim, v.embed_dim)
                s[p + f"mlp.{n}.bias"] = (v.mlp_dim,)
            s[p + "mlp.down_proj.weight"] = (v.embed_dim, v.mlp_dim)
            s[p + "mlp.down_proj.bias"] = (v.embed_dim,)
        else:
            s[p + "mlp.fc1.weight"] = (v.mlp_dim, v.embed_dim)
            s[p + "mlp.fc1.bias"] = (v.mlp_dim,)
            s[p + "mlp.fc2.weight"] = (v.embed_dim, v.mlp_dim)
            s[p + "mlp.fc2.bias"] = (v.embed_dim,)
    s["model.visual.merger.ln_q.weight"] = (v.embed_dim,)
    if not v25:
        s["model.visual.merger.ln_q.bias"] = (v.embed_dim,)
    s["model.visual.merger.mlp.0.weight"] = (v.merge_dim, v.merge_dim)
    s["model.visual.merger.mlp.0.bias"] = (v.merge_dim,)
    s["model.visual.merger.mlp.2.weight"] = (v.hidden_size, v.merge_dim)
    s["model.visual.merger.mlp.2.bias"] = (v.hidden_size,)
    s["model.language_model.embed_tokens.weight"] = (t.vocab_size, t.hidden_size)
    for i in range(t.num_layers):
        p = f"model.language_model.layers.{i}."
        s[p + "self_attn.q_proj.weight"] = (t.q_dim, t.hidden_size)
        s[p + "self_attn.q_proj.bias"] = (t.q_dim,)
        s[p + "self_attn.k_proj.weight"] = (t.kv_dim, t.hidden_size)
        s[p + "self_attn.k_proj.bias"] = (t.kv_dim,)
        s[p + "self_attn.v_proj.weight"] = (t.kv_dim, t.hidden_size)
        s[p + "self_attn.v_proj.bias"] = (t.kv_dim,)
        s[p + "self_attn.o_proj.weight"] = (t.hidden_size, t.q_dim)
        s[p + "mlp.gate_proj.weight"] = (t.intermediate_size, t.hidden_size)
        s[p + "mlp.up_proj.weight"] = (t.intermediate_size, t.hidden_size)
        s[p + "mlp.down_proj.weight"] = (t.hidden_size, t.intermediate_size)
        s[p + "input_layernorm.weight"] = (t.hidden_size,)
        s[p + "post_attention_layernorm.weight"] = (t.hidden_size,)
    s["model.language_model.norm.weight"] = (t.hidden_size,)
    if not t.tie_word_embeddings:
        s["lm_head.weight"] = (t.vocab_size, t.hidden_size)
    return s


def _random_tensor(shapes, seed: int, idx: int, as_bits: bool) -> np.ndarray:
    name, shape = shapes[idx]
    rng = np.random.default_rng([seed, idx])
    n = int(np.prod(shape))
    if name.endswith("bias"):
        w = rng.standard_normal(n, dtype=np.float32) * np.float32(0.02)
    elif len(shape) == 1:
        w = np.float32(1.0) + rng.standard_normal(n, dtype=np.float32) * np.float32(0.1)
    elif "embed_tokens" in name:
        w = rng.standard_normal(n, dtype=np.float32) * np.float32(0.5)
    else:
        fan_in = int(np.prod(shape[1:]))
        w = rng.standard_normal(n, dtype=np.float32) * np.float32(1.0 / np.sqrt(fan_in))
    w = w.reshape(shape)
    return to_bf16_bits(w) if as_bits else bf16_round(w)


def random_weights(cfg: ModelConfig, seed: int = 0, as_bits: bool = False, threads: Optional[int] = None,
                   only: Optional[Iterable[str]] = None) -> Dict[str, np.ndarray]:
    shapes = list(weight_shapes(cfg).items())
    if only is not None:
        want = set(only)
        return {shapes[i][0]: _random_tensor(shapes, seed, i, as_bits) for i in range(len(shapes)) if shapes[i][0] in want}

    def one(idx: int) -> np.ndarray:
        return _random_tensor(shapes, seed, idx, as_bits)

    total = sum(int(np.prod(sh)) for _, sh in shapes)
    if threads is None:
        threads = min(8, os.cpu_count() or 1) if total > (1 << 26) else 1
    if threads <= 1:
        return {shapes[i][0]: one(i) for i in range(len(shapes))}
    from concurrent.futures import ThreadPoolExecutor
    order = sorted(range(len(shapes)), key=lambda i: -int(np.prod(shapes[i][1])))
    with ThreadPoolExecutor(max_workers=threads) as ex:
        done = dict(zip(order, ex.map(one, order)))
    return {shapes[i][0]: done[i] for i in range(len(shapes))}



_V4_RENAMES = (
    ("visual.", "model.visual."),
    ("model.embed_tokens.", "model.language_model.embed_tokens."),
    ("model.layers.", "model.language_model.layers."),
    ("model.norm.", "model.language_model.norm."),
)


def canonical_name(name: str) -> str:
    if name.startswith("model.visual.") or name.startswith("model.language_model.") or name == "lm_head.weight":
        return name
    for old, new in _V4_RENAMES:
        if name.startswith(old):
            return new + name[len(old):]
    return name


def load_config(model_dir: str) -> ModelConfig:
    with open(os.path.join(model_dir, "config.json")) as f:
        return from_hf_config_dict(json.load(f), name=os.path.basename(model_dir.rstrip("/")))


def load_checkpoint(model_dir: str) -> tuple:
    from safetensors import safe_open

    cfg = load_config(model_dir)
    import torch

    tensors: Dict[str, np.ndarray] = {}
    files = sorted(f for f in os.listdir(model_dir) if f.endswith(".safetensors"))
    if not files:
        raise FileNotFoundError(f"no *.safetensors under {model_dir}")
    raw: Dict[str, np.ndarray] = {}
    for fn in files:
        with safe_open(os.path.join(model_dir, fn), framework="pt") as sf:
            for k in sf.keys():
                t = sf.get_tensor(k)
                if t.dtype == torch.bfloat16:
                    arr = t.view(torch.int16).numpy().view(np.uint16)
                else:
                    arr = t.float().numpy()
                raw[k] = arr
    for k in [k for k in raw if k.endswith(".weight_scale") or k.endswith(".weight_scale_inv")]:
        base = k[: k.rindex(".")] + ".weight"
        sc = as_f32(raw.pop(k)).reshape(-1)
        if base not in raw:
            continue
        w = as_f32(raw[base])
        if sc.size not in (1, w.shape[0]):
            raise ValueError(f"{k}: {sc.size} scales for a weight of shape {w.shape} (per-tensor or per-output-channel only)")
        raw[base] = w * (sc.reshape(-1, 1) if sc.size > 1 else sc[0])
    for k in [k for k in raw if k.endswith(".input_scale")]:
        raw.pop(k)
    for k, arr in raw.items():
        tensors[canonical_name(k)] = arr
    return cfg, tensors


def as_f32(w: np.ndarray) -> np.ndarray:
    return from_bf16_bits(w) if w.dtype == np.uint16 else np.asarray(w, dtype=np.float32)


def pack_w16x64(w: np.ndarray) -> np.ndarray:
    n, k = w.shape
    if n % 16 or k % 64:
        raise ValueError(f"pack_w16x64: shape {w.shape} is not a multiple of (16, 64)")
    return np.ascontiguousarray(w.reshape(n // 16, 16, k // 32, 4, 8).transpose(0, 2, 3, 1, 4)).reshape(n, k)


def pack_rows32(x: np.ndarray) -> np.ndarray:
    m, k = x.shape
    if m > 32 or k % 64:
        raise ValueError(f"pack_rows32: shape {x.shape} (at most 32 rows, K % 64 == 0)")
    full = np.zeros((32, k), x.dtype)
    full[:m] = x
    return np.ascontiguousarray(full.reshape(2, 16, k // 64, 2, 4, 8).transpose(2, 0, 3, 4, 1, 5)).reshape(-1)


def unpack_rows32(xp: np.ndarray, k: int) -> np.ndarray:
    return np.ascontiguousarray(np.asarray(xp).reshape(k // 64, 2, 2, 4, 16, 8).transpose(1, 4, 0, 2, 3, 5)).reshape(32, k)


def _e4m3_table() -> np.ndarray:
    codes = np.arange(256, dtype=np.int64)
    sign = np.where(codes & 0x80, -1.0, 1.0)
    e, m = (codes >> 3) & 0xF, codes & 0x7
    val = np.where(e == 0, m / 8.0 * 2.0 ** -6, (1.0 + m / 8.0) * 2.0 ** (e - 7.0))
    val = sign * val
    val[(codes & 0x7F) == 0x7F] = np.nan
    return val.astype(np.float32)


E4M3 = _e4m3_table()
E4M3_MAX = 448.0


def fp8_e4m3_to_f32(q: np.ndarray) -> np.ndarray:
    return E4M3[np.asarray(q, np.uint8)]


def f32_to_fp8_e4m3_fast(x: np.ndarray) -> np.ndarray:
    x = np.ascontiguousarray(x, np.float32)
    bits = x.view(np.uint32)
    sign = ((bits >> np.uint32(24)) & np.uint32(0x80)).astype(np.uint8)
    u = bits & np.uint32(0x7FFFFFFF)
    r = u - np.uint32((127 - 7) << 23)
    r = (r + np.uint32(0x7FFFF) + ((r >> np.uint32(20)) & np.uint32(1))) >> np.uint32(20)
    sub = np.rint(np.minimum(np.abs(x), np.float32(1.0)) * np.float32(512.0)).astype(np.uint32)
    is_sub = u < np.uint32((127 - 6) << 23)
    code = np.where(is_sub, sub, r)
    code = np.minimum(code, np.uint32(0x7E)).astype(np.uint8)
    return code | sign


def f32_to_fp8_e4m3(x: np.ndarray) -> np.ndarray:
    x = np.asarray(x, np.float32)
    mag = np.minimum(np.abs(x).astype(np.float64), E4M3_MAX)
    pos = E4M3[:0x7F].astype(np.float64)
    hi = np.clip(np.searchsorted(pos, mag, side="left"), 0, 0x7E)
    lo = np.clip(hi - 1, 0, 0x7E)
    d_lo, d_hi = mag - pos[lo], pos[hi] - mag
    pick_hi = (d_hi < d_lo) | ((d_hi == d_lo) & ((hi & 1) == 0))
    code = np.where(pick_hi, hi, lo).astype(np.uint8)
    return (code | np.where(np.signbit(x), 0x80, 0).astype(np.uint8)).astype(np.uint8)


def quantize_fp8_rows(w: np.ndarray) -> tuple:
    w = np.asarray(w, np.float32)
    amax = np.abs(w).max(axis=1)
    scale = np.where(amax > 0, amax / np.float32(E4M3_MAX), np.float32(1.0)).astype(np.float32)
    return f32_to_fp8_e4m3_fast(w / scale[:, None]), scale


def pack_w16x64_fp8(q: np.ndarray) -> np.ndarray:
    n, k = q.shape
    if n % 16 or k % 64:
        raise ValueError(f"pack_w16x64_fp8: shape {q.shape} is not a multiple of (16, 64)")
    return np.ascontiguousarray(q.reshape(n // 16, 16, k // 64, 4, 16).transpose(0, 2, 3, 1, 4)).reshape(n, k)


def unpack_w16x64_fp8(p: np.ndarray) -> np.ndarray:
    n, k = p.shape
    return np.ascontiguousarray(p.reshape(n // 16, k // 64, 4, 16, 16).transpose(0, 3, 1, 2, 4)).reshape(n, k)


FP8_LINEARS = ("self_attn.q_proj", "self_attn.k_proj", "self_attn.v_proj", "self_attn.o_proj", "mlp.gate_proj", "mlp.up_proj",
               "mlp.down_proj")


def fp8_dequantized_weights(weights: Dict[str, np.ndarray], cfg: ModelConfig) -> Dict[str, np.ndarray]:
    out = dict(weights)
    for i in range(cfg.text.num_layers):
        for n in FP8_LINEARS:
            key = f"model.language_model.layers.{i}.{n}.weight"
            q, s = quantize_fp8_rows(as_f32(weights[key]))
            out[key] = (fp8_e4m3_to_f32(q) * s[:, None]).astype(np.float32)
    return out


def unpack_w16x64(p: np.ndarray) -> np.ndarray:
    n, k = p.shape
    return np.ascontiguousarray(p.reshape(n // 16, k // 32, 4, 16, 8).transpose(0, 3, 1, 2, 4)).reshape(n, k)
```

Baseline: 6.129 pages/s.

## Fuse QKV GEMM with rotary embedding and K/V^T scatter epilogue

Adds a QKV GEMM variant whose epilogue applies bias and rotary embedding and then scatters Q, K and transposed V blocks straight into the attention buffers. This replaces the separate qkv_prep kernel and the intermediate QKV activation buffer for both the ViT and the LLM prefill in bf16. ViT QKV weights are reordered offline so rotary pairs fall in the same tile. The cost is a heavier epilogue with extra LDS staging and scattered stores. The fp8 path still uses the old two-step route.

```diff
diff --git a/include/karanta_hip.h b/include/karanta_hip.h
--- a/include/karanta_hip.h
+++ b/include/karanta_hip.h
@@ -64,6 +64,12 @@
 int kr_gemm_bf16_ws(const kr_bf16* A, int64_t lda, const kr_bf16* W, const kr_bf16* bias,
                     const kr_bf16* residual, int64_t ldr, kr_bf16* C, int64_t ldc,
                     int64_t M, int N, int K, int epilogue, int w_packed, float* scratch, size_t scratch_bytes, kr_stream s);
+
+int kr_gemm_qkv_bf16(const kr_bf16* A, int64_t lda, const kr_bf16* W, const kr_bf16* bias, int64_t M, int N, int K, int w_packed,
+                     const float* cos, const float* sin, const int32_t* row_dst,
+                     kr_bf16* q_out, int64_t q_head_stride, kr_bf16* k_out, int64_t k_head_stride,
+                     kr_bf16* vt_out, int64_t vt_head_stride, int q_heads, int kv_heads, int hd,
+                     float* scratch, size_t scratch_bytes, kr_stream s);
 
 int kr_gemm_fp8(const kr_bf16* A, int64_t lda, const uint8_t* w_packed_fp8, const float* w_scale, const kr_bf16* bias,
                 const kr_bf16* residual, int64_t ldr, kr_bf16* C, int64_t ldc, int64_t M, int N, int K, int epilogue,
diff --git a/karanta_ocr_amd/_lib.py b/karanta_ocr_amd/_lib.py
--- a/karanta_ocr_amd/_lib.py
+++ b/karanta_ocr_amd/_lib.py
@@ -46,6 +46,8 @@
     "kr_quantize_rows_fp8": [c_p, i64, c_p, i64, c_p, i64, i32, c_p],
     "kr_gemm_fp8a": [c_p, i64, c_p, c_p, c_p, c_p, c_p, i64, c_p, i64, i64, i32, i32, i32, c_p],
     "kr_gemm_bf16_ws": [c_p, i64, c_p, c_p, c_p, i64, c_p, i64, i64, i32, i32, i32, i32, c_p, C.c_size_t, c_p],
+    "kr_gemm_qkv_bf16": [c_p, i64, c_p, c_p, i64, i32, i32, i32, c_p, c_p, c_p, c_p, i64, c_p, i64, c_p, i64, i32, i32, i32, c_p,
+                         C.c_size_t, c_p],
     "kr_gemv_bf16": [c_p, i64, c_p, c_p, c_p, i64, c_p, c_p, i64, i32, i32, i32, i32, c_p, f32, c_p],
     "kr_qkv_prep": [c_p, i64, i32, i32, i32, c_p, c_p, c_p, c_p, c_p, c_p, i32, c_p, i64, c_p, i64, c_p, i64,
                     i32, i32, i32, c_p],
diff --git a/karanta_ocr_amd/csrc/kr_gemm.hip b/karanta_ocr_amd/csrc/kr_gemm.hip
--- a/karanta_ocr_amd/csrc/kr_gemm.hip
+++ b/karanta_ocr_amd/csrc/kr_gemm.hip
@@ -181,13 +181,168 @@
     tm = first + (r - tn * gsz);
 }
 
+constexpr int EPI_QKV_I80 = 100, EPI_QKV_128 = 101;
+struct QkvEpi {
+    const float *cos, *sin;
+    const int32_t* row_dst;
+    kr_bf16 *q, *k, *vt;
+    int64_t q_hs, k_hs, vt_hs;
+    int q_heads, kv_heads;
+};
+
+__device__ __forceinline__ void rope_pair8(bf16x8 a, bf16x8 b, const float* c0, const float* s0, const float* c1, const float* s1,
+                                           bf16x8& lo, bf16x8& hi) {
+#pragma unroll
+    for (int j = 0; j < 8; ++j) {
+        const float fa = bf2f(a[j]), fb = bf2f(b[j]);
+        lo[j] = f2bf(__builtin_fmaf(fa, c0[j], -__fmul_rn(fb, s0[j])));
+        hi[j] = f2bf(__builtin_fmaf(fa, s1[j], __fmul_rn(fb, c1[j])));
+    }
+}
+
+template <int EPI>
+constexpr bool is_qkv_epi = EPI == EPI_QKV_I80 || EPI == EPI_QKV_128;
+constexpr int qkv_lds_bytes(int bm, int bn) { return bm * bn * 2 + bm * 16; }
+
+template <int EPI, int BM, int BN, int NTHR, int NT, int MT>
+__device__ __forceinline__ void qkv_epilogue(f32x4 (&acc)[NT][MT], const kr_bf16* __restrict__ bias, const QkvEpi& e, int64_t M, int N,
+                                             int64_t m0, int n0, int wm, int wn, int fr, int fg, int tid, char* smem) {
+    constexpr int HD = EPI == EPI_QKV_I80 ? 80 : 128;
+    constexpr int CM = BN / 8 - 1;
+    auto tl = [](int r, int col) { return r * (BN * 2) + ((((col >> 3) ^ r) & CM) << 4) + (col & 7) * 2; };
+    int* const rinfo = reinterpret_cast<int*>(smem + BM * BN * 2);
+    const int v_off = (e.q_heads + e.kv_heads) * HD, k_off = e.q_heads * HD;
+    {
+        bf16x4 bv[NT];
+#pragma unroll
+        for (int nt = 0; nt < NT; ++nt)
+            bv[nt] = bias ? *reinterpret_cast<const bf16x4*>(bias + min(n0 + wn + nt * 16 + fg * 4, N - 4)) : bf16x4{};
+#pragma unroll
+        for (int mt = 0; mt < MT; ++mt) {
+            const int r = wm + mt * 16 + fr;
+#pragma unroll
+            for (int nt = 0; nt < NT; ++nt) {
+                float v[4];
+#pragma unroll
+                for (int j = 0; j < 4; ++j) v[j] = acc[nt][mt][j];
+                if (bias) {
+#pragma unroll
+                    for (int j = 0; j < 4; ++j) v[j] += bf2f(bv[nt][j]);
+                }
+                bf16x4 o;
+#pragma unroll
+                for (int j = 0; j < 4; ++j) o[j] = f2bf(v[j]);
+                *reinterpret_cast<bf16x4*>(smem + tl(r, wn + nt * 16 + fg * 4)) = o;
+            }
+        }
+    }
+    for (int r = tid; r < BM; r += NTHR) {
+        const int64_t m = m0 + r;
+        int kr = 0, vk = 0, code = 0;
+        if (m < M) {
+            kr = e.row_dst[2 * m];
+            vk = e.row_dst[2 * m + 1];
+            const int j8 = vk & 7, rs = r - j8;
+            const bool whole = rs >= 0 && rs + 7 < BM && m0 + rs + 7 < M && e.row_dst[2 * (m0 + rs) + 1] == vk - j8 &&
+                               e.row_dst[2 * (m0 + rs + 7) + 1] == vk - j8 + 7;
+            code = whole ? (j8 == 0 ? 1 : 0) : 2;
+            const bool last = m + 1 >= M || e.row_dst[2 * (m + 1) + 1] != vk + 1;
+            if (last) code |= (63 - (vk & 63)) << 8;
+        }
+        rinfo[4 * r + 0] = kr;
+        rinfo[4 * r + 1] = vk;
+        rinfo[4 * r + 2] = code;
+    }
+    __syncthreads();
+    {
+        constexpr int HC = HD / 16;
+        const int qk_end = min(v_off, N);
+        for (int idx = tid; idx < BM * HC; idx += NTHR) {
+            const int r = idx / HC, c = idx - r * HC;
+            const int64_t m = m0 + r;
+            if (m >= M) continue;
+            int col, step;
+            if constexpr (EPI == EPI_QKV_I80) {
+                const int cs = (n0 % HD) >> 4;
+                col = ((c - cs + HC) % HC) * 16;
+                step = HD;
+            } else {
+                col = c * 8;
+                step = HD;
+            }
+            if (n0 + col >= qk_end || col >= BN) continue;
+            const int d0 = c * 8, d1 = d0 + HD / 2;
+            float c0[8], s0[8], c1[8], s1[8];
+            {
+                const float* cp = e.cos + m * HD;
+                const float* sp = e.sin + m * HD;
+#pragma unroll
+                for (int h = 0; h < 2; ++h) {
+                    *reinterpret_cast<f32x4*>(c0 + 4 * h) = *reinterpret_cast<const f32x4*>(cp + d0 + 4 * h);
+                    *reinterpret_cast<f32x4*>(s0 + 4 * h) = *reinterpret_cast<const f32x4*>(sp + d0 + 4 * h);
+                    *reinterpret_cast<f32x4*>(c1 + 4 * h) = *reinterpret_cast<const f32x4*>(cp + d1 + 4 * h);
+                    *reinterpret_cast<f32x4*>(s1 + 4 * h) = *reinterpret_cast<const f32x4*>(sp + d1 + 4 * h);
+                }
+            }
+            const int64_t krow = rinfo[4 * r];
+            for (; col < BN && n0 + col < qk_end; col += step) {
+                const int n = n0 + col;
+                const int hi_col = EPI == EPI_QKV_I80 ? col + 8 : col + HD / 2;
+                const bf16x8 a = *reinterpret_cast<const bf16x8*>(smem + tl(r, col));
+                const bf16x8 b = *reinterpret_cast<const bf16x8*>(smem + tl(r, hi_col));
+                bf16x8 lo, hi;
+                rope_pair8(a, b, c0, s0, c1, s1, lo, hi);
+                const bool is_q = n < k_off;
+                const int head = (is_q ? n : n - k_off) / HD;
+                kr_bf16* dst = is_q ? e.q + (int64_t)head * e.q_hs + m * HD : e.k + (int64_t)head * e.k_hs + krow * HD;
+                st8(dst + d0, lo);
+                st8(dst + d1, hi);
+            }
+        }
+    }
+    {
+        const int vc0 = max(0, v_off - n0), vc1 = min(BN, N - n0);
+        if (vc0 < vc1) {
+            constexpr int RG = BM / 32, NW = NTHR / 64;
+            const int ncg = (vc1 - vc0) >> 4;
+            const int o = tid & 3, dd = (tid >> 2) & 15, wave = tid >> 6;
+            for (int it = wave; it < RG * ncg; it += NW) {
+                const int rg = it % RG, cg = it / RG;
+                const int col = vc0 + cg * 16 + dd;
+                const int vn = n0 + col - v_off, head = vn / HD, d = vn - head * HD;
+                kr_bf16* const vt = e.vt + (int64_t)head * e.vt_hs;
+                unsigned short* const vts = reinterpret_cast<unsigned short*>(vt);
+#pragma unroll 1
+                for (int s = 0; s < 8; ++s) {
+                    const int r = rg * 32 + o * 8 + s;
+                    if (m0 + r >= M) break;
+                    const int vk = rinfo[4 * r + 1], code = rinfo[4 * r + 2];
+                    const int64_t blk = (int64_t)(vk >> 6) * (HD * 64);
+                    if ((code & 3) == 1) {
+                        unsigned short x[8];
+#pragma unroll
+                        for (int i = 0; i < 8; ++i) x[i] = *reinterpret_cast<const unsigned short*>(smem + tl(r + i, col));
+                        u32x4 v;
+#pragma unroll
+                        for (int i = 0; i < 4; ++i) v[i] = (unsigned)x[2 * i] | ((unsigned)x[2 * i + 1] << 16);
+                        *reinterpret_cast<u32x4*>(vt + blk + kr_vt_off(d, vk & 63, HD)) = v;
+                    } else if ((code & 3) == 2) {
+                        vts[blk + kr_vt_off(d, vk & 63, HD)] = *reinterpret_cast<const unsigned short*>(smem + tl(r, col));
+                    }
+                    for (int p = 1; p <= (code >> 8); ++p) vts[blk + kr_vt_off(d, (vk & 63) + p, HD)] = 0;
+                }
+            }
+        }
+    }
+}
+
 template <int EPI, bool WPACK, typename G, int STAGES = 2>
 __global__ void __launch_bounds__(G::WM * G::WN * 64) gemm_kernel(const kr_bf16* __restrict__ A, int64_t lda,
                                                    const kr_bf16* __restrict__ W, const kr_bf16* __restrict__ bias,
                                                    const kr_bf16* __restrict__ R, int64_t ldr, kr_bf16* __restrict__ C,
                                                    int64_t ldc, int64_t M, int N, int K, int tiles_n, unsigned nwg,
                                                    int ptiles_n, unsigned qbase, int group_m, int ksplit, int ks_mode,
-                                                   float* __restrict__ ws) {
+                                                   float* __restrict__ ws, QkvEpi qe = QkvEpi{}) {
     constexpr int BM = G::BM, BN = G::BN, NTHR = G::WM * G::WN * 64;
     constexpr int WTM = BM / G::WM, WTN = BN / G::WN;
     constexpr int MT = WTM / 16, NT = WTN / 16;
@@ -316,8 +471,12 @@
             for (int j = 0; j < MT; ++j) part[i * MT + j] = acc[i][j];
         return;
     }
-    gemm_epilogue<EPI, NT, MT, G::BM == 256>(acc, bias, R, ldr, C, ldc, M, N, m0 + wr * WTM, n0 + wc * WTN, fr, fg,
-                                             smem + wave * (WTM * 128));
+    if constexpr (is_qkv_epi<EPI>) {
+        qkv_epilogue<EPI, BM, BN, NTHR, NT, MT>(acc, bias, qe, M, N, m0, n0, wr * WTM, wc * WTN, fr, fg, tid, smem);
+    } else {
+        gemm_epilogue<EPI, NT, MT, G::BM == 256>(acc, bias, R, ldr, C, ldc, M, N, m0 + wr * WTM, n0 + wc * WTN, fr, fg,
+                                                 smem + wave * (WTM * 128));
+    }
 }
 
 constexpr int PK = 32, PBUF = 2 * 256 * PK * 2, PSTAGES = 4;
@@ -376,8 +535,10 @@
                                                         const kr_bf16* __restrict__ bias, const kr_bf16* __restrict__ R,
                                                         int64_t ldr, kr_bf16* __restrict__ C, int64_t ldc, int64_t M, int N, int K,
                                                         int tiles_n, unsigned nwg, const float* __restrict__ w_scale, int group_m,
-                                                        const float* __restrict__ a_scale = nullptr, int stagger = 0) {
+                                                        const float* __restrict__ a_scale = nullptr, int stagger = 0,
+                                                        QkvEpi qe = QkvEpi{}) {
     static_assert(!A8 || W8, "fp8 activations go with fp8 weights");
+    static_assert(!is_qkv_epi<EPI> || (!W8 && !PERSIST), "the QKV epilogue: bf16 weights, one tile per workgroup");
     if (stagger > 0 && blockIdx.x < 256u && ((blockIdx.x >> 3) & 1u)) {
         for (int i = 0; i < stagger; ++i) __builtin_amdgcn_s_sleep(127);
     }
@@ -568,6 +729,9 @@
         if (!more_tiles) break;
         asm volatile("s_waitcnt vmcnt(0)" ::: "memory");
         __builtin_amdgcn_s_barrier();
+    } else if constexpr (is_qkv_epi<EPI>) {
+        qkv_epilogue<EPI, 256, 256, 512, NT, MT>(acc, bias, qe, M, N, m0_cur, n0_cur, wr * 128, wc * 64, fr, fg, tid, smem);
+        break;
     } else {
         gemm_epilogue<EPI, NT, MT, true>(acc, bias, R, ldr, C, ldc, M, N, m0_cur + wr * 128, n0_cur + wc * 64, fr, fg,
                                          smem + wave * (128 * 128));
@@ -944,6 +1108,7 @@
     float* scratch;
     kr_stream s;
     GemmTuning tune;
+    QkvEpi qkv{};
 };
 constexpr int TAIL_MAX_WGS = 512, TAIL_WG_BYTES = 256 * 16 * 16;
 static_assert((size_t)TAIL_MAX_WGS * TAIL_WG_BYTES == KR_GEMM_SCRATCH_BYTES, "karanta_hip.h: KR_GEMM_SCRATCH_BYTES");
@@ -951,14 +1116,16 @@
 template <int EPI, bool WPACK, typename G, int STAGES>
 int launch_gemm_kernel(const GemmCall& c, unsigned nwg, int tiles_n, int ptiles_n, unsigned qbase, int group_m, int ksplit = 1,
                        int ks_mode = 0, float* ws = nullptr) {
-    constexpr int LDS = STAGES * (G::BM + G::BN) * BK * 2;
+    constexpr int RING = STAGES * (G::BM + G::BN) * BK * 2;
+    constexpr int LDS = is_qkv_epi<EPI> ? std::max(RING, qkv_lds_bytes(G::BM, G::BN)) : RING;
     static KrPerDeviceOnce attr_set;
     if (attr_set.need()) {
         KR_CHECK_HIP(hipFuncSetAttribute(reinterpret_cast<const void*>(&gemm_kernel<EPI, WPACK, G, STAGES>),
                                          hipFuncAttributeMaxDynamicSharedMemorySize, LDS));
     }
     gemm_kernel<EPI, WPACK, G, STAGES><<<nwg, G::WM * G::WN * 64, LDS, kr_hs(c.s)>>>(
-        c.A, c.lda, c.W, c.bias, c.R, c.ldr, c.C, c.ldc, c.M, c.N, c.K, tiles_n, nwg, ptiles_n, qbase, group_m, ksplit, ks_mode, ws);
+        c.A, c.lda, c.W, c.bias, c.R, c.ldr, c.C, c.ldc, c.M, c.N, c.K, tiles_n, nwg, ptiles_n, qbase, group_m, ksplit, ks_mode, ws,
+        c.qkv);
     KR_CHECK_LAUNCH();
     return KR_OK;
 }
@@ -993,7 +1160,7 @@
 
 template <int EPI, bool WPACK, bool W8 = false, bool A8 = false>
 int launch_gemm_pipe(const GemmCall& c) {
-    constexpr int LDS = PSTAGES * PBUF;
+    constexpr int LDS = is_qkv_epi<EPI> ? std::max(PSTAGES * PBUF, qkv_lds_bytes(256, 256)) : PSTAGES * PBUF;
     const int64_t tiles_m = (c.M + 255) / 256;
     const int tiles_n = (c.N + 255) / 256;
     int64_t nwg = tiles_m * tiles_n;
@@ -1025,7 +1192,7 @@
 #endif
         gemm_pipe_kernel<EPI, WPACK, W8, A8><<<(unsigned)nwg, 512, LDS, kr_hs(c.s)>>>(
             c.A, c.lda, c.W, c.bias, c.R, c.ldr, c.C, c.ldc, c.M, c.N, c.K, tiles_n, (unsigned)nwg, c.w_scale, group_m, c.a_scale,
-            c.tune.stagger);
+            c.tune.stagger, c.qkv);
     KR_CHECK_LAUNCH();
     if constexpr (!W8) {
         if (tail) return launch_gemm_tail<EPI, WPACK>(c, tiles_n, (unsigned)nwg, tail, group_m);
@@ -1118,6 +1285,33 @@
     }
 }
 
+extern "C" int kr_gemm_qkv_bf16(const kr_bf16* A, int64_t lda, const kr_bf16* W, const kr_bf16* bias, int64_t M, int N, int K,
+                                int w_packed, const float* cos, const float* sin, const int32_t* row_dst, kr_bf16* q_out,
+                                int64_t q_head_stride, kr_bf16* k_out, int64_t k_head_stride, kr_bf16* vt_out, int64_t vt_head_stride,
+                                int q_heads, int kv_heads, int hd, float* scratch, size_t scratch_bytes, kr_stream s) {
+    KR_CHECK_ARG(scratch == nullptr || (scratch_bytes >= KR_GEMM_SCRATCH_BYTES && ((uintptr_t)scratch & 15) == 0),
+                 "kr_gemm_qkv_bf16: scratch of %zu bytes (KR_GEMM_SCRATCH_BYTES = %zu, 16-byte aligned)", scratch_bytes,
+                 (size_t)KR_GEMM_SCRATCH_BYTES);
+    KR_CHECK_ARG(A && W && cos && sin && row_dst && q_out && k_out && vt_out, "kr_gemm_qkv_bf16: null pointer");
+    KR_CHECK_ARG(M >= 0 && M < (1ll << 30) && N > 0 && K > 0 && K % BK == 0, "kr_gemm_qkv_bf16: bad sizes M=%lld N=%d K=%d (K %% %d)",
+                 (long long)M, N, K, BK);
+    KR_CHECK_ARG((hd == 80 && !w_packed) || (hd == 128 && w_packed),
+                 "kr_gemm_qkv_bf16: hd=%d w_packed=%d (80 with row-major pair-interleaved W, or 128 with W in the decode layout)", hd,
+                 w_packed);
+    KR_CHECK_ARG(q_heads > 0 && kv_heads > 0 && (int64_t)(q_heads + 2 * kv_heads) * hd == N, "kr_gemm_qkv_bf16: N=%d is not (%d + 2 x %d) x %d",
+                 N, q_heads, kv_heads, hd);
+    KR_CHECK_ARG(lda >= K && (lda & 7) == 0 && ((uintptr_t)A & 15) == 0 && ((uintptr_t)W & 15) == 0 && (bias == nullptr || ((uintptr_t)bias & 7) == 0),
+                 "kr_gemm_qkv_bf16: operand alignment");
+    KR_CHECK_ARG(((uintptr_t)cos & 15) == 0 && ((uintptr_t)sin & 15) == 0 && ((uintptr_t)row_dst & 7) == 0 && ((uintptr_t)q_out & 15) == 0 &&
+                     ((uintptr_t)k_out & 15) == 0 && ((uintptr_t)vt_out & 15) == 0 && (q_head_stride & 7) == 0 && (k_head_stride & 7) == 0 &&
+                     (vt_head_stride & 7) == 0,
+                 "kr_gemm_qkv_bf16: table / destination alignment");
+    if (M == 0) return KR_OK;
+    GemmCall c{A, lda, W, bias, nullptr, 0, nullptr, 0, M, N, K, nullptr, nullptr, scratch, s, GemmTuning()};
+    c.qkv = QkvEpi{cos, sin, row_dst, q_out, k_out, vt_out, q_head_stride, k_head_stride, vt_head_stride, q_heads, kv_heads};
+    return hd == 80 ? launch_gemm2<EPI_QKV_I80, false>(c) : launch_gemm2<EPI_QKV_128, true>(c);
+}
+
 namespace {
 template <int QMAX>
 __global__ void __launch_bounds__(256) quantize_rows_fp8_kernel(const kr_bf16* __restrict__ x, int64_t ldx, uint8_t* __restrict__ q,
diff --git a/karanta_ocr_amd/engine.py b/karanta_ocr_amd/engine.py
--- a/karanta_ocr_amd/engine.py
+++ b/karanta_ocr_amd/engine.py
@@ -16,7 +16,7 @@
                    KarantaHipError, lib, narrow_opts, ptr)
 from .config import ModelConfig
 from .sampling import StepFeatures, adjust_table, has_penalties, needs_processing, sampling_params, temperature
-from .weights import pack_w16x64, to_bf16_bits
+from .weights import interleave_rotary_rows, pack_w16x64, to_bf16_bits
 
 BF16 = torch.bfloat16
 GEMM_SCRATCH_BYTES = 512 * 65536
@@ -132,7 +132,12 @@
                 names += [("norm1.bias", "ln1.b"), ("norm2.bias", "ln2.b"), ("mlp.fc1.weight", "fc1.w"),
                           ("mlp.fc1.bias", "fc1.b"), ("mlp.fc2.weight", "fc2.w"), ("mlp.fc2.bias", "fc2.b")]
             for a, b in names:
-                self._put(d + b, _bits(w[s + a]))
+                bits = _bits(w[s + a])
+                if b in ("qkv.w", "qkv.b"):
+                    D = v.embed_dim
+                    bits = np.concatenate([interleave_rotary_rows(bits[:D], v.num_heads, v.head_dim),
+                                           interleave_rotary_rows(bits[D:2 * D], v.num_heads, v.head_dim), bits[2 * D:]], 0)
+                self._put(d + b, bits)
             if v25:
                 ffv, fp, D = v.mlp_dim, v.mlp_dim_padded, v.embed_dim
                 def padded(a, rows):
@@ -245,12 +250,13 @@
     qblk: torch.Tensor
     qlen: torch.Tensor
     n_blk: int
+    rows: torch.Tensor
 
 
 def device_plan(plan: POS.AttnPlan, dev: torch.device) -> DevicePlan:
     t_ = lambda a: torch.from_numpy(np.ascontiguousarray(a)).to(dev)
     return DevicePlan(plan, t_(plan.blk_tok0), t_(plan.blk_ntok), t_(plan.blk_k_row0), t_(plan.blk_vt_blk), t_(plan.qblk),
-                      t_(plan.qblk_len), len(plan.blk_tok0))
+                      t_(plan.qblk_len), len(plan.blk_tok0), t_(POS.attn_row_table(plan)))
 
 
 @dataclass
@@ -357,7 +363,6 @@
         self.v_in = z(N, v.patch_dim_padded)
         self.v_x = z(N, v.embed_dim)
         self.v_h = z(N, v.embed_dim)
-        self.v_qkv = z(N, 3 * v.embed_dim)
         self.v_q = z(v.num_heads, N, v.head_dim)
         self.v_k = z(v.num_heads, N, v.head_dim)
         self.v_vt = z(v.num_heads, nvb, v.head_dim, 64)
@@ -370,7 +375,7 @@
         self.img_embeds = z(N // 4 + 1, t.hidden_size)
         self.p_x = z(M, t.hidden_size)
         self.p_h = z(M, t.hidden_size)
-        self.p_qkv = z(M, t.qkv_dim)
+        self.p_qkv = z(M, t.qkv_dim) if self.fp8 else None
         self.p_q = z(t.num_heads, M, t.head_dim)
         self.p_o = z(M, t.q_dim)
         self.p_act = z(M, t.intermediate_size)
@@ -714,8 +719,8 @@
             for i in range(v.depth):
                 p = f"vit.{i}."
                 norm(p + "ln1")
-                self._gemm(h, w.view(p + "qkv.w"), self.v_qkv, n, bias=w.view(p + "qkv.b"))
-                self._attention(self.v_qkv, D, 2 * D, tab.cos, tab.sin, tab.win if v25 and i not in v.fullatt_block_indexes else tab.full,
+                self._attention(h, w.view(p + "qkv.w"), w.view(p + "qkv.b"), n, False, None, tab.cos, tab.sin,
+                                tab.win if v25 and i not in v.fullatt_block_indexes else tab.full,
                                 self.v_q, self.v_k, self.v_k.stride(0), self.v_vt, self.v_vt.stride(0), self.v_o, H, H, hd, causal=False)
                 self._gemm(self.v_o, w.view(p + "proj.w"), x, n, bias=w.view(p + "proj.b"), res=x)
                 norm(p + "ln2")
@@ -731,11 +736,19 @@
                 L.kr_embed_scatter(ptr(tab.inv), ptr(out), 0, ptr(self.img_embeds), T, d_out, s)
         return self.img_embeds[:T]
 
-    def _attention(self, qkv, k_off, v_off, cos, sin, dp: DevicePlan, q, k, k_stride, vt, vt_stride, out, H, KVH, hd, causal):
+    def _attention(self, x, W, bias, M, packed, w8kw, cos, sin, dp: DevicePlan, q, k, k_stride, vt, vt_stride, out, H, KVH, hd, causal):
         L, s = self.L, self.s
-        L.kr_qkv_prep(ptr(qkv), qkv.shape[1], 0, k_off, v_off, ptr(cos), ptr(sin),
-                      ptr(dp.blk_tok0), ptr(dp.blk_ntok), ptr(dp.blk_kr), ptr(dp.blk_vb), dp.n_blk,
-                      ptr(q), q.stride(0), ptr(k), k_stride, ptr(vt), vt_stride, H, KVH, hd, s)
+        N, K = W.shape
+        if w8kw:
+            qkv, k_off, v_off = self.p_qkv, H * hd, (H + KVH) * hd
+            self._gemm(x, W, qkv, M, bias=bias, packed=packed, **w8kw)
+            L.kr_qkv_prep(ptr(qkv), qkv.shape[1], 0, k_off, v_off, ptr(cos), ptr(sin),
+                          ptr(dp.blk_tok0), ptr(dp.blk_ntok), ptr(dp.blk_kr), ptr(dp.blk_vb), dp.n_blk,
+                          ptr(q), q.stride(0), ptr(k), k_stride, ptr(vt), vt_stride, H, KVH, hd, s)
+        else:
+            L.kr_gemm_qkv_bf16(ptr(x), x.stride(0), ptr(W), ptr(bias), M, N, K, 1 if packed else 0, ptr(cos), ptr(sin), ptr(dp.rows),
+                               ptr(q), q.stride(0), ptr(k), k_stride, ptr(vt), vt_stride, H, KVH, hd, ptr(self.gemm_scratch),
+                               self.gemm_scratch.numel() * 4, s)
         L.kr_attn_varlen_q(ptr(q), ptr(k), ptr(vt), ptr(out), ptr(dp.qblk), ptr(dp.qlen), dp.host.qblk.shape[0], q.shape[1],
                            H, KVH, hd, k_stride, vt_stride, hd ** -0.5, 1 if causal else 0, dp.host.q_block, s)
 
@@ -889,10 +902,10 @@
             for i in range(t.num_layers):
                 p = f"llm.{i}."
                 L.kr_rmsnorm(ptr(self.p_x), d, ptr(w.view(p + "ln1.w")), ptr(self.p_h), M, d, t.rms_norm_eps, s)
-                self._gemm(self.p_h, w.view(p + "qkv.w"), self.p_qkv, M, bias=w.view(p + "qkv.b"), packed=True, **self._w8kw(p + "qkv.w"))
                 kc, vc = self.kcache[i], self.vtcache[i]
-                self._attention(self.p_qkv, t.q_dim, t.q_dim + t.kv_dim, self.p_cos, self.p_sin, dp, self.p_q, kc, kc.stride(1),
-                                vc, vc.stride(1), self.p_o, t.num_heads, t.num_kv_heads, t.head_dim, causal=True)
+                self._attention(self.p_h, w.view(p + "qkv.w"), w.view(p + "qkv.b"), M, True, self._w8kw(p + "qkv.w"), self.p_cos, self.p_sin,
+                                dp, self.p_q, kc, kc.stride(1), vc, vc.stride(1), self.p_o, t.num_heads, t.num_kv_heads, t.head_dim,
+                                causal=True)
                 self._gemm(self.p_o, w.view(p + "o.w"), self.p_x, M, res=self.p_x, packed=True, **self._w8kw(p + "o.w"))
                 L.kr_rmsnorm(ptr(self.p_x), d, ptr(w.view(p + "ln2.w")), ptr(self.p_h), M, d, t.rms_norm_eps, s)
                 self._gemm(self.p_h, w.view(p + "gate_up.w"), self.p_act, M, epi=EPI_SILU_MUL8, packed=True, **self._w8kw(p + "gate_up.w"))
diff --git a/karanta_ocr_amd/positions.py b/karanta_ocr_amd/positions.py
--- a/karanta_ocr_amd/positions.py
+++ b/karanta_ocr_amd/positions.py
@@ -135,6 +135,17 @@
         np.asarray(qlen, np.int32).reshape(-1, 2), tok, nvb, q_block)
 
 
+def attn_row_table(plan: AttnPlan) -> np.ndarray:
+    tab = np.zeros((plan.n_tokens, 2), np.int32)
+    for t0, n, kr, vb in zip(plan.blk_tok0, plan.blk_ntok, plan.blk_k_row0, plan.blk_vt_blk):
+        j = np.arange(int(n), dtype=np.int64)
+        if int(kr) + int(n) >= 2 ** 31 or int(vb) * 64 + 64 >= 2 ** 31:
+            raise ValueError("attn_row_table: K row / V^T key index beyond int32")
+        tab[int(t0):int(t0) + int(n), 0] = int(kr) + j
+        tab[int(t0):int(t0) + int(n), 1] = int(vb) * 64 + j
+    return tab
+
+
 def vit_attn_plan(grid_thw: Sequence[Sequence[int]]) -> AttnPlan:
     lens = [int(t * h * w) for t, h, w in grid_thw]
     k_row0 = np.concatenate([[0], np.cumsum(lens)[:-1]]) if lens else []
diff --git a/karanta_ocr_amd/weights.py b/karanta_ocr_amd/weights.py
--- a/karanta_ocr_amd/weights.py
+++ b/karanta_ocr_amd/weights.py
@@ -197,6 +197,13 @@
     return np.ascontiguousarray(w.reshape(n // 16, 16, k // 32, 4, 8).transpose(0, 2, 3, 1, 4)).reshape(n, k)
 
 
+def interleave_rotary_rows(w: np.ndarray, heads: int, hd: int) -> np.ndarray:
+    if w.shape[0] != heads * hd or hd % 16:
+        raise ValueError(f"interleave_rotary_rows: shape {w.shape} for {heads} heads of {hd}")
+    a = w.reshape(heads, 2, hd // 16, 8, *w.shape[1:])
+    return np.ascontiguousarray(np.swapaxes(a, 1, 2)).reshape(w.shape)
+
+
 def pack_rows32(x: np.ndarray) -> np.ndarray:
     m, k = x.shape
     if m > 32 or k % 64:
```

Result: no change. 6.125 pages/s (median of 2 runs) (-0.1%).
